# kmjc/riptide

Measured on AMD Instinct MI355X. Metric: DM trials/sec (node) at 2^23 samples, P=0.1-10 s; FFA-pass HBM GB/s, higher is better.
Workload: dtype f32

## Files before the change

### include/riptide_amd.h

```cpp
#ifndef RIPTIDE_AMD_H
#define RIPTIDE_AMD_H

#include <stddef.h>
#include <stdint.h>

#ifdef __cplusplus
extern "C" {
#endif

#define RT_OK 0
#define RT_EINVAL 1
#define RT_EHIP 2
#define RT_EINTERNAL 3

const char* rt_last_error(void);
const char* rt_version(void);
int rt_set_device(int device);


int rt_rollback(const float* x, size_t size, size_t shift, float* out);

int rt_fused_rollback_add(const float* x, const float* y, size_t size, size_t shift, float* out);

int rt_circular_prefix_sum(const float* x, size_t size, size_t nsum, float* out);

int rt_ffa2(const float* in, size_t rows, size_t cols, float* out);

int rt_benchmark_ffa2(size_t rows, size_t cols, size_t loops, double* seconds);

int rt_snr1(const float* x, size_t size, const uint64_t* widths, size_t num_widths, float stdnoise, float* out);

int rt_snr2(const float* x, size_t rows, size_t cols, const uint64_t* widths, size_t num_widths,
            float stdnoise, float* out);

size_t rt_downsampled_size(size_t size, double f);

int rt_downsample(const float* x, size_t size, double factor, float* out);
int rt_downsample_rows(const float* x, size_t rows, size_t size, double f, float* out);

int rt_periodogram_length(size_t size, double tsamp, double period_min, double period_max,
                          size_t bins_min, size_t bins_max, size_t* length);

int rt_periodogram(const float* data, size_t size, double tsamp, const uint64_t* widths, size_t num_widths,
                   double period_min, double period_max, size_t bins_min, size_t bins_max,
                   double* periods, uint32_t* foldbins, float* snrs);

int rt_running_median(const float* x, size_t size, size_t width, float* out);

int rt_fast_running_median(const float* x, size_t size, size_t width_samples, size_t min_points, double* out);

int rt_deredden_normalise(const float* x, size_t size, size_t width_samples, size_t min_points,
                          int deredden, int normalise, float* out);

int rt_periodogram_grid(size_t size, double tsamp, double period_min, double period_max, size_t bins_min,
                        size_t bins_max, double* periods, uint32_t* foldbins);

int rt_schedule_check(size_t size, double tsamp, size_t num_widths, double period_min, double period_max,
                      size_t bins_min, size_t bins_max, uint64_t* transforms, uint64_t* items,
                      uint64_t* launches, double* alg_bytes_per_trial, double* moved_bytes_per_trial,
                      uint64_t* cells_per_trial);

int rt_schedule_final_kinds(size_t size, double tsamp, const uint64_t* widths, size_t num_widths, double period_min,
                            double period_max, size_t bins_min, size_t bins_max, uint64_t* launches,
                            uint64_t* rows_launches, uint64_t* seg_launches, uint8_t* bins_kinds, size_t bins_cap);

int rt_ladder_check(size_t size, double tsamp, double period_min, double period_max, size_t bins_min,
                    size_t bins_max, int* fused, uint64_t* rungs);

typedef struct rt_ladder_rung {
    double   f;
    uint64_t n;
    uint64_t leaf_off;
    uint32_t fused;
    uint32_t reserved;
} rt_ladder_rung;
int rt_ladder_layout(size_t size, double tsamp, double period_min, double period_max, size_t bins_min,
                     size_t bins_max, rt_ladder_rung* rungs, size_t cap, uint64_t* count, uint64_t* leaf_floats,
                     int* mode, uint32_t* margin);

int rt_ffa_schedule_check(size_t rows, size_t cols, uint64_t* launches);


typedef struct rt_plan rt_plan;

int rt_plan_create(size_t size, double tsamp, const uint64_t* widths, size_t num_widths,
                   double period_min, double period_max, size_t bins_min, size_t bins_max,
                   rt_plan** plan);
void rt_plan_destroy(rt_plan* plan);
int rt_plan_shape(const rt_plan* plan, size_t* length, size_t* num_widths);
int rt_plan_grid(const rt_plan* plan, double* periods, uint32_t* foldbins);
int rt_plan_workspace_bytes(const rt_plan* plan, size_t batch, size_t* bytes);

int rt_periodogram_device(const rt_plan* plan, const float* d_data, size_t batch, size_t data_stride,
                          float* d_snrs, size_t snr_stride, void* d_workspace, size_t workspace_bytes,
                          void* stream);
int rt_periodogram_ladder_device(const rt_plan* plan, const float* d_data, size_t batch, size_t data_stride,
                                 void* d_workspace, size_t workspace_bytes, void* stream);
int rt_periodogram_passes_device(const rt_plan* plan, size_t batch, float* d_snrs, size_t snr_stride,
                                 void* d_workspace, size_t workspace_bytes, void* stream);

int rt_plan_check(const rt_plan* plan, void* stream);

int rt_deredden_workspace_bytes(size_t size, size_t width_samples, size_t min_points, size_t batch,
                                size_t* bytes);
int rt_deredden_normalise_device(const float* d_in, size_t size, size_t batch, size_t in_stride,
                                 size_t width_samples, size_t min_points, int deredden, int normalise,
                                 float* d_out, size_t out_stride, void* d_workspace, size_t workspace_bytes,
                                 void* stream);

int rt_segment_order_stats_device(const float* d_snrs, size_t batch, size_t snr_stride, size_t length,
                                  size_t num_widths, size_t nseg, size_t per_seg, const uint32_t* ranks,
                                  size_t nranks, float* d_out, void* stream);
int rt_threshold_select_device(const float* d_snrs, size_t batch, size_t snr_stride, size_t length,
                               size_t num_widths, const double* d_logf, const double* d_coeffs, size_t ncoef,
                               double smin, uint32_t* d_counts, uint32_t* d_idx, size_t cap, void* stream);
int rt_find_peaks_workspace_bytes(size_t batch, size_t length, size_t num_widths, size_t chunk_rows, size_t* bytes);
int rt_find_peaks_device(const float* d_snrs, size_t batch, size_t snr_stride, size_t length, size_t num_widths,
                         const double* d_logf, const double* d_freqs, const double* d_coeffs, size_t ncoef,
                         double smin, double radius, uint32_t* d_counts, uint32_t* d_rows, float* d_snr,
                         size_t cap, size_t chunk_rows, void* d_workspace, size_t workspace_bytes, void* stream);
int rt_find_peaks_host(const float* snrs, size_t length, size_t num_widths, const double* logf, const double* freqs,
                       const double* coeffs, size_t ncoef, double smin, double radius,
                       uint32_t* counts, uint32_t* rows, float* snr, size_t cap);

typedef struct rt_fold_spec {
    double   factor;
    uint64_t out_off;
    uint32_t series;
    uint32_t bins;
    uint32_t subints;
    uint32_t reserved;
} rt_fold_spec;

int rt_fold_shape(size_t size, double factor, size_t bins, size_t subints, size_t* m, size_t* rows);
int rt_fold_workspace_bytes(size_t size, const rt_fold_spec* specs, size_t nspecs, size_t* bytes);
int rt_fold_device(const float* d_data, size_t size, size_t data_stride, size_t nseries,
                   const rt_fold_spec* specs, size_t nspecs, float* d_out, size_t out_floats,
                   void* d_workspace, size_t workspace_bytes, void* stream);
int rt_fold(const float* x, size_t size, size_t nseries, const rt_fold_spec* specs, size_t nspecs,
            float* out, size_t out_floats);

typedef struct rt_htest_params {
    double   tobs;
    double   band;
    double   phase_distance_max;
    double   dm_distance_max;
    double   snr_distance_max;
    uint32_t denom_max;
} rt_htest_params;

int rt_hdiag_host(const double* freq, const double* snr, const double* ducy, const double* dm, size_t n,
                  const int32_t* pi, const int32_t* pj, size_t npairs, const rt_htest_params* params,
                  int64_t* num, int64_t* den, double* phase_distance, double* dm_distance, double* snr_distance);
int rt_hdiag_pairs(const double* freq, const double* snr, const double* ducy, const double* dm, size_t n,
                   const int32_t* pi, const int32_t* pj, size_t npairs, const rt_htest_params* params,
                   int64_t* num, int64_t* den, double* phase_distance, double* dm_distance, double* snr_distance);
int rt_flag_harmonics(const double* freq, const double* snr, const double* ducy, const double* dm, size_t n,
                      const rt_htest_params* params, size_t block_rows, int32_t* parent, int64_t* hnum,
                      int64_t* hden);
int rt_flag_harmonics_stats(uint64_t* tiles, uint64_t* near_pairs, uint64_t* host_rows, double* kernel_ms);

int rt_convert_samples_device(const void* d_raw, size_t n, int is_signed, float* d_out, void* stream);

int rt_profile_enable(int on);
int rt_profile_read(int kind, double* milliseconds, double* alg_bytes, double* moved_bytes, uint64_t* launches);
int rt_profile_reset(void);

int rt_diag_stamps(uint64_t* out8, int reset);
int rt_diag_timeline(uint64_t* out, uint64_t cap, uint64_t* count);
int rt_diag_launches(uint64_t* out, uint64_t cap, uint64_t* count);

int rt_plan_stats(const rt_plan* plan, uint64_t* transforms, uint64_t* items, uint64_t* launches,
                  double* alg_bytes_per_trial, double* moved_bytes_per_trial, uint64_t* cells_per_trial);


#ifdef __cplusplus
}
#endif

#endif
```

### riptide_amd/_lib.py

```python
import ctypes
import os

_HERE = os.path.dirname(os.path.abspath(__file__))
LIB_PATH = os.environ.get("RIPTIDE_AMD_LIB") or os.path.join(_HERE, "libriptide_amd.so")

RT_OK, RT_EINVAL, RT_EHIP, RT_EINTERNAL = 0, 1, 2, 3

_c_sz = ctypes.c_size_t
_c_d = ctypes.c_double
_c_f = ctypes.c_float
_c_i = ctypes.c_int
_vp = ctypes.c_void_p
_psz = ctypes.POINTER(ctypes.c_size_t)
_pd = ctypes.POINTER(ctypes.c_double)
_pu64 = ctypes.POINTER(ctypes.c_uint64)

_SIGNATURES = {
    "rt_last_error": (ctypes.c_char_p, []),
    "rt_version": (ctypes.c_char_p, []),
    "rt_set_device": (_c_i, [_c_i]),
    "rt_rollback": (_c_i, [_vp, _c_sz, _c_sz, _vp]),
    "rt_fused_rollback_add": (_c_i, [_vp, _vp, _c_sz, _c_sz, _vp]),
    "rt_circular_prefix_sum": (_c_i, [_vp, _c_sz, _c_sz, _vp]),
    "rt_ffa2": (_c_i, [_vp, _c_sz, _c_sz, _vp]),
    "rt_benchmark_ffa2": (_c_i, [_c_sz, _c_sz, _c_sz, _pd]),
    "rt_snr1": (_c_i, [_vp, _c_sz, _vp, _c_sz, _c_f, _vp]),
    "rt_snr2": (_c_i, [_vp, _c_sz, _c_sz, _vp, _c_sz, _c_f, _vp]),
    "rt_downsampled_size": (_c_sz, [_c_sz, _c_d]),
    "rt_downsample": (_c_i, [_vp, _c_sz, _c_d, _vp]),
    "rt_downsample_rows": (_c_i, [_vp, _c_sz, _c_sz, _c_d, _vp]),
    "rt_fold_shape": (_c_i, [_c_sz, _c_d, _c_sz, _c_sz, _psz, _psz]),
    "rt_fold_workspace_bytes": (_c_i, [_c_sz, _vp, _c_sz, _psz]),
    "rt_fold_device": (_c_i, [_vp, _c_sz, _c_sz, _c_sz, _vp, _c_sz, _vp, _c_sz, _vp, _c_sz, _vp]),
    "rt_fold": (_c_i, [_vp, _c_sz, _c_sz, _vp, _c_sz, _vp, _c_sz]),
    "rt_periodogram_length": (_c_i, [_c_sz, _c_d, _c_d, _c_d, _c_sz, _c_sz, _psz]),
    "rt_periodogram": (_c_i, [_vp, _c_sz, _c_d, _vp, _c_sz, _c_d, _c_d, _c_sz, _c_sz, _vp, _vp, _vp]),
    "rt_running_median": (_c_i, [_vp, _c_sz, _c_sz, _vp]),
    "rt_fast_running_median": (_c_i, [_vp, _c_sz, _c_sz, _c_sz, _vp]),
    "rt_deredden_normalise": (_c_i, [_vp, _c_sz, _c_sz, _c_sz, _c_i, _c_i, _vp]),
    "rt_periodogram_grid": (_c_i, [_c_sz, _c_d, _c_d, _c_d, _c_sz, _c_sz, _vp, _vp]),
    "rt_ffa_schedule_check": (_c_i, [_c_sz, _c_sz, _pu64]),
    "rt_schedule_check": (_c_i, [_c_sz, _c_d, _c_sz, _c_d, _c_d, _c_sz, _c_sz, _pu64, _pu64, _pu64, _pd, _pd,
                                 _pu64]),
    "rt_schedule_final_kinds": (_c_i, [_c_sz, _c_d, _vp, _c_sz, _c_d, _c_d, _c_sz, _c_sz, _pu64, _pu64, _pu64, _vp,
                                       _c_sz]),
    "rt_plan_create": (_c_i, [_c_sz, _c_d, _vp, _c_sz, _c_d, _c_d, _c_sz, _c_sz, _vp]),
    "rt_plan_destroy": (None, [_vp]),
    "rt_plan_shape": (_c_i, [_vp, _psz, _psz]),
    "rt_plan_grid": (_c_i, [_vp, _vp, _vp]),
    "rt_plan_workspace_bytes": (_c_i, [_vp, _c_sz, _psz]),
    "rt_periodogram_device": (_c_i, [_vp, _vp, _c_sz, _c_sz, _vp, _c_sz, _vp, _c_sz, _vp]),
    "rt_periodogram_ladder_device": (_c_i, [_vp, _vp, _c_sz, _c_sz, _vp, _c_sz, _vp]),
    "rt_periodogram_passes_device": (_c_i, [_vp, _c_sz, _vp, _c_sz, _vp, _c_sz, _vp]),
    "rt_plan_check": (_c_i, [_vp, _vp]),
    "rt_deredden_workspace_bytes": (_c_i, [_c_sz, _c_sz, _c_sz, _c_sz, _psz]),
    "rt_deredden_normalise_device": (_c_i, [_vp, _c_sz, _c_sz, _c_sz, _c_sz, _c_sz, _c_i, _c_i, _vp, _c_sz,
                                            _vp, _c_sz, _vp]),
    "rt_profile_enable": (_c_i, [_c_i]),
    "rt_profile_read": (_c_i, [_c_i, _pd, _pd, _pd, _pu64]),
    "rt_profile_reset": (_c_i, []),
    "rt_diag_stamps": (_c_i, [_pu64, _c_i]),
    "rt_diag_timeline": (_c_i, [_pu64, ctypes.c_uint64, _pu64]),
    "rt_diag_launches": (_c_i, [_pu64, ctypes.c_uint64, _pu64]),
    "rt_plan_stats": (_c_i, [_vp, _pu64, _pu64, _pu64, _pd, _pd, _pu64]),
    "rt_convert_samples_device": (_c_i, [_vp, _c_sz, _c_i, _vp, _vp]),
    "rt_segment_order_stats_device": (_c_i, [_vp, _c_sz, _c_sz, _c_sz, _c_sz, _c_sz, _c_sz, _vp, _c_sz, _vp, _vp]),
    "rt_threshold_select_device": (_c_i, [_vp, _c_sz, _c_sz, _c_sz, _c_sz, _vp, _vp, _c_sz, _c_d, _vp, _vp, _c_sz,
                                          _vp]),
    "rt_find_peaks_workspace_bytes": (_c_i, [_c_sz, _c_sz, _c_sz, _c_sz, _psz]),
    "rt_find_peaks_device": (_c_i, [_vp, _c_sz, _c_sz, _c_sz, _c_sz, _vp, _vp, _vp, _c_sz, _c_d, _c_d, _vp, _vp, _vp,
                                    _c_sz, _c_sz, _vp, _c_sz, _vp]),
    "rt_find_peaks_host": (_c_i, [_vp, _c_sz, _c_sz, _vp, _vp, _vp, _c_sz, _c_d, _c_d, _vp, _vp, _vp, _c_sz]),
    "rt_ladder_check": (_c_i, [_c_sz, _c_d, _c_d, _c_d, _c_sz, _c_sz, ctypes.POINTER(_c_i), _pu64]),
    "rt_ladder_layout": (_c_i, [_c_sz, _c_d, _c_d, _c_d, _c_sz, _c_sz, _vp, _c_sz, _pu64, _pu64,
                                ctypes.POINTER(_c_i), ctypes.POINTER(ctypes.c_uint32)]),
    "rt_hdiag_host": (_c_i, [_vp, _vp, _vp, _vp, _c_sz, _vp, _vp, _c_sz, _vp, _vp, _vp, _vp, _vp, _vp]),
    "rt_hdiag_pairs": (_c_i, [_vp, _vp, _vp, _vp, _c_sz, _vp, _vp, _c_sz, _vp, _vp, _vp, _vp, _vp, _vp]),
    "rt_flag_harmonics": (_c_i, [_vp, _vp, _vp, _vp, _c_sz, _vp, _c_sz, _vp, _vp, _vp]),
    "rt_flag_harmonics_stats": (_c_i, [_pu64, _pu64, _pu64, _pd]),
}

EXPORTED = tuple(_SIGNATURES)

_TEST_SIGNATURES = {
    "rt_test_corrupt_next_plans": (_c_i, [_c_i]),
}
TESTHOOKS_PATH = os.path.join(_HERE, "libriptide_amd_testhooks.so")

_lib = None


class EngineError(RuntimeError):
    """A HIP runtime or internal failure inside the engine."""


def load():
    global _lib
    if _lib is not None:
        return _lib
    if not os.path.exists(LIB_PATH):
        raise ImportError(
            f"riptide_amd engine library not found at {LIB_PATH}; build it with "
            "`make -C riptide_amd/csrc` or `python -c 'import __graft_entry__ as g; g.build()'`")
    try:
        import torch
    except ImportError:
        pass
    lib = ctypes.CDLL(LIB_PATH, mode=ctypes.RTLD_LOCAL)
    for name, (res, args) in _SIGNATURES.items():
        fn = getattr(lib, name)
        fn.restype = res
        fn.argtypes = args
    for name, (res, args) in _TEST_SIGNATURES.items():
        if hasattr(lib, name):
            fn = getattr(lib, name)
            fn.restype = res
            fn.argtypes = args
    _lib = lib
    return lib


def check(rc):
    if rc == RT_OK:
        return
    msg = _lib.rt_last_error().decode("utf-8", "replace")
    if rc == RT_EINVAL:
        raise ValueError(msg)
    raise EngineError(msg)


def ptr(a):
    if hasattr(a, "data_ptr"):
        return ctypes.c_void_p(a.data_ptr())
    return ctypes.c_void_p(a.ctypes.data)
```

### riptide_amd/csrc/common.hpp

```cpp
#pragma once
#include <cmath>
#include <cstddef>
#include <cstdint>

#if defined(__HIPCC__)
#define RT_HD __host__ __device__
#else
#define RT_HD
#endif

namespace rt {

constexpr int kConeWgsPerCu = 2;
constexpr int kConeBlock = 512;
static_assert(kConeBlock % 64 == 0, "whole waves");
constexpr int kConeWaves = kConeBlock / 64;
constexpr int kConeWavesPerSimd = kConeWgsPerCu * kConeWaves / 4;
constexpr int kLdsBufFloats = 18176;
constexpr int kLdsDataFloats = kLdsBufFloats - 256;
constexpr int kLdsPadFloats = 128;
constexpr int kMaxRows = 384;
constexpr int kDescEntries = 1024;
constexpr int kMaxTileLevels = 6;
constexpr int kMaxLevels = 11;
constexpr int kMaxRanges = (1 << (kMaxTileLevels + 1)) - 1;
constexpr int kMaxWidths = 32;
constexpr int kSnrChunk = 17;
constexpr int kSnrWin = 12;
constexpr int kSnrMaxChunk = 17;
RT_HD inline int snr_wide_stride(int p, int wmax)
{
    return p + (wmax > kSnrMaxChunk ? wmax : kSnrMaxChunk);
}
RT_HD inline bool snr_wide_ok(int p, int q, int wmax)
{
    return wmax > kSnrWin && wmax < p && q >= snr_wide_stride(p, wmax);
}
RT_HD constexpr int snr_group(int p)
{
    int G = 8;
    while (G < 64 && ((((p + G - 1) / G) | 1) > kSnrMaxChunk)) G <<= 1;
    return G;
}
constexpr int kSnrSegCols = 33;
constexpr int kSnrSegWmax = 9;
constexpr int kSnrSegRows = 64;
constexpr int kSnrSegStride = 8 * kSnrSegCols + 1;
constexpr int kSnrSegExch = 2 * 64 * 8;
static_assert(kSnrSegRows * kSnrSegStride <= kLdsDataFloats, "segmented S/N rows");
static_assert(kSnrSegRows * kSnrSegStride + kSnrSegExch <= kLdsBufFloats, "segmented S/N exchange area");
RT_HD inline bool snr_seg_ok(int p, int wmax, int rows)
{
    return p >= 8 * kSnrSegCols - 24 && p <= 8 * kSnrSegCols && wmax >= 1 && wmax <= kSnrSegWmax && rows >= 1 &&
           rows <= kSnrSegRows;
}
RT_HD inline bool snr_seg_unit(int smax, int levels, int p, int wmax, int rows)
{
    return (smax == 4 || smax == 5) && levels > 0 && snr_seg_ok(p, wmax, rows);
}
constexpr int kStageRegs = 45 * 8 / kConeWaves;
constexpr int kMaxSlots = 45;
constexpr int kMaxRowsPerWave = 24;
constexpr int kBlobHeader = 48;
enum : int {
    kHdrRows = 0, kHdrDesc = 12, kHdrRuns = 24, kHdrEntries = 25, kHdrBottom = 26, kHdrSlotWords = 27,
    kHdrRunOff = 28, kHdrFill = 29, kHdrZero = 30, kHdrSlotOff = 32
};
enum : uint32_t { kSlotOne = 0, kSlotTwo = 1, kSlotPair = 2, kSlotHalf = 3 };
constexpr int kSlotWords = 544;
RT_HD constexpr bool resolved_slots(int smax) { return smax == 4 || smax == 5; }
constexpr int kAuxMetaWords = kBlobHeader + kDescEntries + kMaxRows + kSlotWords;
constexpr int kLutPad = 64;
constexpr int kLut4Words = 2 * (256 + 64);
constexpr int kLut4Off = kAuxMetaWords + kLutPad - kLut4Words;
constexpr uint32_t kNoBlob = 0xFFFFFFFFu;
constexpr uint32_t kCarriedRow = 1023;
RT_HD inline int fill_chunks_bound(int n, int p, int runs) { return (n * p + 6 * runs + 3) >> 2; }
RT_HD inline int pack_blob_words(int entries, int nb) { return (kBlobHeader + entries + nb + 2 * kMaxLevels + 4) & ~3; }

constexpr int kPack2 = 64;
RT_HD inline int merge_slots(uint32_t p)
{
    if (p <= 32) return kPack2;
    if (p == 0) return 1;
    const int s = (int)((p + 63) / 64);
    if (s <= 5) return s;
    if (s <= 8) return 8;
    if (s <= 11) return 11;
    if (s <= 16) return 16;
    if (s <= 22) return 22;
    if (s <= kMaxSlots) return kMaxSlots;
    return 0;
}

RT_HD inline int pack_stride(int p)
{
    if (p < 8) return p;
    if (p < 16) return p <= 8 ? 9 : 17;
    if (p <= 32)
        return p == 16 ? 34 : p < 20 ? 35 : p < 25 ? 36 : p < 28 ? 37 : p == 28 ? 36 : p == 29 ? 37 : 38;
    return p | 1;
}
RT_HD constexpr int slot_count(int smax) { return smax == kPack2 ? 1 : smax; }
RT_HD constexpr int row_pack(int smax) { return smax == kPack2 ? 2 : 1; }

constexpr int kRw4 = (72 + kConeWaves - 1) / kConeWaves;
RT_HD constexpr int merge_rows_per_wave(int smax)
{
    return smax == 4
               ? kRw4
               : (kStageRegs / slot_count(smax) < 1
                      ? 1
                      : (kStageRegs / slot_count(smax) < kMaxRowsPerWave ? kStageRegs / slot_count(smax)
                                                                         : kMaxRowsPerWave));
}

RT_HD inline int lds_row_capacity(uint32_t p, int smax)
{
    if (!smax || p == 0) return 0;
    int c = kLdsDataFloats / (int)p;
    const int stage = kConeWaves * merge_rows_per_wave(smax) * row_pack(smax);
    if (stage < c) c = stage;
    return c < kMaxRows ? c : kMaxRows;
}

RT_HD inline int lds_row_capacity(uint32_t p) { return lds_row_capacity(p, merge_slots(p)); }

constexpr uint32_t kDsSpanFloats = 4096;
constexpr uint32_t kDsFusedMargin = 512;
constexpr uint32_t kDsMaxRungs = 256;

struct DsRung {
    double f;
    uint64_t n;
    uint64_t out_off;
    uint32_t first_block;
    uint32_t identity;
    uint32_t per_block;
    uint32_t staged;
};

inline uint32_t ds_per_block(double f)
{
    const double o = std::floor((double)(kDsSpanFloats - 4) / (f + 1.0)) - 1.0;
    if (o < 1.0) return 0;
    return o > 256.0 ? 256u : (uint32_t)o;
}

inline void ds_configure(DsRung& r)
{
    const uint32_t o = r.identity ? 256u : ds_per_block(r.f);
    r.staged = o >= 32;
    r.per_block = r.staged ? o : 256u;
}

inline uint32_t ds_fused_margin(const DsRung* rungs, size_t num_rungs)
{
    double need = 2.0;
    for (size_t i = 0; i < num_rungs; ++i)
        if (!rungs[i].identity) need = std::fmax(need, std::ceil(rungs[i].f) + 2.0);
    if (need > (double)kDsFusedMargin) return 0;
    const uint32_t m = ((uint32_t)need + 63u) & ~63u;
    return m < kDsFusedMargin ? m : kDsFusedMargin;
}

struct FfaXform {
    uint32_t p;
    uint32_t m;
    uint32_t rows_eval;
    uint32_t rung;
    uint64_t src_off;
    uint64_t buf_off;
    uint64_t snr_row;
    float stdnoise;
    uint32_t pad;
};
static_assert(sizeof(FfaXform) == 48, "FfaXform layout");

enum : uint8_t { kModeWhole = 0, kModeTile = 1 };
constexpr int kStampMarks = 16;
constexpr int kStampRecWords = kStampMarks + 2;
constexpr uint64_t kTimelineCap = 1u << 23;
enum : uint32_t {
    kConeStoreFromRegs = 1u,
    kConeFuse2 = 2u,
    kConeSnrStride = 4u,
    kConeSnrSeg = 8u,
    kConeDiagNoSnr = 1u << 30,
    kConeDiagNoMerge = 1u << 29,
    kConeDiagNoWrite = 1u << 28,
    kConeDiagNoBarrier = 1u << 27,
    kConeDiagNoLand = 1u << 26,
    kConeDiagNoDesc = 1u << 25,
    kConeDiagNoFill = 1u << 23,
    kConeDefaultFeatures = 15u
};
enum : uint8_t { kSelLeaves = 0, kSelPing = 1, kSelPong = 2, kSelSnr = 3, kSelSnrSeg = 4 };
RT_HD inline bool is_snr_dst(int dst) { return dst == kSelSnr || dst == kSelSnrSeg; }
enum : uint32_t { kSnrNone = 0, kSnrRows = 1, kSnrSeg = 2 };

struct ConeItem {
    uint32_t xform;
    uint32_t node_start;
    uint32_t node_size;
    uint32_t s0, s1;
    uint8_t levels;
    uint8_t mode;
    uint8_t src;
    uint8_t dst;
    uint32_t pad;
};
static_assert(sizeof(ConeItem) == 28, "ConeItem layout");

struct UnitDesc {
    uint32_t node_start, node_size, s0, s1;
    uint32_t p, m, rows_eval;
    float stdnoise;
    uint64_t src_off, buf_off, snr_row;
    uint8_t levels, mode, src, dst;
    uint32_t pad;
    uint32_t nruns, entries, nb, slot_words, run_off;
    uint32_t fill_chunks;
    uint32_t zero_row;
    uint32_t pad2;
};
static_assert(sizeof(UnitDesc) == 96, "UnitDesc layout");

struct ConeArgs {
    const UnitDesc* items;
    uint32_t num_items;
    uint32_t num_widths;
    const float* leaves;
    uint64_t leaves_stride;
    float* ping;
    float* pong;
    uint64_t buf_stride;
    float* snr;
    uint64_t snr_stride;
    const uint32_t* widths;
    int* error_flag;
    const uint32_t* blob;
    unsigned long long* stamps;
    uint32_t batch;
    uint32_t flags;
    uint32_t trials_per_wg;
};
constexpr uint32_t kConeTrialsPerWg = 16;
RT_HD inline uint32_t cone_trial_groups(uint32_t batch, uint32_t tpw)
{
    const uint32_t t = tpw ? tpw : 1u;
    return (batch + t - 1) / t;
}

#if defined(__HIPCC__)
__host__ __device__
#endif
inline uint32_t merge_index(float k, uint32_t s)
{
#if defined(__HIP_DEVICE_COMPILE__)
    return (uint32_t)__builtin_fmaf(k, (float)s, 0.5f);
#else
    return (uint32_t)__builtin_fmaf(k, (float)s, 0.5f);
#endif
}

#if defined(__HIPCC__)
__host__ __device__
#endif
inline float merge_coef(uint32_t child_rows, uint32_t rows)
{
    return ((float)child_rows - 1.0f) / ((float)rows - 1.0f);
}

}
```

### riptide_amd/csrc/ffa_kernels.hip

```cpp
#include <hip/hip_runtime.h>

#include <cstdlib>

#include "common.hpp"
#include "kernels.hpp"

namespace rt {

template <int N> struct IntC { static constexpr int value = N; };

__device__ __forceinline__ float window_sum(const float* w, float wmin, uint32_t cnt)
{
    float acc = __fmul_rn(wmin, w[0]);
    uint32_t i = 1;
    for (; i + 8 <= cnt; i += 8) {
        float v[8];
#pragma unroll
        for (int j = 0; j < 8; ++j) v[j] = w[i + j];
#pragma unroll
        for (int j = 0; j < 8; ++j) acc = __fadd_rn(acc, v[j]);
    }
    if (i < cnt) {
        float v[8];
#pragma unroll
// ... 341 lines not shown
}

template <class T>
__device__ __forceinline__ T* uni_ptr(T* p)
{
    return reinterpret_cast<T*>(uni64(reinterpret_cast<uint64_t>(p)));
}

struct UnitView {
    int item, trial;
    int node_start, node_size, s0, s1, levels, mode, src, dst;
    int p, m, rows_eval;
    uint64_t src_off, buf_off, snr_row;
    float stdnoise;
    uint32_t blob;
    int nruns, entries, nb, slot_words, run_off;
    int fill_chunks;
    int zero_row;
};

typedef const __attribute__((address_space(4))) uint32_t* const_u32_ptr;

__device__ __forceinline__ UnitView unit_view(const ConeArgs& a, int item, int trial)
{
    UnitView v;
    v.item = uni(item);
    v.trial = uni(trial);
    const const_u32_ptr w = (const_u32_ptr)(uintptr_t)(a.items + v.item);
    uint32_t x[sizeof(UnitDesc) / 4];
#pragma unroll
    for (int i = 0; i < (int)(sizeof(UnitDesc) / 4); ++i) x[i] = w[i];
    UnitDesc d;
    __builtin_memcpy(&d, x, sizeof d);
    v.node_start = uni((int)d.node_start);
    v.node_size = uni((int)d.node_size);
    v.s0 = uni((int)d.s0);
    v.s1 = uni((int)d.s1);
    v.levels = uni((int)d.levels);
    v.mode = uni((int)d.mode);
    v.src = uni((int)d.src);
    v.dst = uni((int)d.dst);
    v.p = uni((int)d.p);
    v.m = uni((int)d.m);
    v.rows_eval = uni((int)d.rows_eval);
    v.src_off = uni64(d.src_off);
    v.buf_off = uni64(d.buf_off);
    v.snr_row = uni64(d.snr_row);
    v.stdnoise = __int_as_float(uni(__float_as_int(d.stdnoise)));
    v.blob = (uint32_t)uni((int)d.pad);
    v.nruns = uni((int)d.nruns);
    v.entries = uni((int)d.entries);
    v.nb = uni((int)d.nb);
    v.slot_words = uni((int)d.slot_words);
    v.run_off = uni((int)d.run_off);
    v.fill_chunks = uni((int)d.fill_chunks);
    v.zero_row = uni((int)d.zero_row);
    return v;
}

constexpr int kAuxWords = kBlobHeader + kDescEntries + kMaxRows + kSlotWords;
static_assert(kAuxWords == kAuxMetaWords, "metadata area");
struct UnitCtx {
    UnitView U;
    bool tile;
    bool table;
    int al;
    bool slots;
    int nruns, entries, nb;
    const uint32_t* aux;
    const uint32_t* aux0;
    uint4 sv;
    int mine;
};

__device__ __forceinline__ int rows_at(const UnitCtx& C, int l)
{
    return C.table ? uni((int)C.aux[kHdrRows + l]) : C.U.node_size;
}
__device__ __forceinline__ int desc_offset(const UnitCtx& C, int l) { return uni((int)C.aux[kHdrDesc + l]); }
__device__ __forceinline__ const uint32_t* desc_table(const UnitCtx& C) { return C.aux + kBlobHeader; }
__device__ __forceinline__ const uint32_t* slot_table(const UnitCtx& C, int lo)
{
    return C.aux + uni((int)C.aux[kHdrSlotOff + lo]);
}
__device__ __forceinline__ const int* bottom_offsets(const UnitCtx& C)
{
    return reinterpret_cast<const int*>(desc_table(C) + C.entries);
}

__device__ __forceinline__ __amdgpu_buffer_rsrc_t buffer_rsrc(const void* p, uint32_t bytes)
{
    return __builtin_amdgcn_make_buffer_rsrc(uni_ptr(const_cast<void*>(p)), (short)0, uni((int)bytes), 0x00020000);
}

__device__ __forceinline__ void dma_run(__amdgpu_buffer_rsrc_t rs, uint32_t goff, int nch, float* lds, int wave,
                                        int wstep, int lane)
{
    for (int c0 = wave * 64; c0 < nch; c0 += wstep * 64) {
        const int c = c0 + lane;
        if (c < nch)
            __builtin_amdgcn_raw_ptr_buffer_load_lds(rs, (__attribute__((address_space(3))) void*)(lds + 4 * c0), 16,
                                                     (int)(goff + 16u * (uint32_t)c), 0, 0, kFillCpol);
    }
}

__device__ __forceinline__ __amdgpu_buffer_rsrc_t unit_src(const ConeArgs& a, const UnitView& U, int trial)
{
    const float* src;
    if (U.src == kSelLeaves) src = a.leaves + (uint64_t)trial * a.leaves_stride + U.src_off;
    else src = (U.src == kSelPing ? a.ping : a.pong) + (uint64_t)trial * a.buf_stride + U.buf_off;
    return buffer_rsrc(src, (((uint32_t)U.m * (uint32_t)U.p + 3u) & ~3u) * 4u);
}

template <int SMAX>
__device__ __forceinline__ void unit_fill(const ConeArgs& a, const UnitCtx& C, int trial, float* buf, int tid,
                                          bool blob_too)
{
    const int lane = tid & 63, wave = tid >> 6;
    const UnitView& U = C.U;
    const int p = U.p;
    const __amdgpu_buffer_rsrc_t rs = unit_src(a, U, trial);
    if (!C.table) {
        const int nch = (U.node_size * p + C.al + 3) >> 2;
        dma_run(rs, ((uint32_t)U.node_start * (uint32_t)p - (uint32_t)C.al) * 4u, nch, buf, wave, kConeWaves, lane);
        return;
    }
    const int words = U.run_off;
    const uint4 sv = C.sv;
    const int mine = C.mine;
    if (blob_too && wave == kConeWaves - 1) {
        const __amdgpu_buffer_rsrc_t rb = buffer_rsrc(a.blob + U.blob, (uint32_t)words * 4u);
        dma_run(rb, 0u, words >> 2, (float*)const_cast<uint32_t*>(C.aux), 0, 1, lane);
    }
    for (int i = 0; i < mine; ++i) {
        const int c0 = __builtin_amdgcn_readlane((int)sv.x, i);
        const int n = __builtin_amdgcn_readlane((int)sv.y, i);
        const uint32_t g = (uint32_t)__builtin_amdgcn_readlane((int)sv.z, i);
        if (lane < n && 4 * (c0 + n) <= kLdsBufFloats && !(a.flags & kConeDiagNoFill))
            __builtin_amdgcn_raw_ptr_buffer_load_lds(rs, (__attribute__((address_space(3))) void*)(buf + 4 * c0), 16,
                                                     (int)((g + (uint32_t)lane) * 16u), 0, 0, kFillCpol);
    }
}

__device__ __forceinline__ void unit_segments(const ConeArgs& a, UnitCtx& C, int tid)
{
    const int lane = tid & 63, wave = tid >> 6;
    const uint4* const segs = reinterpret_cast<const uint4*>(a.blob + C.U.blob + C.U.run_off);
    C.mine = uni(C.nruns > wave ? (C.nruns - wave + kConeWaves - 1) / kConeWaves : 0);
    C.sv = make_uint4(0u, 0u, 0u, 0u);
    const int K = (C.nruns + kConeWaves - 1) / kConeWaves;
    if (lane < C.mine) C.sv = segs[wave * K + lane];
}

template <int SMAX, int RW>
__device__ __forceinline__ UnitCtx unit_begin(const ConeArgs& a, uint32_t item, uint32_t trial, uint32_t* aux,
                                              float* buf, int tid, bool dma, bool& ok, unsigned long long* ts = nullptr)
{
    UnitCtx C;
    C.U = unit_view(a, (int)item, (int)trial);
    const UnitView& U = C.U;
#ifdef RT_STAMPS
    if (ts) ts[0] = __builtin_amdgcn_s_memtime() + (U.p & 0);
#endif
    C.tile = U.mode == kModeTile;
    C.table = U.blob != kNoBlob;
    C.aux = aux;
    C.aux0 = aux;
    const int p = U.p;
    const int slots = merge_slots((uint32_t)p);
    ok = U.levels <= kMaxLevels && p > 0 &&
         ((SMAX <= 5 || SMAX == kPack2) ? slots == SMAX : (slots <= SMAX && slots != kPack2));
    const int cap = min(lds_row_capacity((uint32_t)p, SMAX), kConeWaves * RW * row_pack(SMAX));
    if (!C.table) {
        ok = ok && SMAX != kPack2 && (!resolved_slots(SMAX) || U.levels == 0);
        C.al = (int)(((uint32_t)U.node_start * (uint32_t)p) & 3u);
        C.slots = false;
        C.nruns = C.entries = C.nb = 0;
        const int nch = (U.node_size * p + C.al + 3) >> 2;
        ok = ok && !C.tile && U.node_size <= cap && 4 * nch <= kLdsBufFloats;
    } else {
        C.al = 0;
        C.nruns = U.nruns;
        C.entries = U.entries;
        C.nb = U.nb;
        C.slots = U.slot_words != 0;
        const int words = U.run_off;
        if constexpr (SMAX == kPack2) {
            C.aux = reinterpret_cast<uint32_t*>(buf + kLdsBufFloats) - words;
            ok = ok && C.nb <= cap && 4 * U.fill_chunks + words <= kLdsBufFloats &&
                 C.nb * pack_stride(p) + words <= kLdsBufFloats;
        } else {
            ok = ok && C.nb <= cap && C.entries <= kDescEntries && words <= kAuxWords;
            if (SMAX == 4 && C.slots) ok = ok && words <= kLut4Off;
            if (resolved_slots(SMAX)) ok = ok && (U.levels == 0 || (C.slots && (a.flags & kConeFuse2)));
            if (U.zero_row)
                ok = ok && resolved_slots(SMAX) && !C.tile && U.zero_row >= 4 * U.fill_chunks &&
                     U.zero_row + 64 * SMAX <= kLdsDataFloats;
        }
        ok = ok && words >= kBlobHeader + C.entries + C.nb && C.nruns <= 64 * kConeWaves && (words & 3) == 0;
    }
#ifdef RT_STAMPS
    if (ts) ts[1] = __builtin_amdgcn_s_memtime() + (ok ? 0 : 0);
#endif
    C.sv = make_uint4(0u, 0u, 0u, 0u);
    C.mine = 0;
    if (ok && dma) {
        if (C.table) unit_segments(a, C, tid);
        unit_fill<SMAX>(a, C, (int)trial, buf, tid, true);
    }
#ifdef RT_STAMPS
    if (ts) ts[2] = __builtin_amdgcn_s_memtime();
#endif
    return C;
}

__device__ __forceinline__ int mod_small(int x, int p)
{
    const int q = (int)((float)x * __builtin_amdgcn_rcpf((float)p));
    int r = x - (int)__umul24((unsigned)q, (unsigned)p);
    r = r < 0 ? r + p : r;
    return r >= p ? r - p : r;
}

__device__ __forceinline__ void row_desc(int node_size, int l, int r, int p, int& h, int& t, int& sh)
{
    int a0 = 0, sz = node_size;
    for (int d = 0; d < l; ++d) {
        if (sz > 1) {
            const int hs = sz >> 1;
            if (r - a0 < hs) sz = hs;
            else {
                a0 += hs;
                sz -= hs;
            }
        }
    }
    if (sz <= 1) {
        h = r;
        t = -1;
        sh = 0;
    } else {
        const int s = r - a0;
        const uint32_t hs = (uint32_t)sz >> 1, ts = (uint32_t)sz - hs;
        const int hh = (int)merge_index(merge_coef(hs, (uint32_t)sz), (uint32_t)s);
        const int tt = (int)merge_index(merge_coef(ts, (uint32_t)sz), (uint32_t)s);
        h = a0 + hh;
        t = a0 + (int)hs + tt;
        sh = mod_small(s - tt, p);
    }
}

constexpr uint32_t kCarried = kCarriedRow;

__device__ __forceinline__ uint32_t pack_desc(int h, int t, int sh)
{
    return (uint32_t)h | ((t < 0 ? kCarried : (uint32_t)t) << 10) | ((uint32_t)sh << 20);
}

__device__ __forceinline__ uint32_t unit_desc(const UnitCtx& C, int l, int r, int p)
{
    if (C.table) return desc_table(C)[desc_offset(C, l) + r];
    int h, t, sh;
    row_desc(C.U.node_size, l, r, p, h, t, sh);
    return pack_desc(h, t, sh);
}

typedef const __attribute__((address_space(3))) float* lds_cptr;

__device__ __forceinline__ float lds_ld(lds_cptr p) { return *(const volatile __attribute__((address_space(3))) float*)p; }

template <int SMAX, int RW, bool CARRIED>
__device__ __forceinline__ void merge_level_dense(const UnitCtx& C, const float* src, int p, int l, int lane,
                                                  int wave, int nr, float (&v)[RW][SMAX], const int* loff)
{
    const int S = (p + 63) >> 6;
    int ho = 0, to = 0, sh = 0, car = 0;
    if (lane < nr) {
        const uint32_t d = unit_desc(C, l, wave + kConeWaves * lane, p);
        const uint32_t tc = (d >> 10) & 1023u;
        sh = (int)(d >> 20);
        ho = loff ? loff[d & 1023u] : (int)(d & 1023u) * p;
        to = (tc == kCarried ? ho : (loff ? loff[tc] : (int)tc * p)) + sh;
        car = tc == kCarried;
    }
    const lds_cptr l1 = (lds_cptr)src + lane;
#pragma unroll
    for (int i = 0; i < RW; ++i) {
        const int hoi = __builtin_amdgcn_readlane(ho, i);
        const int toi = __builtin_amdgcn_readlane(to, i);
        const int si = __builtin_amdgcn_readlane(sh, i);
        uint32_t keep = 0xFFFFFFFFu, neg0 = 0u;
        if (CARRIED) {
            keep = __builtin_amdgcn_readlane(car, i) ? 0u : 0xFFFFFFFFu;
            neg0 = ~keep & 0x80000000u;
        }
        const lds_cptr hrow = l1 + hoi;
        lds_cptr ta = l1 + toi;
        lds_cptr tw = ta - p;
        asm("" : "+v"(ta), "+v"(tw));
        const int ls = lane + si;
#pragma unroll
        for (int k = 0; k < SMAX; ++k) {
            if (SMAX <= 5 || k < S) {
                const lds_cptr tp = ls >= p - 64 * k ? tw : ta;
                float x = lds_ld(tp + 64 * k);
                if (CARRIED) x = __uint_as_float((__float_as_uint(x) & keep) | neg0);
                v[i][k] = __fadd_rn(hrow[64 * k], x);
            }
        }
    }
}

template <int SMAX, int RW>
__device__ __forceinline__ void merge_level2_dense(const UnitCtx& C, const float* src, int p, int l, int lane,
                                                   int wave, int nr, float (&v)[RW][SMAX], const int* loff)
{
    const int S = (p + 63) >> 6;
    int o0 = 0, o1 = 0, o2 = 0, o3 = 0, s1 = 0, s2 = 0, s3 = 0;
    if (lane < nr) {
        const uint32_t d0 = unit_desc(C, l, wave + kConeWaves * lane, p);
        const uint32_t dh = unit_desc(C, l + 1, (int)(d0 & 1023u), p);
        const uint32_t dt = unit_desc(C, l + 1, (int)((d0 >> 10) & 1023u), p);
        const int sh = (int)(d0 >> 20), sH = (int)(dh >> 20), sT = (int)(dt >> 20);
        int sTT = sh + sT;
        sTT = sTT >= p ? sTT - p : sTT;
        const uint32_t r0 = dh & 1023u, r1 = (dh >> 10) & 1023u, r2 = dt & 1023u, r3 = (dt >> 10) & 1023u;
        o0 = (loff ? loff[r0] : (int)r0 * p);
        o1 = (loff ? loff[r1] : (int)r1 * p) + sH;
        o2 = (loff ? loff[r2] : (int)r2 * p) + sh;
        o3 = (loff ? loff[r3] : (int)r3 * p) + sTT;
        s1 = sH;
        s2 = sh;
        s3 = sTT;
    }
    const lds_cptr l1 = (lds_cptr)src + lane;
#pragma unroll
    for (int i = 0; i < RW; ++i) {
        const lds_cptr hrow = l1 + __builtin_amdgcn_readlane(o0, i);
        lds_cptr b1 = l1 + __builtin_amdgcn_readlane(o1, i);
        lds_cptr b2 = l1 + __builtin_amdgcn_readlane(o2, i);
        lds_cptr b3 = l1 + __builtin_amdgcn_readlane(o3, i);
        lds_cptr w1 = b1 - p, w2 = b2 - p, w3 = b3 - p;
        asm("" : "+v"(b1), "+v"(w1), "+v"(b2), "+v"(w2), "+v"(b3), "+v"(w3));
        const int ls1 = lane + __builtin_amdgcn_readlane(s1, i);
        const int ls2 = lane + __builtin_amdgcn_readlane(s2, i);
        const int ls3 = lane + __builtin_amdgcn_readlane(s3, i);
#pragma unroll
        for (int k = 0; k < SMAX; ++k) {
            if (SMAX <= 5 || k < S) {
                const int wk = p - 64 * k;
// ... 93 lines not shown
        }
    } else if constexpr (!HEAD) {
        lds_cptr ta = l1 + r1;
        lds_cptr tw = ta - p;
        asm("" : "+v"(ta), "+v"(tw));
        const int ls = lane + t1;
#pragma unroll
        for (int k = 0; k < SMAX; ++k) ts[k] = lds_ld((ls >= p - 64 * k ? tw : ta) + 64 * k);
    } else {
        const lds_cptr hrow = l1 + r0;
        lds_cptr ta = l1 + r1;
        lds_cptr tw = ta - p;
        asm("" : "+v"(ta), "+v"(tw));
        const int ls = lane + t1;
        const uint32_t keep = c1 ? 0u : 0xFFFFFFFFu;
        const uint32_t neg0 = ~keep & 0x80000000u;
#pragma unroll
        for (int k = 0; k < SMAX; ++k) {
            const float x = lds_ld((ls >= p - 64 * k ? tw : ta) + 64 * k);
            hs[k] = lds_ld(hrow + 64 * k);
            ts[k] = __uint_as_float((__float_as_uint(x) & keep) | neg0);
        }
    }
}

typedef const __attribute__((address_space(3))) unsigned long long* lut_cptr;
typedef const __attribute__((address_space(3))) char* lds_ccptr;

__device__ __forceinline__ void rolled_lut4(lds_ccptr rb, unsigned long long e, float (&x)[4])
{
    const uint32_t e0 = (uint32_t)e, e1 = (uint32_t)(e >> 32);
    x[0] = lds_ld((lds_cptr)(rb + (e0 & 0xFFFFu)));
    x[1] = lds_ld((lds_cptr)(rb + (e0 >> 16)));
    x[2] = lds_ld((lds_cptr)(rb + (e1 & 0xFFFFu)));
    x[3] = lds_ld((lds_cptr)(rb + (e1 >> 16)));
}

template <bool TWO, bool HEAD = true>
__device__ __forceinline__ void row_terms_lut(lds_cptr l1, lds_cptr s0, lut_cptr lutl, int r0, int q1, int q2, int q3,
                                              int t1, int t2, int t3, int c1, float (&hs)[4], float (&ts)[4])
{
    const lds_ccptr b = (lds_ccptr)s0;
    if constexpr (TWO) {
        const unsigned long long e1 = HEAD ? lutl[t1] : 0ull;
        const unsigned long long e2 = lutl[t2], e3 = lutl[t3];
        float h[4], x1[4], x2[4], x3[4];
        if constexpr (HEAD) {
#pragma unroll
            for (int k = 0; k < 4; ++k) h[k] = lds_ld(l1 + r0 + 64 * k);
            rolled_lut4(b + 4 * q1, e1, x1);
        }
        rolled_lut4(b + 4 * q2, e2, x2);
        rolled_lut4(b + 4 * q3, e3, x3);
#pragma unroll
        for (int k = 0; k < 4; ++k) {
            if constexpr (HEAD) hs[k] = __fadd_rn(h[k], x1[k]);
            ts[k] = __fadd_rn(x2[k], x3[k]);
        }
    } else {
        const unsigned long long e = lutl[t1];
        float x[4];
        if constexpr (HEAD) {
#pragma unroll
            for (int k = 0; k < 4; ++k) hs[k] = lds_ld(l1 + r0 + 64 * k);
        }
        rolled_lut4(b + 4 * q1, e, x);
        if constexpr (HEAD) {
            const uint32_t keep = c1 ? 0u : 0xFFFFFFFFu;
            const uint32_t neg0 = ~keep & 0x80000000u;
#pragma unroll
            for (int k = 0; k < 4; ++k) ts[k] = __uint_as_float((__float_as_uint(x[k]) & keep) | neg0);
        } else {
#pragma unroll
            for (int k = 0; k < 4; ++k) ts[k] = x[k];
        }
    }
}

__device__ __forceinline__ void build_roll_lut4(uint32_t* lut, int p, int tid)
{
    for (int w = tid; w < 2 * (p + 64); w += kConeBlock) {
        const int x = (w >> 1) + 128 * (w & 1);
        int y0 = x, y1 = x + 64;
        y0 -= y0 >= p ? p : 0;
        y0 -= y0 >= p ? p : 0;
        y1 -= y1 >= p ? p : 0;
        y1 -= y1 >= p ? p : 0;
        lut[w] = (uint32_t)(4 * y0) | ((uint32_t)(4 * y1) << 16);
    }
}

template <int SMAX, bool TWO, bool HEAD = true>
__device__ __forceinline__ void row_terms(lds_cptr l1, int p, int lane, int i, int o0, int o1, int o2, int o3, int s1,
                                          int s2, int s3, float (&hs)[SMAX], float (&ts)[SMAX],
                                          lds_cptr s0 = nullptr, lut_cptr lutl = nullptr)
{
    if constexpr (SMAX == 4) {
        if constexpr (TWO) {
            if constexpr (HEAD) {
                int r0 = __builtin_amdgcn_readlane(o0, i), q1 = __builtin_amdgcn_readlane(o1, i);
                int q2 = __builtin_amdgcn_readlane(o2, i), q3 = __builtin_amdgcn_readlane(o3, i);
                int t1 = __builtin_amdgcn_readlane(s1, i), t2 = __builtin_amdgcn_readlane(s2, i);
                int t3 = __builtin_amdgcn_readlane(s3, i);
                asm volatile("" : "+s"(r0), "+s"(q1), "+s"(q2), "+s"(q3), "+s"(t1), "+s"(t2), "+s"(t3));
                row_terms_lut<true>(l1, s0, lutl, r0, q1, q2, q3, t1, t2, t3, 0, hs, ts);
            } else {
                int q2 = __builtin_amdgcn_readlane(o2, i), q3 = __builtin_amdgcn_readlane(o3, i);
                int t2 = __builtin_amdgcn_readlane(s2, i), t3 = __builtin_amdgcn_readlane(s3, i);
                asm volatile("" : "+s"(q2), "+s"(q3), "+s"(t2), "+s"(t3));
                row_terms_lut<true, false>(l1, s0, lutl, 0, 0, q2, q3, 0, t2, t3, 0, hs, ts);
            }
        } else {
            if constexpr (HEAD) {
                int r0 = __builtin_amdgcn_readlane(o0, i), q1 = __builtin_amdgcn_readlane(o1, i);
                int t1 = __builtin_amdgcn_readlane(s1, i), c1 = __builtin_amdgcn_readlane(o2, i);
                asm volatile("" : "+s"(r0), "+s"(q1), "+s"(t1), "+s"(c1));
                row_terms_lut<false>(l1, s0, lutl, r0, q1, 0, 0, t1, 0, 0, c1, hs, ts);
            } else {
                int q1 = __builtin_amdgcn_readlane(o1, i), t1 = __builtin_amdgcn_readlane(s1, i);
                asm volatile("" : "+s"(q1), "+s"(t1));
                row_terms_lut<false, false>(l1, s0, lutl, 0, q1, 0, 0, t1, 0, 0, 0, hs, ts);
            }
        }
        return;
    }
    if constexpr (TWO) {
        if constexpr (HEAD) {
            int r0 = __builtin_amdgcn_readlane(o0, i), r1 = __builtin_amdgcn_readlane(o1, i);
            int r2 = __builtin_amdgcn_readlane(o2, i), r3 = __builtin_amdgcn_readlane(o3, i);
            int t1 = __builtin_amdgcn_readlane(s1, i), t2 = __builtin_amdgcn_readlane(s2, i);
            int t3 = __builtin_amdgcn_readlane(s3, i);
            asm volatile("" : "+s"(r0), "+s"(r1), "+s"(r2), "+s"(r3), "+s"(t1), "+s"(t2), "+s"(t3));
            row_terms_s<SMAX, true>(l1, p, lane, r0, r1, r2, r3, t1, t2, t3, 0, hs, ts);
        } else {
            int r2 = __builtin_amdgcn_readlane(o2, i), r3 = __builtin_amdgcn_readlane(o3, i);
            int t2 = __builtin_amdgcn_readlane(s2, i), t3 = __builtin_amdgcn_readlane(s3, i);
            asm volatile("" : "+s"(r2), "+s"(r3), "+s"(t2), "+s"(t3));
            row_terms_s<SMAX, true, false>(l1, p, lane, 0, 0, r2, r3, 0, t2, t3, 0, hs, ts);
        }
    } else {
        if constexpr (HEAD) {
            int r0 = __builtin_amdgcn_readlane(o0, i), r1 = __builtin_amdgcn_readlane(o1, i);
            int t1 = __builtin_amdgcn_readlane(s1, i), c1 = __builtin_amdgcn_readlane(o2, i);
            asm volatile("" : "+s"(r0), "+s"(r1), "+s"(t1), "+s"(c1));
            row_terms_s<SMAX, false>(l1, p, lane, r0, r1, 0, 0, t1, 0, 0, c1, hs, ts);
        } else {
            int r1 = __builtin_amdgcn_readlane(o1, i), t1 = __builtin_amdgcn_readlane(s1, i);
            asm volatile("" : "+s"(r1), "+s"(t1));
            row_terms_s<SMAX, false, false>(l1, p, lane, 0, r1, 0, 0, t1, 0, 0, 0, hs, ts);
        }
    }
}

template <int SMAX, int RW, bool TWO>
__device__ __forceinline__ void merge_step_slots(const UnitCtx& C, const float* src, int p, int lo, int lane,
                                                 int wave, float (&v)[RW][SMAX], const int* loff, uint32_t& sw,
                                                 int& nq)
{
    constexpr int Q = (RW + 1) / 2;
    static_assert(Q <= 32, "row slots: one lane per slot row");
    const uint32_t* st = slot_table(C, lo);
    const int ns = uni((int)st[0]);
    nq = uni(ns > wave ? (ns - wave + kConeWaves - 1) / kConeWaves : 0);
    const int qi = lane & 31;
    int o0 = 0, o1 = 0, o2 = 0, o3 = 0, s1 = 0, s2 = 0, s3 = 0;
    if constexpr (resolved_slots(SMAX)) {
        const int qc = qi < Q ? qi : Q - 1;
        const uint4 e = reinterpret_cast<const uint4*>(st)[1 + (lane >> 5) * (kConeWaves * Q) + wave * Q + qc];
        sw = lane < 32 ? e.w : 0u;
        s1 = (int)(e.z & 1023u);
        constexpr int roll_in = SMAX == 4 ? 0 : 1;
        if constexpr (TWO) {
            s2 = (int)((e.z >> 10) & 1023u);
            s3 = (int)((e.z >> 20) & 1023u);
            o0 = (int)(e.x & 0xFFFFu);
            o1 = (int)(e.x >> 16) + roll_in * s1;
            o2 = (int)(e.y & 0xFFFFu) + roll_in * s2;
            o3 = (int)(e.y >> 16) + roll_in * s3;
        } else {
            o0 = (int)(e.x & 0xFFFFu);
            o1 = (int)(e.x >> 16) + roll_in * s1;
            o2 = (int)((e.z >> 30) & 1u);
        }
        (void)loff;
    } else {
    sw = qi < nq ? st[1 + wave + kConeWaves * qi] : 0u;
    const bool act = qi < nq && (lane < 32 || (sw >> 20) == kSlotTwo || (sw >> 20) == kSlotHalf);
    const int r = lane < 32 ? (int)(sw & 1023u) : (int)((sw >> 10) & 1023u);
    const uint32_t* const desc = desc_table(C);
    const bool use_loff = loff != nullptr;
    if (act) {
        if constexpr (TWO) {
            const uint32_t d0 = desc[desc_offset(C, lo) + r];
            const uint32_t dh = desc[desc_offset(C, lo + 1) + (int)(d0 & 1023u)];
            const uint32_t dt = desc[desc_offset(C, lo + 1) + (int)((d0 >> 10) & 1023u)];
            const int sh = (int)(d0 >> 20), sH = (int)(dh >> 20), sT = (int)(dt >> 20);
            int sTT = sh + sT;
            sTT = sTT >= p ? sTT - p : sTT;
            const uint32_t r0 = dh & 1023u, r1 = (dh >> 10) & 1023u, r2 = dt & 1023u, r3 = (dt >> 10) & 1023u;
            o0 = (use_loff ? loff[r0] : (int)__umul24(r0, (uint32_t)p));
            o1 = (use_loff ? loff[r1] : (int)__umul24(r1, (uint32_t)p)) + sH;
            o2 = (use_loff ? loff[r2] : (int)__umul24(r2, (uint32_t)p)) + sh;
            o3 = (use_loff ? loff[r3] : (int)__umul24(r3, (uint32_t)p)) + sTT;
            s1 = sH;
            s2 = sh;
            s3 = sTT;
        } else {
            const uint32_t d = desc[desc_offset(C, lo) + r];
            const uint32_t tc = (d >> 10) & 1023u;
            s1 = (int)(d >> 20);
            o0 = use_loff ? loff[d & 1023u] : (int)__umul24(d & 1023u, (uint32_t)p);
            o1 = (tc == kCarried ? o0 : (use_loff ? loff[tc] : (int)__umul24(tc, (uint32_t)p))) + s1;
            o2 = tc == kCarried;
        }
    }
    }
    const lds_cptr l1 = (lds_cptr)src + lane;
    const lds_cptr s0 = (lds_cptr)src;
    const lut_cptr lutl = (lut_cptr)(C.aux0 + kLut4Off) + lane;
    const int jl = p - 1 - 64 * (SMAX - 1);
#pragma unroll
    for (int q = 0; q < Q; ++q) {
        if (q < nq) {
            const uint32_t kq = (uint32_t)__builtin_amdgcn_readlane((int)sw, q) >> 20;
            float hs[SMAX], ts[SMAX];
            row_terms<SMAX, TWO>(l1, p, lane, q, o0, o1, o2, o3, s1, s2, s3, hs, ts, s0, lutl);
#pragma unroll
            for (int k = 0; k < SMAX; ++k) v[2 * q][k] = __fadd_rn(hs[k], ts[k]);
            const int qb = 2 * q + 1 < RW ? 2 * q + 1 : RW - 1;
            if (2 * q + 1 < RW) {
                if (kq == kSlotPair) {
#ifdef RT_PAIR_SELECT
                    int n0[SMAX];
#pragma unroll
                    for (int k = 0; k < SMAX; ++k) n0[k] = __builtin_amdgcn_readlane(__float_as_int(ts[(k + 1) % SMAX]), 0);
#pragma unroll
                    for (int k = 0; k < SMAX; ++k) {
                        float x = __int_as_float(__builtin_amdgcn_mov_dpp(__float_as_int(ts[k]), 0x130, 0xF, 0xF, true));
                        x = lane == (k + 1 < SMAX ? 63 : jl) ? __int_as_float(n0[k]) : x;
                        v[qb][k] = __fadd_rn(hs[k], x);
                    }
#else
                    const int w0 = __builtin_amdgcn_readlane(__float_as_int(ts[0]), 0);
#pragma unroll
                    for (int k = 0; k < SMAX; ++k) {
                        int x;
                        if (k + 1 < SMAX) {
                            const int nx = __builtin_amdgcn_mov_dpp(__float_as_int(ts[k + 1]), 0x134, 0xF, 0xF, false);
                            x = __builtin_amdgcn_update_dpp(nx, __float_as_int(ts[k]), 0x130, 0xF, 0xF, false);
                        } else {
                            x = __builtin_amdgcn_mov_dpp(__float_as_int(ts[k]), 0x130, 0xF, 0xF, true);
                            asm volatile("s_mov_b32 m0, %2\n\tv_writelane_b32 %0, %1, m0" : "+v"(x) : "s"(w0), "s"(jl)
                                         : "m0");
                        }
                        v[qb][k] = __fadd_rn(hs[k], __int_as_float(x));
                    }
#endif
                } else if (kq == kSlotHalf) {
                    float tb[SMAX];
                    row_terms<SMAX, TWO, false>(l1, p, lane, 32 + q, o0, o1, o2, o3, s1, s2, s3, hs, tb, s0, lutl);
#pragma unroll
                    for (int k = 0; k < SMAX; ++k) v[qb][k] = __fadd_rn(hs[k], tb[k]);
                } else if (kq == kSlotTwo) {
                    row_terms<SMAX, TWO>(l1, p, lane, 32 + q, o0, o1, o2, o3, s1, s2, s3, hs, ts, s0, lutl);
#pragma unroll
                    for (int k = 0; k < SMAX; ++k) v[qb][k] = __fadd_rn(hs[k], ts[k]);
                }
            }
        }
    }
}

#ifndef RT_NO_ADDTID_WRITES
template <int SMAX>
__device__ __forceinline__ void write_row_addtid(uint32_t a, const float (&x)[SMAX])
{
    static_assert(SMAX == 4 || SMAX == 5, "4/5-slot rows");
    if (a <= 0xFFFFu - 256u * (SMAX - 2)) {
        if constexpr (SMAX == 4)
            asm volatile("s_mov_b32 m0, %0\n\ts_nop 0\n\tds_write_addtid_b32 %1\n\tds_write_addtid_b32 %2 offset:256\n\t"
                         "ds_write_addtid_b32 %3 offset:512"
                         :: "s"(a), "v"(x[0]), "v"(x[1]), "v"(x[2]) : "memory", "m0");
        else
            asm volatile("s_mov_b32 m0, %0\n\ts_nop 0\n\tds_write_addtid_b32 %1\n\tds_write_addtid_b32 %2 offset:256\n\t"
                         "ds_write_addtid_b32 %3 offset:512\n\tds_write_addtid_b32 %4 offset:768"
                         :: "s"(a), "v"(x[0]), "v"(x[1]), "v"(x[2]), "v"(x[3]) : "memory", "m0");
    } else {
        const uint32_t b = a - 32768u;
        if constexpr (SMAX == 4)
            asm volatile("s_mov_b32 m0, %0\n\ts_nop 0\n\tds_write_addtid_b32 %1 offset:32768\n\t"
                         "ds_write_addtid_b32 %2 offset:33024\n\tds_write_addtid_b32 %3 offset:33280"
                         :: "s"(b), "v"(x[0]), "v"(x[1]), "v"(x[2]) : "memory", "m0");
        else
            asm volatile("s_mov_b32 m0, %0\n\ts_nop 0\n\tds_write_addtid_b32 %1 offset:32768\n\t"
                         "ds_write_addtid_b32 %2 offset:33024\n\tds_write_addtid_b32 %3 offset:33280\n\t"
                         "ds_write_addtid_b32 %4 offset:33536"
                         :: "s"(b), "v"(x[0]), "v"(x[1]), "v"(x[2]), "v"(x[3]) : "memory", "m0");
    }
}
#endif

template <int SMAX, int RW>
__device__ __forceinline__ void write_rows_slots(float* base, float* dummy, const float (&v)[RW][SMAX], int p,
                                                 int lane, uint32_t sw, int nq, int q)
{
    const bool tail_ok = lane + 64 * (SMAX - 1) < p;
#ifndef RT_NO_ADDTID_WRITES
    if constexpr (resolved_slots(SMAX)) {
        typedef __attribute__((address_space(3))) float* lds_fptr;
        const uint32_t b0 = (uint32_t)(uintptr_t)(lds_fptr)base;
#pragma unroll
        for (int i = 0; i < RW; ++i) {
            if (i / 2 < nq) {
                const uint32_t w = (uint32_t)__builtin_amdgcn_readlane((int)sw, i / 2);
                if (i % 2 == 0 || (w >> 20) != kSlotOne) {
                    const int row = (int)((i % 2 == 0 ? w : w >> 10) & 1023u);
                    write_row_addtid<SMAX>(b0 + 4u * (uint32_t)(row * q), v[i]);
                    float* orow = base + row * q + lane;
                    *(tail_ok ? orow + 64 * (SMAX - 1) : dummy) = v[i][SMAX - 1];
                }
            }
        }
        return;
    }
#endif
#pragma unroll
    for (int i = 0; i < RW; ++i) {
        if (i / 2 < nq) {
            const uint32_t w = (uint32_t)__builtin_amdgcn_readlane((int)sw, i / 2);
            if (i % 2 == 0 || (w >> 20) != kSlotOne) {
                const int row = (int)((i % 2 == 0 ? w : w >> 10) & 1023u);
                float* orow = base + row * q + lane;
#pragma unroll
                for (int k = 0; k < SMAX; ++k) {
                    if (k < SMAX - 1) orow[64 * k] = v[i][k];
                    else *(tail_ok ? orow + 64 * k : dummy) = v[i][k];
                }
            }
        }
    }
}

template <int SMAX, int RW>
__device__ __forceinline__ void store_rows_slots(const float (&v)[RW][SMAX], int p, int lane, uint32_t sw, int nq,
                                                 __amdgpu_buffer_rsrc_t rs, uint32_t st_o0)
{
    const bool tail_ok = lane + 64 * (SMAX - 1) < p;
#pragma unroll
    for (int i = 0; i < RW; ++i) {
        if (i / 2 < nq) {
            const uint32_t w = (uint32_t)__builtin_amdgcn_readlane((int)sw, i / 2);
            if (i % 2 == 0 || (w >> 20) != kSlotOne) {
                const int row = (int)((i % 2 == 0 ? w : w >> 10) & 1023u);
                const uint32_t ob = st_o0 + (uint32_t)(row * p + lane) * 4u;
#pragma unroll
                for (int k = 0; k < SMAX; ++k) {
                    const uint32_t o = k < SMAX - 1 ? ob + 256u * (uint32_t)k
                                                    : (tail_ok ? ob + 256u * (uint32_t)k : 0x80000000u);
                    __builtin_amdgcn_raw_buffer_store_b32(__float_as_uint(v[i][k]), rs, (int)o, 0, kStoreCpol);
                }
            }
        }
    }
}

template <int RW, bool TWO, bool FIRST>
__device__ __forceinline__ void merge_step_lanes(const UnitCtx& C, const float* src, int p, int lo, int lane, int wave,
                                                 int nrows, float (&v)[RW][1], const int* loff)
{
    int ln = lane;
    asm volatile("" : "+v"(ln));
    const int h = ln >> 5, j = (ln & 31) < p ? (ln & 31) : 0;
    const uint32_t* const desc = desc_table(C);
    const int dl = TWO ? 0 : desc_offset(C, lo);
    const uint2* const step = reinterpret_cast<const uint2*>(TWO ? slot_table(C, lo) : C.aux);
    const lds_cptr sp = (lds_cptr)src;
    constexpr int G = 4;
    auto rowidx = [&](int i) {
        const int r = 2 * (wave + kConeWaves * i) + h;
        return r < nrows ? r : nrows - 1;
    };
    uint2 enext = make_uint2(0u, 0u);
    auto row = [&](int i, bool pre) {
        const int r = rowidx(i);
        if constexpr (TWO) {
            const uint2 e = enext;
            if (pre) enext = step[rowidx(i + 1)];
            const uint32_t q0 = e.x & 1023u, q1 = (e.x >> 10) & 1023u, q2 = (e.x >> 20) & 1023u, q3 = e.y & 1023u;
            const int sH = (int)((e.y >> 10) & 63u), sh = (int)((e.y >> 16) & 63u), sTT = (int)((e.y >> 22) & 63u);
            const int o0 = FIRST ? loff[q0] : (int)__umul24(q0, (uint32_t)p);
            const int o1 = FIRST ? loff[q1] : (int)__umul24(q1, (uint32_t)p);
            const int o2 = FIRST ? loff[q2] : (int)__umul24(q2, (uint32_t)p);
            const int o3 = FIRST ? loff[q3] : (int)__umul24(q3, (uint32_t)p);
            uint32_t u1 = (uint32_t)(j + sH), u2 = (uint32_t)(j + sh), u3 = (uint32_t)(j + sTT);
            const int i1 = (int)min(u1, u1 - (uint32_t)p), i2 = (int)min(u2, u2 - (uint32_t)p);
            const int i3 = (int)min(u3, u3 - (uint32_t)p);
            const float x0 = lds_ld(sp + o0 + j);
            const float x1 = lds_ld(sp + o1 + i1);
            const float x2 = lds_ld(sp + o2 + i2);
            const float x3 = lds_ld(sp + o3 + i3);
            v[i][0] = __fadd_rn(__fadd_rn(x0, x1), __fadd_rn(x2, x3));
        } else {
            const uint32_t d = desc[dl + r];
            const uint32_t tc = (d >> 10) & 1023u;
            const bool car = tc == kCarried;
            const int sh = (int)(d >> 20);
            const int ho = FIRST ? loff[d & 1023u] : (int)__umul24(d & 1023u, (uint32_t)p);
            const int to = car ? ho : (FIRST ? loff[tc & 1023u] : (int)__umul24(tc, (uint32_t)p));
            const uint32_t u1 = (uint32_t)(j + sh);
            const int i1 = (int)min(u1, u1 - (uint32_t)p);
            const float x0 = lds_ld(sp + ho + j);
            float x1 = lds_ld(sp + to + i1);
            x1 = car ? -0.0f : x1;
            v[i][0] = __fadd_rn(x0, x1);
        }
    };
#pragma unroll
    for (int g = 0; g < RW; g += G) {
        if (2 * (wave + kConeWaves * g) < nrows) {
            const int ge = g + G < RW ? g + G : RW;
            if constexpr (TWO) enext = step[rowidx(g)];
#pragma unroll
            for (int i = g; i < ge; ++i) row(i, i + 1 < ge);
        }
    }
}

template <int RW>
__device__ __forceinline__ void write_rows_lanes(float* base, float* dummy, const float (&v)[RW][1], int p, int lane,
                                                 int wave, int nrows)
{
    int ln = lane;
    asm volatile("" : "+v"(ln));
    const int h = ln >> 5, j = ln & 31;
#pragma unroll
    for (int i = 0; i < RW; ++i) {
        if (2 * (wave + kConeWaves * i) < nrows) {
            const int r = 2 * (wave + kConeWaves * i) + h;
            *((r < nrows && j < p) ? base + (int)__umul24((uint32_t)r, (uint32_t)p) + j : dummy) = v[i][0];
        }
    }
}

template <int RW>
__device__ __forceinline__ void store_rows_lanes(const float (&v)[RW][1], int p, int lane, int wave, int nrows,
                                                 __amdgpu_buffer_rsrc_t rs, uint32_t st_o0)
{
    int ln = lane;
    asm volatile("" : "+v"(ln));
    const int h = ln >> 5, j = ln & 31;
#pragma unroll
    for (int i = 0; i < RW; ++i) {
        if (2 * (wave + kConeWaves * i) < nrows) {
            const int r = 2 * (wave + kConeWaves * i) + h;
            const uint32_t o = (r < nrows && j < p) ? st_o0 + (__umul24((uint32_t)r, (uint32_t)p) + (uint32_t)j) * 4u : 0x80000000u;
            __builtin_amdgcn_raw_buffer_store_b32(__float_as_uint(v[i][0]), rs, (int)o, 0, 0);
        }
    }
}

constexpr int kPackSeg = 8;
constexpr int kPackTasks = 3;
static_assert(kMaxRows * 4 <= kPackTasks * kConeBlock, "short-row tasks per lane");
RT_HD inline int pack_segments(int p) { return (p + kPackSeg - 1) / kPackSeg; }

__device__ __forceinline__ void pack_task(int t, int segs, int p, int& r, int& j0)
{
    const uint32_t m = segs == 1 ? (1u << 20) : (segs == 2 ? (1u << 19) : (segs == 3 ? 349526u : (1u << 18)));
    r = (int)(__umul24((uint32_t)t, m) >> 20);
    j0 = min((t - r * segs) * kPackSeg, p - kPackSeg);
}

__device__ __forceinline__ void pack_rolled_lut(lds_cptr sp, int o, unsigned long long e, float (&x)[kPackSeg])
{
    const lds_ccptr rb = (lds_ccptr)(sp + o);
    const uint32_t e0 = (uint32_t)e, e1 = (uint32_t)(e >> 32);
#pragma unroll
    for (int k = 0; k < 4; ++k) x[k] = lds_ld((lds_cptr)(rb + ((e0 >> (8 * k)) & 0xFFu)));
#pragma unroll
    for (int k = 0; k < 4; ++k) x[4 + k] = lds_ld((lds_cptr)(rb + ((e1 >> (8 * k)) & 0xFFu)));
}

constexpr int kPackLutI = 128;
static_assert(kPackLutI + 2 * (32 + 4) <= kAuxWords, "short-row roll tables");

__device__ __forceinline__ void build_pack_lut(uint32_t* lut, int p, int tid)
{
    for (int w = tid; w < 4 * p; w += kConeBlock) {
        const int x = (w >> 1) + 4 * (w & 1);
        uint32_t word = 0;
#pragma unroll
        for (int i = 0; i < 4; ++i) {
            int y = x + i;
            y -= y >= p ? p : 0;
            y -= y >= p ? p : 0;
            word |= (uint32_t)(4 * y) << (8 * i);
        }
        lut[w] = word;
    }
    const int segs = pack_segments(p);
    if (segs >= 2)
        for (int w = tid; w < 2 * (p + segs); w += kConeBlock) {
            const int x = w >> 1, e0 = 4 * (w & 1);
            uint32_t word = 0;
#pragma unroll
            for (int i = 0; i < 4; ++i) {
                int y = x + segs * (e0 + i);
                y -= y >= p ? p : 0;
                y -= y >= p ? p : 0;
                word |= (uint32_t)(4 * y) << (8 * i);
            }
            lut[kPackLutI + w] = word;
        }
}

template <int SEGS>
__device__ __forceinline__ void pack_task_i(int t, int& r, int& seg)
{
    r = t / SEGS;
    seg = t - r * SEGS;
}

template <bool TWO, bool FIRST, int SEGS>
__device__ __forceinline__ void merge_step_tasks(const UnitCtx& C, const float* src, int p, int qs, int lo, int tid,
                                                 int nrows, float (&v)[kPackTasks][kPackSeg], const int* loff)
{
    const lut_cptr plut = (lut_cptr)(C.aux0 + (SEGS ? kPackLutI : 0));
    const int segs = SEGS ? SEGS : pack_segments(p);
    constexpr int ES = SEGS ? SEGS : 1;
    const int ntask = nrows * segs;
    const uint32_t* const desc = desc_table(C);
    const int dl = TWO ? 0 : desc_offset(C, lo);
    const uint2* const step = reinterpret_cast<const uint2*>(TWO ? slot_table(C, lo) : C.aux);
    const lds_cptr sp = (lds_cptr)src;
    const int wave0 = tid & ~63;
#pragma unroll
    for (int i = 0; i < kPackTasks; ++i) {
        if (kConeBlock * i + wave0 < ntask) {
            int r, j0;
            if constexpr (SEGS) pack_task_i<SEGS>(min(tid + kConeBlock * i, ntask - 1), r, j0);
            else pack_task(min(tid + kConeBlock * i, ntask - 1), segs, p, r, j0);
            float x0[kPackSeg], x1[kPackSeg];
            if constexpr (TWO) {
                const uint2 e = step[r];
                const uint32_t q0 = e.x & 1023u, q1 = (e.x >> 10) & 1023u, q2 = (e.x >> 20) & 1023u, q3 = e.y & 1023u;
                const int sH = (int)((e.y >> 10) & 63u), sh = (int)((e.y >> 16) & 63u), sTT = (int)((e.y >> 22) & 63u);
                const int o0 = FIRST ? loff[q0] : (int)__umul24(q0, (uint32_t)qs);
                const int o1 = FIRST ? loff[q1] : (int)__umul24(q1, (uint32_t)qs);
                const int o2 = FIRST ? loff[q2] : (int)__umul24(q2, (uint32_t)qs);
                const int o3 = FIRST ? loff[q3] : (int)__umul24(q3, (uint32_t)qs);
                float x2[kPackSeg], x3[kPackSeg];
                const lds_cptr h0 = sp + o0 + j0;
                const unsigned long long e1 = plut[j0 + sH], e2 = plut[j0 + sh], e3 = plut[j0 + sTT];
#pragma unroll
                for (int k = 0; k < kPackSeg; ++k) x0[k] = lds_ld(h0 + ES * k);
                pack_rolled_lut(sp, o1, e1, x1);
                pack_rolled_lut(sp, o2, e2, x2);
                pack_rolled_lut(sp, o3, e3, x3);
#pragma unroll
                for (int k = 0; k < kPackSeg; ++k) v[i][k] = __fadd_rn(__fadd_rn(x0[k], x1[k]), __fadd_rn(x2[k], x3[k]));
            } else {
                const uint32_t d = desc[dl + r];
                const uint32_t tc = (d >> 10) & 1023u;
                const bool car = tc == kCarried;
                const int sh = (int)(d >> 20);
                const int ho = FIRST ? loff[d & 1023u] : (int)__umul24(d & 1023u, (uint32_t)qs);
                const int to = car ? ho : (FIRST ? loff[tc & 1023u] : (int)__umul24(tc, (uint32_t)qs));
                const lds_cptr h0 = sp + ho + j0;
                const unsigned long long e1 = plut[j0 + (car ? 0 : sh)];
#pragma unroll
                for (int k = 0; k < kPackSeg; ++k) x0[k] = lds_ld(h0 + ES * k);
                pack_rolled_lut(sp, to, e1, x1);
#pragma unroll
                for (int k = 0; k < kPackSeg; ++k) v[i][k] = __fadd_rn(x0[k], car ? -0.0f : x1[k]);
            }
        }
    }
}

typedef uint32_t v4u __attribute__((ext_vector_type(4)));

template <bool GLOBAL, int SEGS>
__device__ __forceinline__ void put_tasks(float* base, int q, const float (&v)[kPackTasks][kPackSeg], int p, int tid,
                                          int nrows, __amdgpu_buffer_rsrc_t rs, uint32_t st_o0)
{
    static_assert(!(GLOBAL && SEGS), "HBM stores take the contiguous tasks");
    const int segs = SEGS ? SEGS : pack_segments(p);
    constexpr int ES = SEGS ? SEGS : 1;
    const int ntask = nrows * segs;
    const int wave0 = tid & ~63;
#pragma unroll
    for (int i = 0; i < kPackTasks; ++i) {
        if (kConeBlock * i + wave0 < ntask) {
            int r, j0;
            if constexpr (SEGS) pack_task_i<SEGS>(min(tid + kConeBlock * i, ntask - 1), r, j0);
            else pack_task(min(tid + kConeBlock * i, ntask - 1), segs, p, r, j0);
            if constexpr (GLOBAL) {
                const uint32_t ob = st_o0 + (uint32_t)(r * p + j0) * 4u;
#pragma unroll
                for (int k = 0; k < kPackSeg; k += 4) {
                    const v4u w = {__float_as_uint(v[i][k]), __float_as_uint(v[i][k + 1]),
                                   __float_as_uint(v[i][k + 2]), __float_as_uint(v[i][k + 3])};
                    __builtin_amdgcn_raw_buffer_store_b128(w, rs, (int)(ob + 4u * k), 0, 0);
                }
            } else {
                float* const o = base + r * q + j0;
#pragma unroll
                for (int k = 0; k < kPackSeg; ++k) o[ES * k] = v[i][k];
            }
        }
    }
}

template <int SMAX, int RW, class PreStore>
__device__ __forceinline__ void merge_levels(const UnitCtx& C, float* base, int p, int L, int tid, bool st,
                                             __amdgpu_buffer_rsrc_t rs, uint32_t st_o0, uint32_t flags, float* dummy,
                                             int qout, int oshift, PreStore&& pre_store)
{
    const int lane = tid & 63, wave = tid >> 6;
    const bool tile = C.tile;
    const int node_size = C.U.node_size;
    const int* const loff = C.table ? bottom_offsets(C) : nullptr;
    float* const src0 = C.table ? base : base + C.al;
    const bool fuse = (flags & kConeFuse2) != 0;
    if constexpr (SMAX == kPack2) {
        if (p >= kPackSeg) {
            const int qs = pack_stride(p);
            for (int l = L - 1; l >= 0;) {
                const bool two = fuse && l >= 1 && (tile || (node_size >> l) >= 2);
                const int lo = two ? l - 1 : l;
                const int nrows = rows_at(C, lo);
                float v[kPackTasks][kPackSeg];
                const bool first = l == L - 1;
                const float* src = first ? src0 : base;
                const int segs = pack_segments(p);
                const int inter = (segs >= 2 && !(lo == 0 && st)) ? segs : 0;
                auto step = [&](auto sc) {
                    constexpr int S = decltype(sc)::value;
                    if (first) {
                        if (two) merge_step_tasks<true, true, S>(C, src, p, qs, lo, tid, nrows, v, loff);
                        else merge_step_tasks<false, true, S>(C, src, p, qs, lo, tid, nrows, v, loff);
                    } else {
                        if (two) merge_step_tasks<true, false, S>(C, src, p, qs, lo, tid, nrows, v, nullptr);
                        else merge_step_tasks<false, false, S>(C, src, p, qs, lo, tid, nrows, v, nullptr);
                    }
                };
                if (inter == 2) step(IntC<2>{});
                else if (inter == 3) step(IntC<3>{});
                else if (inter == 4) step(IntC<4>{});
                else step(IntC<0>{});
                l = lo - 1;
                if (lo == 0 && st) {
                    pre_store();
                    put_tasks<true, 0>(base, qs, v, p, tid, nrows, rs, st_o0);
                    return;
                }
                if (!(flags & kConeDiagNoBarrier)) lds_barrier();
                if (!(flags & kConeDiagNoWrite)) {
                    const int qw = lo == 0 ? qout : qs;
                    if (inter == 2) put_tasks<false, 2>(base, qw, v, p, tid, nrows, rs, st_o0);
                    else if (inter == 3) put_tasks<false, 3>(base, qw, v, p, tid, nrows, rs, st_o0);
                    else if (inter == 4) put_tasks<false, 4>(base, qw, v, p, tid, nrows, rs, st_o0);
                    else put_tasks<false, 0>(base, qw, v, p, tid, nrows, rs, st_o0);
                }
                if (!(flags & kConeDiagNoBarrier)) lds_barrier();
            }
            return;
        }
        for (int l = L - 1; l >= 0;) {
            const bool two = fuse && l >= 1 && (tile || (node_size >> l) >= 2);
            const int lo = two ? l - 1 : l;
            const int nrows = rows_at(C, lo);
            float v[RW][1];
            const bool first = l == L - 1;
            const float* src = first ? src0 : base;
            const int* lo_src = first ? loff : nullptr;
            if (first) {
                if (two) merge_step_lanes<RW, true, true>(C, src, p, lo, lane, wave, nrows, v, lo_src);
                else merge_step_lanes<RW, false, true>(C, src, p, lo, lane, wave, nrows, v, lo_src);
            } else {
                if (two) merge_step_lanes<RW, true, false>(C, src, p, lo, lane, wave, nrows, v, lo_src);
                else merge_step_lanes<RW, false, false>(C, src, p, lo, lane, wave, nrows, v, lo_src);
            }
            l = lo - 1;
            if (lo == 0 && st) {
                pre_store();
                store_rows_lanes<RW>(v, p, lane, wave, nrows, rs, st_o0);
                return;
            }
            if (!(flags & kConeDiagNoBarrier)) lds_barrier();
            if (!(flags & kConeDiagNoWrite)) write_rows_lanes<RW>(base, dummy, v, p, lane, wave, nrows);
            if (!(flags & kConeDiagNoBarrier)) lds_barrier();
        }
        return;
    }
    if constexpr (SMAX <= 5) {
        if (resolved_slots(SMAX) || (C.slots && fuse)) {
            const bool all2 = C.U.zero_row != 0;
            for (int l = L - 1; l >= 0;) {
                const bool two = l >= 1 && (tile || all2 || (node_size >> l) >= 2);
                const int lo = two ? l - 1 : l;
                float v[RW][SMAX];
                const bool first = l == L - 1;
                const float* src = first ? src0 : base;
                const int* lo_src = first ? loff : nullptr;
                uint32_t sw;
                int nq;
                if (two) merge_step_slots<SMAX, RW, true>(C, src, p, lo, lane, wave, v, lo_src, sw, nq);
                else merge_step_slots<SMAX, RW, false>(C, src, p, lo, lane, wave, v, lo_src, sw, nq);
                l = lo - 1;
                if (lo == 0 && st) {
                    pre_store();
                    store_rows_slots<SMAX, RW>(v, p, lane, sw, nq, rs, st_o0);
                    return;
                }
                if (!(flags & kConeDiagNoBarrier)) lds_barrier();
                if (!(flags & kConeDiagNoWrite))
                    write_rows_slots<SMAX, RW>(lo == 0 ? base + oshift : base, dummy, v, p, lane, sw, nq,
                                               lo == 0 ? qout : p);
                if (!(flags & kConeDiagNoBarrier)) lds_barrier();
            }
            return;
        }
    }
    if constexpr (!resolved_slots(SMAX)) {
    for (int l = L - 1; l >= 0;) {
        const bool two = fuse && l >= 1 && (tile || (node_size >> l) >= 2);
        const int lo = two ? l - 1 : l;
        const int orows = rows_at(C, lo);
        const int nr = uni(orows > wave ? (orows - wave + kConeWaves - 1) / kConeWaves : 0);
        constexpr int S = slot_count(SMAX);
        float v[RW][S];
        const bool carried = !tile && (node_size >> l) < 2;
        const bool first = l == L - 1;
        const float* src = first ? src0 : base;
        const int* lo_src = first ? loff : nullptr;
        if (two)
            merge_level2_dense<S, RW>(C, src, p, lo, lane, wave, nr, v, lo_src);
        else if (carried)
            merge_level_dense<S, RW, true>(C, src, p, l, lane, wave, nr, v, lo_src);
        else
            merge_level_dense<S, RW, false>(C, src, p, l, lane, wave, nr, v, lo_src);
        l = lo - 1;
        if (lo == 0 && st) {
            pre_store();
            store_rows<S, RW>(v, p, lane, wave, nr, rs, st_o0);
            return;
        }
        if (!(flags & kConeDiagNoBarrier)) lds_barrier();
        if (!(flags & kConeDiagNoWrite)) {
            write_rows<S, RW>(base, dummy, v, p, lane, wave, nr);
        }
        if (!(flags & kConeDiagNoBarrier)) lds_barrier();
    }
    }
}

template <int CTRL>
__device__ __forceinline__ double dpp_d(double v)
{
    const int lo = __builtin_amdgcn_update_dpp(0, __double2loint(v), CTRL, 0xF, 0xF, true);
    const int hi = __builtin_amdgcn_update_dpp(0, __double2hiint(v), CTRL, 0xF, 0xF, true);
    return __hiloint2double(hi, lo);
}

template <int CTRL, int ROWS>
__device__ __forceinline__ double dpp_d_rows(double v)
{
    const int lo = __builtin_amdgcn_update_dpp(0, __double2loint(v), CTRL, ROWS, 0xF, false);
    const int hi = __builtin_amdgcn_update_dpp(0, __double2hiint(v), CTRL, ROWS, 0xF, false);
    return __hiloint2double(hi, lo);
}

template <int G>
__device__ __forceinline__ double seg_scan_dpp(double v, int lane)
{
    const int g = lane & (G < 16 ? G - 1 : 15);
    double y = dpp_d<0x111>(v);
    v = g >= 1 ? v + y : v;
    if (G >= 4) {
        y = dpp_d<0x112>(v);
        v = g >= 2 ? v + y : v;
    }
    if (G >= 8) {
        y = dpp_d<0x114>(v);
        v = g >= 4 ? v + y : v;
    }
    if (G >= 16) {
        y = dpp_d<0x118>(v);
        v = g >= 8 ? v + y : v;
    }
    if (G >= 32) v = v + dpp_d_rows<0x142, 0xA>(v);
    if (G >= 64) v = v + dpp_d_rows<0x143, 0xC>(v);
    return v;
}

template <int CH, int W>
__device__ __forceinline__ float window_max(const float (&z)[CH + kSnrWin], const float (&cp)[CH])
{
    float dm = -INFINITY;
#pragma unroll
    for (int i = 0; i + 1 < CH; i += 2) {
        float t0, t1;
        asm volatile("v_sub_f32 %1, %3, %4\n\tv_sub_f32 %2, %5, %6\n\tv_max3_f32 %0, %0, %1, %2"
                     : "+v"(dm), "=&v"(t0), "=&v"(t1)
                     : "v"(z[i + W]), "v"(cp[i]), "v"(z[i + 1 + W]), "v"(cp[i + 1]));
    }
    if constexpr (CH & 1) {
        float t0;
        asm volatile("v_sub_f32 %1, %2, %3\n\tv_max_f32 %0, %0, %1"
                     : "+v"(dm), "=&v"(t0)
                     : "v"(z[CH - 1 + W]), "v"(cp[CH - 1]));
    }
    return dm;
}

template <int CH>
__device__ __forceinline__ float window_dispatch(int w, const float (&z)[CH + kSnrWin], const float (&cp)[CH])
{
    static_assert(kSnrWin == 12, "cases below");
    switch (w) {
    case 1: return window_max<CH, 1>(z, cp);
    case 2: return window_max<CH, 2>(z, cp);
    case 3: return window_max<CH, 3>(z, cp);
    case 4: return window_max<CH, 4>(z, cp);
    case 5: return window_max<CH, 5>(z, cp);
    case 6: return window_max<CH, 6>(z, cp);
    case 7: return window_max<CH, 7>(z, cp);
    case 8: return window_max<CH, 8>(z, cp);
    case 9: return window_max<CH, 9>(z, cp);
    case 10: return window_max<CH, 10>(z, cp);
    case 11: return window_max<CH, 11>(z, cp);
    case 12: return window_max<CH, 12>(z, cp);
    default: return -INFINITY;
    }
}

constexpr int kStdWidths[6] = {1, 2, 3, 4, 6, 9};

template <int CH, int W>
__device__ __forceinline__ float window_max_nv(const float (&z)[CH + kSnrWin], const float (&cp)[CH])
{
    float dm = -INFINITY;
#pragma unroll
    for (int i = 0; i + 1 < CH; i += 2) {
        float t0, t1;
        asm("v_sub_f32 %1, %3, %4\n\tv_sub_f32 %2, %5, %6\n\tv_max3_f32 %0, %0, %1, %2"
            : "+v"(dm), "=&v"(t0), "=&v"(t1)
            : "v"(z[i + W]), "v"(cp[i]), "v"(z[i + 1 + W]), "v"(cp[i + 1]));
    }
    if constexpr (CH & 1) {
        float t0;
        asm("v_sub_f32 %1, %2, %3\n\tv_max_f32 %0, %0, %1" : "+v"(dm), "=&v"(t0) : "v"(z[CH - 1 + W]), "v"(cp[CH - 1]));
    }
    return dm;
}

#define RT_MAX6_STEP(CTRL)                                                                                  \
    asm volatile("v_max_f32_dpp %0, %0, %0 " CTRL " row_mask:0xf bank_mask:0xf\n\t"                        \
                 "v_max_f32_dpp %1, %1, %1 " CTRL " row_mask:0xf bank_mask:0xf\n\t"                        \
                 "v_max_f32_dpp %2, %2, %2 " CTRL " row_mask:0xf bank_mask:0xf\n\t"                        \
                 "v_max_f32_dpp %3, %3, %3 " CTRL " row_mask:0xf bank_mask:0xf\n\t"                        \
                 "v_max_f32_dpp %4, %4, %4 " CTRL " row_mask:0xf bank_mask:0xf\n\t"                        \
                 "v_max_f32_dpp %5, %5, %5 " CTRL " row_mask:0xf bank_mask:0xf"                              \
                 : "+v"(m[0]), "+v"(m[1]), "+v"(m[2]), "+v"(m[3]), "+v"(m[4]), "+v"(m[5]))

template <int CH, int G>
__device__ __forceinline__ float snr_std6(const float (&z)[CH + kSnrWin], const float (&cp)[CH], int g)
{
    static_assert(G == 8 || G == 16, "one DPP row per group");
    float m[6] = {window_max_nv<CH, 1>(z, cp), window_max_nv<CH, 2>(z, cp), window_max_nv<CH, 3>(z, cp),
                  window_max_nv<CH, 4>(z, cp), window_max_nv<CH, 6>(z, cp), window_max_nv<CH, 9>(z, cp)};
// ... 401 lines not shown
        const lds_cptr mx = (lds_cptr)(maxa + (w - 1) * 64 + lane);
        float dm = lds_ld(mx);
#pragma unroll
        for (int k = 1; k < 8; ++k) dm = fmaxf(dm, lds_ld(mx + E * 64 * k));
        const float hpb = whb[2 * iw], b = whb[2 * iw + 1];
        const float v = (hpb * dm - b * sumx) / U.stdnoise;
        const uint32_t o = act ? ((uint32_t)r * nw + (uint32_t)iw) * 4u : 0x80000000u;
        __builtin_amdgcn_raw_buffer_store_b32(__float_as_uint(v), srs, (int)o, 0, kSnrCpol);
    }
}

constexpr int variant_pmin(int smax)
{
    return smax == kPack2 ? 1
                          : (smax <= 5 ? 64 * (smax - 1) + 1
                                       : (smax == 8 ? 321 : (smax == 11 ? 513 : (smax == 16 ? 705 : (smax == 22 ? 1025 : 1409)))));
}
constexpr int variant_pmax(int smax) { return smax == kPack2 ? 32 : 64 * smax; }
constexpr bool variant_has_group(int smax, int G)
{
    return snr_group(variant_pmin(smax)) <= G && G <= snr_group(variant_pmax(smax));
}

constexpr int kSnrShortG = 4;

__device__ __forceinline__ int snr_short_ch(int p)
{
    const int cs = ((p + kSnrShortG - 1) / kSnrShortG) | 1;
    return cs <= 5 ? 5 : (cs <= 9 ? 9 : kSnrMaxChunk);
}

__device__ __forceinline__ int snr_short_stride(int p)
{
    const int cs = ((p + kSnrShortG - 1) / kSnrShortG) | 1;
    const int ch = snr_short_ch(p);
    const int q0 = max(p + max(ch, kSnrWin), (kSnrShortG - 1) * cs + ch);
    return q0 + ((4 - q0) & 7);
}

template <int SMAX, bool WIDE = false>
__device__ __forceinline__ void snr_epilogue(const ConeArgs& a, const UnitView& U, float* data, int q, const int* wl,
                                             int nrows, int tid, float* whb, unsigned long long* tl)
{
    asm volatile("" : "+v"(tid));
    const int lane = tid & 63, wave = tid >> 6;
    const int p = U.p;
    const int nev = (int)min((int64_t)nrows, (int64_t)U.rows_eval - (int64_t)U.s0);
    if (nev <= 0) return;
    int G = 8;
    while (G < 64 && (((p + G - 1) / G) | 1) > kSnrMaxChunk) G <<= 1;
    int c = (p + G - 1) / G;
    if (c < kSnrMaxChunk) c |= 1;
    const uint32_t nw = a.num_widths;
    float* snr = a.snr + (uint64_t)U.trial * a.snr_stride + (U.snr_row + (uint64_t)U.s0) * (uint64_t)nw;
    if constexpr (SMAX == kPack2) {
        constexpr int GS = kSnrShortG;
        const int cs = ((p + GS - 1) / GS) | 1;
        if (cs <= 5) snr_rows<5, GS>(a, U, data, q, wl, nev, cs, tid, whb, tl);
        else if (cs <= 9) snr_rows<9, GS>(a, U, data, q, wl, nev, cs, tid, whb, tl);
        else snr_rows<kSnrMaxChunk, GS>(a, U, data, q, wl, nev, cs, tid, whb, tl);
        return;
    }
    if (c <= kSnrMaxChunk) {
        if constexpr (variant_has_group(SMAX, 8)) {
            if (G == 8) {
                if (c <= 5) snr_rows<5, 8>(a, U, data, q, wl, nev, c, tid, whb, tl);
                else if (c <= 9) snr_rows<9, 8>(a, U, data, q, wl, nev, c, tid, whb, tl);
                else snr_rows<kSnrMaxChunk, 8>(a, U, data, q, wl, nev, c, tid, whb, tl);
                return;
            }
        }
        if constexpr (variant_has_group(SMAX, 16)) {
            if (G == 16) {
                if constexpr (WIDE) {
                    if (snr_wide_ok(p, q, wl[kMaxWidths])) {
                        snr_rows<kSnrMaxChunk, 16, true>(a, U, data, q, wl, nev, c, tid, whb, tl);
                        return;
                    }
                }
                snr_rows<kSnrMaxChunk, 16>(a, U, data, q, wl, nev, c, tid, whb, tl);
                return;
            }
        }
        if constexpr (variant_has_group(SMAX, 32)) {
            if (G == 32) {
                snr_rows<kSnrMaxChunk, 32>(a, U, data, q, wl, nev, c, tid, whb, tl);
                return;
            }
        }
        if constexpr (variant_has_group(SMAX, 64)) snr_rows<kSnrMaxChunk, 64>(a, U, data, q, wl, nev, c, tid, whb, tl);
    } else if (c <= kSnrChunk) {
        if constexpr (variant_has_group(SMAX, 64)) snr_rows<kSnrChunk, 64>(a, U, data, q, wl, nev, c, tid, whb, tl);
    } else if constexpr (variant_pmax(SMAX) > 64 * kSnrChunk) {
        const int g = lane;
        const int j0 = min(g * c, p);
        const int cnt = min(j0 + c, p) - j0;
        const int owner = (p - 1) / c;
        for (int base = 0; base < nev; base += kConeWaves) {
            const int r = base + wave;
            const bool active = r < nev;
            float* row = data + min(r, nev - 1) * q;
            double part = 0.0;
            for (int j = j0; j < j0 + cnt; ++j) part += (double)row[j];
            double incl = part;
            for (int d = 1; d < 64; d <<= 1) {
                const double y = __shfl_up(incl, d, 64);
                if (g >= d) incl += y;
            }
            double acc = __shfl_up(incl, 1, 64);
            if (g == 0) acc = 0.0;
            lds_barrier();
            if (active)
                for (int j = j0; j < j0 + cnt; ++j) {
                    acc += (double)row[j];
                    row[j] = (float)acc;
                }
            const float sum = __shfl((float)acc, owner, 64);
            lds_barrier();
            for (uint32_t iw = 0; iw < nw; ++iw) {
                const int w = uni(wl[iw]);
                float dmax = -INFINITY;
                for (int i = j0; i < j0 + cnt; ++i) {
                    const int k = i + w;
                    const float ck = k < p ? row[k] : __fadd_rn(row[k - p], sum);
                    dmax = fmaxf(dmax, __fsub_rn(ck, row[i]));
                }
                for (int o = 32; o > 0; o >>= 1) dmax = fmaxf(dmax, __shfl_xor(dmax, o, 64));
                if (active && g == 0) {
                    const float h = sqrtf((float)(p - w) / (float)(p * w));
                    const float b = (float)w / (float)(p - w) * h;
                    snr[(uint64_t)r * nw + iw] = ((h + b) * dmax - b * sum) / U.stdnoise;
                }
            }
            lds_barrier();
        }
    }
}

#ifdef RT_STAMPS
#define RT_MARK(i)                                                               \
    do {                                                                         \
        if (tid == 0) tl[i] = __builtin_amdgcn_s_memtime();                      \
    } while (0)
#else
#define RT_MARK(i) do { } while (0)
#endif

#ifdef RT_NO_TRIAL_LOOP
template <int SMAX> constexpr bool kTrialLoop = false;
#else
template <int SMAX> constexpr bool kTrialLoop = SMAX >= 4;
#endif

template <int SMAX, int RWT, bool WIDE, uint32_t SNR>
__global__ __launch_bounds__(kConeBlock, kConeWavesPerSimd) void cone_kernel(ConeArgs a)
{
    constexpr bool FIN = SNR != kSnrNone;
    constexpr bool SEG = SNR == kSnrSeg;
    static_assert(SNR <= kSnrSeg && (!WIDE || SNR == kSnrRows), "S/N kind");
    static_assert(!SEG || (resolved_slots(SMAX) && RWT == 0), "the segmented S/N: 4/5-slot instances");
    constexpr int RW = RWT ? RWT : merge_rows_per_wave(SMAX);
    __shared__ __attribute__((aligned(16))) float data[kLdsBufFloats + kLdsPadFloats];
    __shared__ __attribute__((aligned(16))) uint32_t aux[kAuxWords + kLutPad];
    __shared__ int wl[kMaxWidths + 1];
    __shared__ float whb[2 * kMaxWidths];

    const int tid = threadIdx.x;
#ifdef RT_STAMPS
    unsigned long long t_entry = __builtin_amdgcn_s_memtime();
    unsigned long long r_entry = __builtin_amdgcn_s_memrealtime();
    unsigned long long t_begin[3] = {};
#endif
    const uint32_t tpw = (kTrialLoop<SMAX> && a.trials_per_wg) ? a.trials_per_wg : 1u;
    const uint32_t groups = cone_trial_groups(a.batch, tpw);
    const uint32_t total = a.num_items * groups;
    if (blockIdx.x >= total) return;
    const uint32_t item = blockIdx.x / groups;
    const uint32_t t0 = (blockIdx.x - item * groups) * tpw;
    const int tn = (int)min(tpw, a.batch - t0);
    if (tid < (int)a.num_widths) wl[tid] = (int)a.widths[tid];
    if (tid == 0) {
        uint32_t wm = 0;
        for (uint32_t i = 0; i < a.num_widths; ++i) wm = max(wm, a.widths[i]);
        wl[kMaxWidths] = (int)wm;
    }
    const bool dma = !(a.flags & kConeDiagNoLand);
    bool ok;
#ifdef RT_STAMPS
    UnitCtx C = unit_begin<SMAX, RW>(a, item, t0, aux, data, tid, dma, ok, t_begin);
    unsigned long long tl[kStampMarks] = {};
    tl[0] = __builtin_amdgcn_s_memtime();
#else
    UnitCtx C = unit_begin<SMAX, RW>(a, item, t0, aux, data, tid, dma, ok);
#endif
    const UnitView& U = C.U;
    const int p = U.p;
    const int L = U.levels;
    float* const buf = data;
    {
        const uint32_t ukind = U.dst == kSelSnrSeg ? ((a.flags & kConeSnrSeg) ? kSnrSeg : kSnrRows)
                                                   : (U.dst == kSelSnr ? kSnrRows : kSnrNone);
        ok = ok && ukind == SNR;
    }
    if (FIN && tid < (int)a.num_widths) snr_width_consts(wl[tid], p, whb + 2 * tid);
    if constexpr (SMAX == 4)
        if (C.slots && ok) build_roll_lut4(aux + kLut4Off, p, tid);
    if constexpr (resolved_slots(SMAX))
        if (ok && U.zero_row)
            for (int j = tid; j < 64 * SMAX; j += kConeBlock) data[U.zero_row + j] = -0.0f;
    if constexpr (SMAX == kPack2)
        if (ok && p >= kPackSeg) build_pack_lut(aux, p, tid);
    __builtin_amdgcn_s_waitcnt(0x0F70);
    lds_barrier();
    RT_MARK(1);
    RT_MARK(2);
    if constexpr (SEG)
        ok = ok && C.slots && snr_seg_unit(SMAX, L, p, wl[kMaxWidths], rows_at(C, 0));
    if (!ok) {
        if (tid == 0 && a.error_flag) atomicOr(a.error_flag, 1);
        return;
    }
    constexpr bool st = !FIN;
    const bool st_regs = st && (a.flags & kConeStoreFromRegs);
    const uint32_t o0 = (uint32_t)(U.node_start + U.s0) * (uint32_t)p * 4u;
    const int n0 = rows_at(C, 0);
    int qout = SEG ? kSnrSegStride : p;
    bool blob_clobbered = SMAX == kPack2 && FIN;
    if constexpr (SMAX == kPack2) {
        if (L > 0) qout = pack_stride(p);
        if (FIN && L > 0 && p >= kPackSeg && (a.flags & kConeSnrStride)) {
            const int qf = snr_short_stride(p);
            if (n0 * qf <= kLdsDataFloats) qout = qf;
            if (qout == qf && n0 * qf + U.run_off <= kLdsBufFloats) blob_clobbered = false;
        }
    }
    if constexpr (SMAX <= 5 && SMAX != kPack2 && !SEG) {
        const int qa = p + kSnrMaxChunk + ((16 - ((p + kSnrMaxChunk) & 31)) & 31);
        const int qb = p + kSnrWin + ((16 - ((p + kSnrWin) & 31)) & 31);
        if (!st && L > 0 && C.slots && (a.flags & kConeFuse2) && (a.flags & kConeSnrStride)) {
            qout = n0 * qa <= kLdsDataFloats ? qa : (n0 * qb <= kLdsDataFloats ? qb : p);
            const int wmax = wl[kMaxWidths];
            if (WIDE && snr_group(p) == 16 && wmax > kSnrWin && wmax < p) {
                const int qw = snr_wide_stride(p, wmax);
                const int qwp = qw + ((16 - (qw & 31)) & 31);
                if (n0 * qwp <= kLdsDataFloats) qout = qwp;
                else if (n0 * qw <= kLdsDataFloats) qout = qw;
            }
        }
    }
    for (int k = 0;;) {
        const int trial = C.U.trial;
        const float* dst = (U.dst == kSelPing ? a.ping : a.pong) + (uint64_t)trial * a.buf_stride + U.buf_off;
        const __amdgpu_buffer_rsrc_t rs = buffer_rsrc(dst, (((uint32_t)U.m * (uint32_t)p + 3u) & ~3u) * 4u);
        const bool more = k + 1 < tn;
        bool next_issued = false;
        auto fill_next = [&]() {
            if (more) {
                lds_barrier();
                if (dma) unit_fill<SMAX>(a, C, trial + 1, buf, tid, blob_clobbered);
            }
            next_issued = true;
        };
        if (L > 0 && !(a.flags & kConeDiagNoMerge))
            merge_levels<SMAX, RW>(C, buf, p, L, tid, st_regs, rs, o0, a.flags, buf + kLdsBufFloats + 4 + (tid & 63),
                                   qout, SEG ? 8 * kSnrSegCols - p : 0, fill_next);
        RT_MARK(3);
        float* const obase = L > 0 ? buf : buf + (C.table ? uni(bottom_offsets(C)[0]) : C.al);
        if (st) {
            if (L == 0 || !st_regs) {
                const int qst = L > 0 ? qout : p;
                for (int r = 0; r < n0; ++r)
                    for (int j = tid; j < p; j += kConeBlock)
                        __builtin_amdgcn_raw_buffer_store_b32(__float_as_uint(obase[r * qst + j]), rs,
                                                              (int)(o0 + (uint32_t)(r * p + j) * 4u), 0, kStoreCpol);
            }
        } else if constexpr (SEG) {
            if (!(a.flags & kConeDiagNoSnr)) snr_segments<SMAX>(a, C.U, buf, wl, n0, tid, whb);
        } else if constexpr (FIN) {
#ifdef RT_STAMPS
            if (!(a.flags & kConeDiagNoSnr)) snr_epilogue<SMAX, WIDE>(a, C.U, obase, qout, wl, n0, tid, whb, tl);
#else
            if (!(a.flags & kConeDiagNoSnr)) snr_epilogue<SMAX, WIDE>(a, C.U, obase, qout, wl, n0, tid, whb, nullptr);
#endif
        }
#ifdef RT_STAMPS
        lds_barrier();
        RT_MARK(4);
        tl[5] = t_entry;
        tl[11] = t_begin[0];
        tl[12] = t_begin[1];
        tl[13] = t_begin[2];
        RT_MARK(6);
        tl[14] = r_entry;
        tl[15] = __builtin_amdgcn_s_memrealtime();
        if (tid == 0 && a.stamps) {
            unsigned long long* e = a.stamps + (uint64_t)kStampRecWords * ((uint64_t)item * a.batch + (uint32_t)trial);
            const uint32_t hw = (uint32_t)__builtin_amdgcn_s_getreg(4 | (31 << 11));
            const uint32_t xcc = (uint32_t)__builtin_amdgcn_s_getreg(20 | (31 << 11));
            e[0] = (unsigned long long)hw | ((unsigned long long)xcc << 32);
#pragma unroll
            for (int i = 0; i < kStampMarks; ++i) e[1 + i] = tl[i];
            e[1 + kStampMarks] = (unsigned long long)p | ((unsigned long long)L << 16) |
                                 ((unsigned long long)U.mode << 24) | ((unsigned long long)rows_at(C, 0) << 32) |
                                 ((unsigned long long)is_snr_dst(U.dst) << 48);
        }
#endif
        if (!kTrialLoop<SMAX> || !more) break;
        if (!next_issued) fill_next();
        if constexpr (resolved_slots(SMAX) && FIN)
            if (U.zero_row)
                for (int j = tid; j < 64 * SMAX; j += kConeBlock) data[U.zero_row + j] = -0.0f;
        ++k;
        C.U.trial = trial + 1;
#ifdef RT_STAMPS
        t_entry = __builtin_amdgcn_s_memtime();
        r_entry = __builtin_amdgcn_s_memrealtime();
        t_begin[0] = t_begin[1] = t_begin[2] = t_entry;
        tl[0] = t_entry;
#endif
        __builtin_amdgcn_s_waitcnt(0x0F70);
        lds_barrier();
        RT_MARK(1);
        RT_MARK(2);
    }
}

template <int SMAX, int RW = 0>
static hipError_t launch_kind(const ConeArgs& args, dim3 g, dim3 b, bool wide_snr, uint32_t snr, hipStream_t s)
{
    if (snr == kSnrNone) {
        if (wide_snr) return hipErrorInvalidValue;
        hipLaunchKernelGGL((cone_kernel<SMAX, RW, false, kSnrNone>), g, b, 0, s, args);
    } else if (snr == kSnrSeg) {
        if (wide_snr || !resolved_slots(SMAX) || RW != 0) return hipErrorInvalidValue;
        if constexpr (resolved_slots(SMAX) && RW == 0) hipLaunchKernelGGL((cone_kernel<SMAX, 0, false, kSnrSeg>), g, b, 0, s, args);
    } else if (snr != kSnrRows) {
        return hipErrorInvalidValue;
    } else if (wide_snr && SMAX >= 3 && SMAX <= 5 && RW == 0) {
        if constexpr (SMAX >= 3 && SMAX <= 5 && RW == 0) hipLaunchKernelGGL((cone_kernel<SMAX, 0, true, kSnrRows>), g, b, 0, s, args);
    } else {
        hipLaunchKernelGGL((cone_kernel<SMAX, RW, false, kSnrRows>), g, b, 0, s, args);
    }
    return hipSuccess;
}

hipError_t launch_cone(const ConeArgs& args_in, uint32_t smax, uint32_t rw, bool wide_snr, uint32_t snr, hipStream_t s)
{
    if (!args_in.num_items || !args_in.batch) return hipSuccess;
    ConeArgs args = args_in;
    if (snr == kSnrSeg && !(args.flags & kConeSnrSeg)) snr = kSnrRows;
#ifdef RT_NO_TRIAL_LOOP
    args.trials_per_wg = 1;
#else
    if (smax < 4) args.trials_per_wg = 1;
#endif
    const uint64_t total = (uint64_t)args.num_items * cone_trial_groups(args.batch, args.trials_per_wg);
    if (total > 0xFFFFFFFFull) return hipErrorInvalidValue;
    const dim3 g((uint32_t)total), b(kConeBlock);
    hipError_t e = hipErrorInvalidValue;
    if (rw != 0) return hipErrorInvalidValue;
    switch (smax) {
    case 1: e = launch_kind<1>(args, g, b, wide_snr, snr, s); break;
    case 2: e = launch_kind<2>(args, g, b, wide_snr, snr, s); break;
    case 3: e = launch_kind<3>(args, g, b, wide_snr, snr, s); break;
    case 4: e = launch_kind<4>(args, g, b, wide_snr, snr, s); break;
    case 5: e = launch_kind<5>(args, g, b, wide_snr, snr, s); break;
    case 8: e = launch_kind<8>(args, g, b, wide_snr, snr, s); break;
    case 11: e = launch_kind<11>(args, g, b, wide_snr, snr, s); break;
    case 16: e = launch_kind<16>(args, g, b, wide_snr, snr, s); break;
    case 22: e = launch_kind<22>(args, g, b, wide_snr, snr, s); break;
    case kMaxSlots: e = launch_kind<kMaxSlots>(args, g, b, wide_snr, snr, s); break;
    case kPack2: e = launch_kind<kPack2>(args, g, b, wide_snr, snr, s); break;
    default: return hipErrorInvalidValue;
    }
    if (e != hipSuccess) return e;
    return hipGetLastError();
}

}

namespace rt {

__global__ __launch_bounds__(256) void ffa_level_kernel(const float* __restrict__ in, float* __restrict__ out,
                                                        const uint2* __restrict__ nodes, uint32_t num_nodes,
                                                        uint32_t p)
{
    const uint32_t u = blockIdx.x;
    uint32_t lo = 0, hi = num_nodes - 1;
    while (lo < hi) {
        const uint32_t mid = (lo + hi + 1) >> 1;
        if (nodes[mid].x <= u) lo = mid; else hi = mid - 1;
    }
    const uint2 nd = nodes[lo];
    const float* hrow;
    const float* trow = nullptr;
    uint32_t shift = 0;
    if (nd.y <= 1) {
        hrow = in + (uint64_t)u * p;
    } else {
        const uint32_t s = u - nd.x, sh = nd.y >> 1, st = nd.y - sh;
        const uint32_t h = merge_index(merge_coef(sh, nd.y), s);
        const uint32_t t = merge_index(merge_coef(st, nd.y), s);
        hrow = in + (uint64_t)(nd.x + h) * p;
        trow = in + (uint64_t)(nd.x + sh + t) * p;
        shift = (s - t) % p;
    }
    float* o = out + (uint64_t)u * p;
    for (uint32_t j = threadIdx.x; j < p; j += 256) {
        float v = hrow[j];
        if (trow) {
            uint32_t c = j + shift;
            if (c >= p) c -= p;
            v = __fadd_rn(v, trow[c]);
        }
        o[j] = v;
    }
}

hipError_t launch_ffa_level(const float* in, float* out, const uint2* d_nodes, uint32_t num_nodes,
                            uint32_t rows, uint32_t p, hipStream_t s)
{
    hipLaunchKernelGGL(ffa_level_kernel, dim3(rows), dim3(256), 0, s, in, out, d_nodes, num_nodes, p);
    return hipGetLastError();
}

}
```

### riptide_amd/csrc/host_api.cpp

```cpp
#include "riptide_amd.h"

#include <algorithm>
#include <stdexcept>

#include "capi_common.hpp"
#include "peaks_host.hpp"
#include "plan.hpp"

using namespace rt;

namespace {

PgramPlan pgram_plan(size_t size, double tsamp, double pmin, double pmax, size_t bmin, size_t bmax)
{
    PgramPlan pg;
    build_pgram_plan(checked_params(size, tsamp, pmin, pmax, bmin, bmax), pg);
    return pg;
}

HostPlan host_plan(size_t size, double tsamp, size_t nw, uint32_t wmax, double pmin, double pmax, size_t bmin,
                   size_t bmax)
{
    HostPlan hp;
    plan_periodogram(checked_params(size, tsamp, pmin, pmax, bmin, bmax), (uint32_t)nw, wmax, scratch_budget_floats(),
                     cosched_banks(), hp);
    return hp;
}

}

extern "C" {

const char* rt_last_error(void) { return last_error().c_str(); }

int rt_periodogram_length(size_t size, double tsamp, double pmin, double pmax, size_t bmin, size_t bmax,
                          size_t* length)
{
    return guarded([&] {
        *length = pgram_plan(size, tsamp, pmin, pmax, bmin, bmax).length;
        return RT_OK;
    });
}

int rt_periodogram_grid(size_t size, double tsamp, double pmin, double pmax, size_t bmin, size_t bmax,
                        double* periods, uint32_t* foldbins)
{
    return guarded([&] {
        fill_grid(pgram_plan(size, tsamp, pmin, pmax, bmin, bmax), periods, foldbins);
        return RT_OK;
    });
}

int rt_ffa_schedule_check(size_t rows, size_t cols, uint64_t* launches)
{
    return guarded([&] {
        if (!rows || !cols || rows > 0xFFFFFFFFull || cols > 0xFFFFFFFFull || !merge_slots((uint32_t)cols))
            throw std::invalid_argument("rt_ffa_schedule_check: bad shape");
        FfaXform X{};
        X.p = (uint32_t)cols;
        X.m = (uint32_t)rows;
        X.rows_eval = (uint32_t)rows;
        ExecPlan ex;
        build_exec_plan({X}, false, 0, ~0ull, ex);
        if (launches) *launches = ex.launches.size();
        return RT_OK;
    });
}

int rt_ladder_check(size_t size, double tsamp, double pmin, double pmax, size_t bmin, size_t bmax, int* fused,
                    uint64_t* rungs)
{
    return guarded([&] {
        const LadderPlan l = plan_ladder(pgram_plan(size, tsamp, pmin, pmax, bmin, bmax));
        if (fused) *fused = l.mode;
        if (rungs) *rungs = l.rungs.size();
        return RT_OK;
    });
}

int rt_ladder_layout(size_t size, double tsamp, double pmin, double pmax, size_t bmin, size_t bmax,
                     rt_ladder_rung* rungs, size_t cap, uint64_t* count, uint64_t* leaf_floats, int* mode,
                     uint32_t* margin)
{
    return guarded([&] {
        const PgramPlan pg = pgram_plan(size, tsamp, pmin, pmax, bmin, bmax);
        if (cap && !rungs) throw std::invalid_argument("rt_ladder_layout: rungs is NULL");
        const LadderPlan l = plan_ladder(pg);
        for (size_t i = 0; i < l.rungs.size() && i < cap; ++i) {
            const DsRung& d = l.rungs[i];
            rt_ladder_rung o{};
            o.f = d.f;
            o.n = d.n;
            o.leaf_off = d.out_off;
            o.fused = rung_in_fused(l.mode, d);
            rungs[i] = o;
        }
        if (count) *count = l.rungs.size();
        if (leaf_floats) *leaf_floats = pg.leaf_floats;
        if (mode) *mode = l.mode;
        if (margin) *margin = l.margin;
        return RT_OK;
    });
}

int rt_schedule_check(size_t size, double tsamp, size_t nw, double pmin, double pmax, size_t bmin, size_t bmax,
                      uint64_t* transforms, uint64_t* items, uint64_t* launches, double* alg_bytes,
                      double* moved_bytes, uint64_t* cells)
{
    return guarded([&] {
        const ExecTotals t = exec_totals(host_plan(size, tsamp, nw, 0, pmin, pmax, bmin, bmax).ex);
        *transforms = t.transforms;
        *items = t.items;
        *launches = t.launches;
        *alg_bytes = t.alg_bytes;
        *moved_bytes = t.moved_bytes;
        *cells = t.cells;
        return RT_OK;
    });
}

int rt_schedule_final_kinds(size_t size, double tsamp, const uint64_t* widths, size_t nw, double pmin, double pmax,
                            size_t bmin, size_t bmax, uint64_t* launches, uint64_t* rows_launches,
                            uint64_t* seg_launches, uint8_t* bins_kinds, size_t bins_cap)
{
    return guarded([&] {
        const uint32_t wmax = checked_plan_widths(widths, nw, bmin);
        const ExecPlan ex = host_plan(size, tsamp, nw, wmax, pmin, pmax, bmin, bmax).ex;
        uint64_t nr = 0, ns = 0;
        if (bins_kinds) std::fill(bins_kinds, bins_kinds + bins_cap, (uint8_t)0);
        for (const Launch& L : ex.launches) {
            if (L.snr == kSnrNone) continue;
            ++(L.snr == kSnrSeg ? ns : nr);
            if (!bins_kinds) continue;
            for (uint32_t i = L.first; i < L.first + L.count; ++i) {
                const uint32_t p = ex.xf[ex.items[i].xform].p;
                if (p < bins_cap) bins_kinds[p] |= (uint8_t)(L.snr == kSnrSeg ? 2 : 1);
            }
        }
        if (launches) *launches = ex.launches.size();
        if (rows_launches) *rows_launches = nr;
        if (seg_launches) *seg_launches = ns;
        return RT_OK;
    });
}

int rt_find_peaks_workspace_bytes(size_t batch, size_t length, size_t num_widths, size_t chunk_rows, size_t* bytes)
{
    return guarded([&] {
        *bytes = checked_peak_workspace(batch, length, num_widths, chunk_rows);
        return RT_OK;
    });
}

int rt_find_peaks_host(const float* snrs, size_t length, size_t num_widths, const double* logf, const double* freqs,
                       const double* coeffs, size_t ncoef, double smin, double radius, uint32_t* counts,
                       uint32_t* rows, float* snr, size_t cap)
{
    return guarded([&] {
        if (!cap) throw std::invalid_argument("rt_find_peaks_host: cap is 0");
        if (!ncoef || ncoef > 64) throw std::invalid_argument("rt_find_peaks_host: 1 to 64 polynomial coefficients");
        if (length >= (1ull << 32)) throw std::invalid_argument("rt_find_peaks_host: length must be below 2^32");
        for (size_t iw = 0; iw < num_widths; ++iw)
            counts[iw] = find_peaks_column(snrs + iw, num_widths, length, logf, freqs, coeffs + iw * ncoef,
                                           (uint32_t)ncoef, smin, radius, rows + iw * cap, snr + iw * cap, cap);
        return RT_OK;
    });
}

}
```

### riptide_amd/csrc/plan.cpp

```cpp
#include "plan.hpp"

#include <algorithm>
#include <cstdlib>
#include <cmath>
#include <stdexcept>
#include <string>

namespace rt {

std::string check_pgram_args(const PgramParams& a)
{
    if (!(a.tsamp > 0)) return "tsamp must be > 0";
    if (!(a.pmin > 0)) return "period_min must be > 0";
    if (!(a.pmax > a.pmin)) return "period_max must be > period_min";
    if (!(a.bmin > 1)) return "bins_min must be > 1";
    if (!(a.bmax >= a.bmin)) return "bins_max must be >= bins_min";
    if (!(a.pmin >= a.tsamp * (double)a.bmin)) return "Must have: period_min >= tsamp * bins_min ";
    return "";
}

size_t downsampled_size(size_t n, double f)
{
    return (size_t)std::floor((double)n / f);
}
// ... 88 lines not shown
            nxt.push_back({n.start + h, n.size - h});
        }
        out.swap(nxt);
    }
}

ConeNeed cone_need(uint32_t node_size, uint32_t s0, uint32_t s1, int levels, uint32_t p)
{
    struct R { uint32_t size, lo, hi; };
    std::vector<R> cur{{node_size, s0, s1 - 1}}, nxt;
    ConeNeed need;
    auto account = [&](const std::vector<R>& lv) {
        int rows = 0;
        for (const R& r : lv) rows += (int)(r.hi - r.lo + 1);
        need.entries += need.rows_bottom;
        need.rows_bottom = rows;
        need.runs_bottom = (int)lv.size();
        need.max_rows = std::max(need.max_rows, rows);
        need.max_floats = std::max(need.max_floats, rows * (int)p);
        need.ranges += (int)lv.size();
    };
    account(cur);
    for (int l = 0; l < levels; ++l) {
        nxt.clear();
        for (const R& r : cur) {
            if (r.size <= 1) {
                need.degenerate = true;
                nxt.push_back(r);
                continue;
            }
            const uint32_t sh = r.size >> 1, st = r.size - sh;
            const float kh = merge_coef(sh, r.size), kt = merge_coef(st, r.size);
            nxt.push_back({sh, merge_index(kh, r.lo), merge_index(kh, r.hi)});
            nxt.push_back({st, merge_index(kt, r.lo), merge_index(kt, r.hi)});
        }
        cur.swap(nxt);
        account(cur);
    }
    return need;
}

static bool fits(const ConeNeed& n, uint32_t p, int smax)
{
    if (n.degenerate || n.max_rows > lds_row_capacity(p, smax) || n.ranges > kMaxRanges) return false;
    const int fill = 4 * fill_chunks_bound(n.rows_bottom, (int)p, n.runs_bottom);
    if (smax == kPack2)
        return std::max(fill, n.max_rows * pack_stride((int)p)) + pack_blob_words(n.entries, n.rows_bottom) <=
               kLdsBufFloats;
    return n.max_floats <= kLdsDataFloats && fill <= kLdsBufFloats && n.entries <= kDescEntries;
}

struct PassItems { std::vector<ConeItem> items; double read = 0, written = 0; };

static double pass_weight()
{
    if (const char* e = std::getenv("RIPTIDE_AMD_PASS_WEIGHT")) {
        const double v = std::atof(e);
        if (v >= 0) return v;
    }
    return 100.0;
}

static void plan_transform(const FfaXform& X, uint32_t xi, int smax, uint32_t final_kmax, std::vector<PassItems>& passes)
{
    passes.clear();
    const uint32_t m = X.m, p = X.p;
    const int C = lds_row_capacity(p, smax);
    if (C < 3) throw std::invalid_argument("phase bins too large for the LDS cone kernel");
    int db = 0;
    while (((uint64_t)m + (1ull << db) - 1) >> db > (uint64_t)C) ++db;
    std::vector<Node> nodes;
    nodes_at_depth(m, db, nodes);
    PassItems bottom;
    for (const Node& n : nodes) {
        ConeItem it{};
        it.xform = xi;
        it.node_start = n.start;
        it.node_size = n.size;
        it.s0 = 0;
        it.s1 = n.size;
        it.levels = (uint8_t)ceil_log2(n.size);
        it.mode = kModeWhole;
        bottom.items.push_back(it);
        bottom.read += 4.0 * n.size * p;
        bottom.written += 4.0 * n.size * p;
    }
    passes.push_back(std::move(bottom));
    if (db == 0) return;

    int bestL = 1;
    double best = 1e300;
    for (int L = 1; L <= kMaxTileLevels; ++L) {
        const int extra = 2 << L;
        if (extra + 1 >= C) break;
        const int npass = (db + L - 1) / L;
        const double cost = npass * ((double)C / (double)(C - extra) + pass_weight());
        if (cost < best - 1e-9) { best = cost; bestL = L; }
    }
    const int npass = (db + bestL - 1) / bestL;
    std::vector<int> lv(npass, db / npass);
    for (int i = 0; i < db % npass; ++i) lv[i] += 1;
    int depth_below = db;
    for (int k = 0; k < npass; ++k) {
        const int L = lv[k];
        const int dtop = depth_below - L;
        nodes_at_depth(m, dtop, nodes);
        PassItems pass;
        const int guess = std::max(1, C - (2 << L) - 2);
        const uint32_t kmax = k == npass - 1 && final_kmax ? final_kmax : ~0u;
        for (const Node& n : nodes) {
            uint32_t s0 = 0;
            while (s0 < n.size) {
                uint32_t K = std::min<uint32_t>(std::min<uint32_t>((uint32_t)guess, kmax), n.size - s0);
                ConeNeed need = cone_need(n.size, s0, s0 + K, L, p);
                while (K > 1 && !fits(need, p, smax)) {
                    K -= std::max<uint32_t>(1, K / 32);
                    need = cone_need(n.size, s0, s0 + K, L, p);
                }
                if (!fits(need, p, smax)) throw std::invalid_argument("cone tile does not fit in LDS");
                while (s0 + K < n.size && K < kmax) {
                    ConeNeed nn = cone_need(n.size, s0, s0 + K + 1, L, p);
                    if (!fits(nn, p, smax)) break;
                    need = nn;
                    ++K;
                }
                ConeItem it{};
                it.xform = xi;
                it.node_start = n.start;
                it.node_size = n.size;
                it.s0 = s0;
                it.s1 = s0 + K;
                it.levels = (uint8_t)L;
                it.mode = kModeTile;
                pass.items.push_back(it);
                pass.read += 4.0 * need.max_rows * p;
                pass.written += 4.0 * K * p;
                s0 += K;
            }
        }
        passes.push_back(std::move(pass));
        depth_below = dtop;
    }
}

static double item_cost(const ConeItem& it, const FfaXform& X)
{
    const double rows = it.mode == kModeTile ? (double)(it.s1 - it.s0) + (double)(2u << it.levels)
                                             : (double)it.node_size;
    return rows * (double)X.p * ((double)it.levels + 2.0);
}

static bool wide_snr(const FfaXform& X, int smax, bool snr_epilogue, uint32_t max_width)
{
    if (!snr_epilogue || smax > 5 || smax == kPack2) return false;
    if (snr_group((int)X.p) != 16 || (int)max_width <= kSnrWin || max_width >= X.p) return false;
    if (const char* e = std::getenv("RIPTIDE_AMD_SNR_WIDE"))
        if (e[0] == '0') return false;
    return true;
}

static bool seg_snr(const FfaXform& X, int smax, bool snr_epilogue, uint32_t max_width)
{
    if (!snr_epilogue || (smax != 4 && smax != 5)) return false;
    if (!snr_seg_ok((int)X.p, (int)max_width, 1)) return false;
    if (const char* e = std::getenv("RIPTIDE_AMD_CONE_FLAGS"))
        if (!(std::strtoul(e, nullptr, 0) & kConeSnrSeg)) return false;
    return true;
}

static uint32_t final_snr_kind(const FfaXform& X, int smax, uint32_t max_width, const std::vector<ConeItem>& items)
{
    if (!seg_snr(X, smax, true, max_width)) return kSnrRows;
    for (const ConeItem& it : items) {
        const int rows = it.mode == kModeTile ? (int)(it.s1 - it.s0) : (int)it.node_size;
        if (!snr_seg_unit(smax, it.levels, (int)X.p, (int)max_width, rows)) return kSnrRows;
    }
    return kSnrSeg;
}

static uint32_t final_tile_cap(const FfaXform& X, int smax, bool snr_epilogue, uint32_t max_width)
{
    if (seg_snr(X, smax, snr_epilogue, max_width)) return kSnrSegRows;
    if (!wide_snr(X, smax, snr_epilogue, max_width)) return 0;
    const int q = snr_wide_stride((int)X.p, (int)max_width);
    const int k = kLdsDataFloats / q;
    return k >= 8 ? (uint32_t)k : 0;
}

void build_exec_plan(const std::vector<FfaXform>& xforms, bool snr_epilogue, uint32_t num_widths,
                     uint64_t scratch_budget, ExecPlan& out, uint32_t max_width, uint32_t banks)
{
    if (banks != 1 && banks != 2) throw std::invalid_argument("scratch banks: 1 or 2");
    out = ExecPlan();
    out.xf = xforms;
    out.max_width = max_width;
    for (const FfaXform& X : xforms) {
        if (!merge_slots(X.p)) throw std::invalid_argument("phase bins too large for the LDS cone kernel");
        if ((uint64_t)X.m * X.p * 4u >= kMaxBlockBytes)
            throw std::invalid_argument("FFA transform block of " + std::to_string(X.m) + " x " + std::to_string(X.p) +
                                        " floats exceeds the 2 GiB range of the cone kernel");
    }
    const size_t nx = xforms.size();
    std::vector<uint32_t> xgroup(nx, 0);
    size_t g0 = 0;
    uint32_t group = 0;
    std::vector<std::vector<PassItems>> sched;
    while (g0 < nx) {
        uint64_t scratch = 0;
        size_t g1 = g0;
        while (g1 < nx) {
            const uint64_t cells = ((uint64_t)xforms[g1].m * xforms[g1].p + 3) & ~(uint64_t)3;
            if (g1 > g0 && scratch + cells > scratch_budget) break;
            out.xf[g1].buf_off = scratch;
            xgroup[g1] = group;
            scratch += cells;
            ++g1;
        }
        out.scratch_floats = std::max(out.scratch_floats, scratch);
        sched.assign(g1 - g0, {});
        uint32_t gpasses = 0;
        for (size_t i = g0; i < g1; ++i) {
            plan_transform(out.xf[i], (uint32_t)i, merge_slots(out.xf[i].p),
                           final_tile_cap(out.xf[i], merge_slots(out.xf[i].p), snr_epilogue, max_width), sched[i - g0]);
            gpasses = std::max<uint32_t>(gpasses, (uint32_t)sched[i - g0].size());
        }
        out.max_passes = std::max(out.max_passes, gpasses);
        const size_t first_launch = out.launches.size();
        std::vector<int> buckets;
        for (size_t i = g0; i < g1; ++i) buckets.push_back(merge_slots(out.xf[i].p));
        std::sort(buckets.begin(), buckets.end());
        buckets.erase(std::unique(buckets.begin(), buckets.end()), buckets.end());
        for (uint32_t k = 0; k < gpasses; ++k) {
            for (const int bucket : buckets) for (uint32_t kind = kSnrNone; kind <= kSnrSeg; ++kind) {
                Launch L;
                L.snr = kind;
                L.smax = (uint32_t)bucket;
                L.first = (uint32_t)out.items.size();
                L.group = group;
                L.pass = k;
                for (size_t i = g0; i < g1; ++i) {
                    auto& sp = sched[i - g0];
                    const uint32_t P = (uint32_t)sp.size();
                    if (k >= P || merge_slots(out.xf[i].p) != bucket) continue;
                    const FfaXform& X = out.xf[i];
                    const uint8_t src = k == 0 ? kSelLeaves : (((P - k) % 2 == 0) ? kSelPing : kSelPong);
                    const bool last = (k == P - 1);
                    const uint32_t xkind =
                        (last && snr_epilogue) ? final_snr_kind(X, bucket, max_width, sp[k].items) : (uint32_t)kSnrNone;
                    if (xkind != kind) continue;
                    const uint8_t dst = last ? (snr_epilogue ? (kind == kSnrSeg ? kSelSnrSeg : kSelSnr) : kSelPing)
                                             : (((P - 1 - k) % 2 == 0) ? kSelPing : kSelPong);
                    for (ConeItem it : sp[k].items) {
                        it.src = src;
                        it.dst = dst;
                        out.items.push_back(it);
                    }
                    const double cells = (double)X.m * X.p;
                    if (last && wide_snr(X, bucket, snr_epilogue, max_width)) L.wide_snr = 1;
                    L.cells += (uint64_t)X.m * X.p;
                    L.alg_bytes += 4.0 * cells + ((last && snr_epilogue) ? 4.0 * X.rows_eval * num_widths : 4.0 * cells);
                    L.moved_bytes += sp[k].read + ((last && snr_epilogue) ? 4.0 * X.rows_eval * num_widths : sp[k].written);
                }
                L.count = (uint32_t)out.items.size() - L.first;
                std::stable_sort(out.items.begin() + L.first, out.items.end(),
                                 [&](const ConeItem& x, const ConeItem& y) {
                                     return item_cost(x, out.xf[x.xform]) > item_cost(y, out.xf[y.xform]);
                                 });
                if (!L.count) continue;
                out.launches.push_back(L);
            }
        }
        std::stable_partition(out.launches.begin() + first_launch, out.launches.end(),
                              [](const Launch& L) { return L.snr == 0; });
        g0 = g1;
        ++group;
    }
    out.groups = group;
    out.bank_floats = out.scratch_floats;
    out.banks = group > 1 ? banks : 1;
    if (out.banks == 2) {
        for (size_t i = 0; i < nx; ++i)
            if (xgroup[i] & 1u) out.xf[i].buf_off += out.bank_floats;
        out.scratch_floats = 2 * out.bank_floats;
    }
    std::vector<int> slot_rw(out.items.size(), 0);
    std::vector<bool> packed(out.items.size(), false);
    std::vector<int> smax_of(out.items.size(), 0);
    for (const Launch& L : out.launches) {
        const int rw = L.smax <= 5 ? (L.rw ? (int)L.rw : merge_rows_per_wave((int)L.smax)) : 0;
        for (uint32_t i = L.first; i < L.first + L.count; ++i) {
            slot_rw[i] = rw;
            packed[i] = L.smax == (uint32_t)kPack2;
            smax_of[i] = (int)L.smax;
        }
    }
    for (size_t i = 0; i < out.items.size(); ++i) {
        ConeItem& it = out.items[i];
        it.pad = kNoBlob;
        if (!packed[i] && it.mode != kModeTile &&
            ((uint64_t)it.levels * it.node_size > (uint64_t)kDescEntries || it.node_size > (uint32_t)kMaxRows))
            continue;
        it.pad = (uint32_t)out.blob.size();
        build_tile_blob(it, out.xf[it.xform].p, slot_rw[i], smax_of[i], out.blob);
    }
    validate_exec_plan(out, snr_epilogue);
}

static void build_row_slots(const uint32_t* d, uint32_t n, uint32_t p, int rw, std::vector<uint32_t>& slots)
{
    struct Item { uint32_t r; uint32_t kind; };
    std::vector<Item> items;
    for (uint32_t r = 0; r < n;) {
        const uint32_t a = d[r];
        const bool carried = ((a >> 10) & 1023u) == kCarriedRow;
        if (r + 1 < n && ((a ^ d[r + 1]) & 0xFFFFFu) == 0 && !carried && (d[r + 1] >> 20) == ((a >> 20) + 1) % p) {
            items.push_back({r, kSlotPair});
            r += 2;
        } else if (r + 1 < n && ((a ^ d[r + 1]) & 1023u) == 0 && !carried &&
                   ((d[r + 1] >> 10) & 1023u) != kCarriedRow) {
            items.push_back({r, kSlotHalf});
            r += 2;
        } else {
            items.push_back({r, kSlotOne});
            r += 1;
        }
    }
    const int Q = (rw + 1) / 2;
    slots.clear();
    size_t c = 0;
    for (int g = 0; c < items.size(); ++g) {
        if (g >= kConeWaves * Q) throw std::runtime_error("schedule: merge level exceeds the register rows");
        const int cap = (g / kConeWaves == Q - 1 && (rw & 1)) ? 1 : 2;
        Item& A = items[c];
        if (A.kind != kSlotOne && cap == 2) {
            slots.push_back(A.r | ((A.r + 1) << 10) | (A.kind << 20));
            ++c;
            continue;
        }
        const uint32_t ra = A.r;
        if (A.kind != kSlotOne) {
            A.r += 1;
            A.kind = kSlotOne;
        } else {
            ++c;
        }
        if (cap == 1 || c == items.size()) {
            slots.push_back(ra | (kSlotOne << 20));
            continue;
        }
        Item& B = items[c];
        const uint32_t rb = B.r;
        if (B.kind != kSlotOne) {
            B.r += 1;
            B.kind = kSlotOne;
        } else {
            ++c;
        }
        slots.push_back(ra | (rb << 10) | (kSlotTwo << 20));
    }
}

void build_tile_blob(const ConeItem& it, uint32_t p, int slot_rw, int smax, std::vector<uint32_t>& out)
{
    const bool packed = smax == kPack2;
    const bool resolved = slot_rw > 0 && resolved_slots(smax);
    struct R { uint32_t size, lo, hi; uint32_t start; uint32_t base; };
    const int L = it.levels;
    const bool tile = it.mode == kModeTile;
    std::vector<std::vector<R>> lv(L + 1);
    lv[0].push_back({it.node_size, it.s0, it.s1 - 1, it.node_start, 0});
    for (int l = 1; l <= L; ++l) {
        if (!tile) {
            lv[l].push_back(lv[0][0]);
            continue;
        }
        for (const R& r : lv[l - 1]) {
            const uint32_t sh = r.size >> 1, st = r.size - sh;
            const float kh = merge_coef(sh, r.size), kt = merge_coef(st, r.size);
            lv[l].push_back({sh, merge_index(kh, r.lo), merge_index(kh, r.hi), r.start, 0});
            lv[l].push_back({st, merge_index(kt, r.lo), merge_index(kt, r.hi), r.start + sh, 0});
        }
    }
    uint32_t nrows[kMaxLevels + 1] = {}, doff[kMaxLevels + 1] = {};
    uint32_t entries = 0;
    for (int l = 0; l <= L; ++l) {
        uint32_t b = 0;
        for (R& r : lv[l]) {
            r.base = b;
            b += r.hi - r.lo + 1;
        }
        nrows[l] = b;
        doff[l] = entries;
        if (l < L) entries += b;
    }
    const size_t o = out.size();
    const uint32_t nruns = (uint32_t)lv[L].size(), nb = nrows[L];
    std::vector<uint32_t> desc_v(entries);
    uint32_t* desc = desc_v.data();
    for (int l = 0; l < L; ++l) {
        if (!tile) {
            for (uint32_t r = 0; r < nrows[l]; ++r) {
                uint32_t a0 = 0, sz = it.node_size;
                for (int d = 0; d < l; ++d)
                    if (sz > 1) {
                        const uint32_t hs = sz >> 1;
                        if (r - a0 < hs) sz = hs;
                        else {
                            a0 += hs;
                            sz -= hs;
                        }
                    }
                uint32_t word;
                if (sz <= 1) {
                    word = r | (kCarriedRow << 10);
                } else {
                    const uint32_t s = r - a0, hs = sz >> 1, ts = sz - hs;
                    const uint32_t hh = merge_index(merge_coef(hs, sz), s);
                    const uint32_t tt = merge_index(merge_coef(ts, sz), s);
                    word = (a0 + hh) | ((a0 + hs + tt) << 10) | (((s - tt) % p) << 20);
                }
                desc[doff[l] + r] = word;
            }
            continue;
        }
        size_t j = 0;
        for (uint32_t r = 0; r < nrows[l]; ++r) {
            while (j + 1 < lv[l].size() && lv[l][j + 1].base <= r) ++j;
            const R& g = lv[l][j];
            const uint32_t u = g.lo + (r - g.base);
            const R& H = lv[l + 1][2 * j];
            const R& T = lv[l + 1][2 * j + 1];
            const uint32_t hs = g.size >> 1, ts = g.size - hs;
            const uint32_t hh = merge_index(merge_coef(hs, g.size), u);
            const uint32_t tt = merge_index(merge_coef(ts, g.size), u);
            const uint32_t h = H.base + hh - H.lo, t = T.base + tt - T.lo;
            const uint32_t sh = (u - tt) % p;
            desc[doff[l] + r] = h | (t << 10) | (sh << 20);
        }
    }
    std::vector<uint32_t> loff_v(nb), segs;
    uint32_t cb = 0;
    for (uint32_t ri = 0; ri < nruns; ++ri) {
        const R& g = lv[L][ri];
        const uint32_t first = (g.start + g.lo) * p;
        const uint32_t al = first & 3u, cnt = g.hi - g.lo + 1;
        const uint32_t nch = (cnt * p + al + 3) >> 2;
        for (uint32_t r = 0; r < cnt; ++r) loff_v[g.base + r] = 4 * cb + al + r * p;
        for (uint32_t c = 0; c < nch; c += 64) {
            segs.push_back(cb + c);
            segs.push_back(std::min<uint32_t>(64u, nch - c));
            segs.push_back((first - al) / 4 + c);
            segs.push_back(0u);
        }
        cb += nch;
    }
    std::vector<uint32_t> slot_area;
    uint32_t slot_off[kMaxLevels + 1] = {};
    uint32_t zero_row = 0;
    if (packed) {
        std::vector<bool> keep(L + 1, false), fused(L + 1, false);
        std::vector<uint32_t> rel(L + 1, 0);
        for (int l = L - 1; l >= 0;) {
            const bool two = l >= 1 && (tile || (it.node_size >> l) >= 2);
            const int lo = two ? l - 1 : l;
            if (!two) {
                keep[lo] = true;
            } else {
                fused[lo] = true;
                rel[lo] = (uint32_t)slot_area.size();
                for (uint32_t r = 0; r < nrows[lo]; ++r) {
                    const uint32_t d0 = desc[doff[lo] + r];
                    const uint32_t dh = desc[doff[lo + 1] + (d0 & 1023u)];
                    const uint32_t dt = desc[doff[lo + 1] + ((d0 >> 10) & 1023u)];
                    const uint32_t sh = d0 >> 20, sH = dh >> 20, sTT = ((d0 >> 20) + (dt >> 20)) % p;
                    slot_area.push_back((dh & 1023u) | (((dh >> 10) & 1023u) << 10) | ((dt & 1023u) << 20));
                    slot_area.push_back(((dt >> 10) & 1023u) | (sH << 10) | (sh << 16) | (sTT << 22));
                }
            }
            l = lo - 1;
        }
        std::vector<uint32_t> dc;
        for (int l = 0; l < L; ++l) {
            const uint32_t o0 = doff[l];
            doff[l] = (uint32_t)dc.size();
            if (keep[l]) dc.insert(dc.end(), desc_v.begin() + o0, desc_v.begin() + o0 + nrows[l]);
        }
        desc_v.swap(dc);
        desc = desc_v.data();
        entries = (uint32_t)desc_v.size();
        const uint32_t base0 = kBlobHeader + entries + nb;
        if (base0 & 1u) slot_area.insert(slot_area.begin(), 0u);
        const uint32_t base = base0 + (base0 & 1u);
        for (int l = 0; l <= L; ++l)
            if (fused[l]) slot_off[l] = base + rel[l];
    } else if (resolved) {
        if (!tile && L >= 2 && (L % 2) == 0 && 4 * cb + 64 * (uint32_t)smax <= (uint32_t)kLdsDataFloats) zero_row = 4 * cb;
        std::vector<uint32_t> sl;
        const uint32_t base0 = kBlobHeader + nb;
        const uint32_t base = (base0 + 3u) & ~3u;
        slot_area.assign(base - base0, 0u);
        for (int l = L - 1; l >= 0;) {
            const bool two = l >= 1 && (tile || zero_row || (it.node_size >> l) >= 2);
            const int lo = two ? l - 1 : l;
            const bool first = l == L - 1;
            build_row_slots(desc + doff[lo], nrows[lo], p, slot_rw, sl);
            slot_off[lo] = (uint32_t)(base0 + slot_area.size());
            slot_area.insert(slot_area.end(), {(uint32_t)sl.size(), 0u, 0u, 0u});
            auto off = [&](uint32_t row) { return first ? loff_v[row] : row * p; };
            auto entry = [&](uint32_t r, uint32_t* e) {
                const uint32_t d0 = desc[doff[lo] + r];
                if (two) {
                    const uint32_t dh = desc[doff[lo + 1] + (d0 & 1023u)];
                    const uint32_t dt = desc[doff[lo + 1] + ((d0 >> 10) & 1023u)];
                    const bool ch = ((dh >> 10) & 1023u) == kCarriedRow, ct = ((dt >> 10) & 1023u) == kCarriedRow;
                    if ((ch || ct) && !(zero_row && first))
                        throw std::runtime_error("schedule: fused step over carried nodes without a zero row");
                    const uint32_t sh = d0 >> 20, sH = ch ? 0u : dh >> 20;
                    const uint32_t sTT = ((d0 >> 20) + (ct ? 0u : dt >> 20)) % p;
                    e[0] = off(dh & 1023u) | ((ch ? zero_row : off((dh >> 10) & 1023u)) << 16);
                    e[1] = off(dt & 1023u) | ((ct ? zero_row : off((dt >> 10) & 1023u)) << 16);
                    e[2] = sH | (sh << 10) | (sTT << 20);
                } else {
                    const uint32_t tc = (d0 >> 10) & 1023u, car = tc == kCarriedRow;
                    const uint32_t oh = off(d0 & 1023u);
                    e[0] = oh | ((car ? oh : off(tc)) << 16);
                    e[1] = 0u;
                    e[2] = (d0 >> 20) | (car << 30);
                }
            };
            const int Q = (slot_rw + 1) / 2;
            const size_t t0 = slot_area.size();
            slot_area.resize(t0 + 4 * 2 * (size_t)kConeWaves * Q, 0u);
            for (size_t g = 0; g < sl.size(); ++g) {
                const uint32_t sw = sl[g];
                const size_t wq = (g % kConeWaves) * Q + g / kConeWaves;
                uint32_t* ea = slot_area.data() + t0 + 4 * wq;
                uint32_t* eb = slot_area.data() + t0 + 4 * ((size_t)kConeWaves * Q + wq);
                entry(sw & 1023u, ea);
                ea[3] = sw;
                if ((sw >> 20) == kSlotTwo || (sw >> 20) == kSlotHalf) entry((sw >> 10) & 1023u, eb);
            }
            l = lo - 1;
        }
        if (slot_area.size() > (size_t)(kAuxMetaWords - kBlobHeader - nb))
            throw std::runtime_error("schedule: resolved row-slot tables exceed their LDS area");
        entries = 0;
        for (int l = 0; l <= L; ++l) doff[l] = 0;
    } else if (slot_rw > 0) {
        std::vector<uint32_t> sl;
        for (int l = L - 1; l >= 0;) {
            const bool two = l >= 1 && (tile || (it.node_size >> l) >= 2);
            const int lo = two ? l - 1 : l;
            build_row_slots(desc + doff[lo], nrows[lo], p, slot_rw, sl);
            slot_off[lo] = (uint32_t)(kBlobHeader + entries + nb + slot_area.size());
            slot_area.push_back((uint32_t)sl.size());
            slot_area.insert(slot_area.end(), sl.begin(), sl.end());
            l = lo - 1;
        }
        if (slot_area.size() > (size_t)kSlotWords) throw std::runtime_error("schedule: row-slot tables exceed their LDS area");
    }
    const uint32_t nsegs = (uint32_t)(segs.size() / 4);
    {
        const uint32_t K = (nsegs + kConeWaves - 1) / kConeWaves;
        std::vector<uint32_t> wm((size_t)4 * K * kConeWaves, 0u);
        for (uint32_t g = 0; g < nsegs; ++g)
            std::copy(segs.begin() + 4 * g, segs.begin() + 4 * g + 4, wm.begin() + 4 * ((g % kConeWaves) * K + g / kConeWaves));
        segs.swap(wm);
    }
    if (nsegs > (uint32_t)(kConeWaves * 64)) throw std::runtime_error("schedule: unit fill exceeds the DMA segment table");
    const size_t lds_words = kBlobHeader + entries + nb + slot_area.size();
    const size_t runoff = (lds_words + 3) & ~(size_t)3;
    const size_t words = runoff + segs.size();
    out.resize(o + ((words + 3) & ~(size_t)3), 0u);
    uint32_t* w = out.data() + o;
    for (int l = 0; l <= L; ++l) {
        w[kHdrRows + l] = nrows[l];
        w[kHdrDesc + l] = doff[l];
        w[kHdrSlotOff + l] = slot_off[l];
    }
    w[kHdrRuns] = nsegs;
    w[kHdrEntries] = entries;
    w[kHdrBottom] = nb;
    w[kHdrSlotWords] = (uint32_t)slot_area.size();
    w[kHdrRunOff] = (uint32_t)runoff;
    w[kHdrFill] = cb;
    w[kHdrZero] = zero_row;
    if (entries) std::copy(desc_v.begin(), desc_v.begin() + entries, w + kBlobHeader);
    std::copy(loff_v.begin(), loff_v.end(), w + kBlobHeader + entries);
    std::copy(slot_area.begin(), slot_area.end(), w + kBlobHeader + entries + nb);
    std::copy(segs.begin(), segs.end(), w + runoff);
}

constexpr int kMaxSteps4 = 4;
constexpr int kBlobLds4Worst =
    kBlobHeader + kConeWaves * kRw4 + 3 + kMaxSteps4 * (4 + 4 * 2 * kConeWaves * ((kRw4 + 1) / 2));
static_assert(kBlobLds4Worst <= kLut4Off, "4-slot unit blobs may overlap the roll table");
static_assert((kMaxTileLevels + 1) / 2 <= kMaxSteps4, "tile steps");

static void validate_blob(const ConeItem& it, uint32_t p, int smax, int rw, const uint32_t* w)
{
    const uint32_t L = it.levels;
    const uint32_t nseg = w[kHdrRuns], entries = w[kHdrEntries], nb = w[kHdrBottom];
    const uint32_t slot_words = w[kHdrSlotWords], runoff = w[kHdrRunOff], fill = w[kHdrFill];
    if (runoff < (uint32_t)kBlobHeader + entries + nb + slot_words || (runoff & 3u) || nb != w[kHdrRows + L])
        throw std::runtime_error("schedule: malformed unit blob header");
    if (4 * fill > (uint32_t)kLdsBufFloats) throw std::runtime_error("schedule: unit fill exceeds the LDS level buffer");
    if (smax == 4 && slot_words && runoff > (uint32_t)kLut4Off)
        throw std::runtime_error("schedule: unit blob overlaps the roll table");
    uint32_t c = 0;
    const uint32_t K = (nseg + kConeWaves - 1) / kConeWaves;
    for (uint32_t i = 0; i < nseg; ++i) {
        const uint32_t* g = w + runoff + 4 * ((i % kConeWaves) * K + i / kConeWaves);
        if (g[0] != c || g[1] == 0 || g[1] > 64) throw std::runtime_error("schedule: DMA segments do not tile the fill");
        c += g[1];
    }
    if (c != fill) throw std::runtime_error("schedule: DMA segments do not tile the fill");
    const uint32_t* desc = w + kBlobHeader;
    if (smax != kPack2 && !(resolved_slots(smax) && slot_words))
        for (uint32_t l = 0; l < L; ++l)
            if (w[kHdrDesc + l] + w[kHdrRows + l] > entries) throw std::runtime_error("schedule: descriptor table overrun");
    const bool tile = it.mode == kModeTile;
    if (smax == kPack2) {
        for (int l = (int)L - 1; l >= 0;) {
            const bool two = l >= 1 && (tile || (it.node_size >> l) >= 2);
            const int lo = two ? l - 1 : l;
            if (two) {
                const uint32_t so = w[kHdrSlotOff + lo], n = w[kHdrRows + lo], nsrc = w[kHdrRows + lo + 2];
                if (!so || (so & 1u) || so + 2 * n > runoff) throw std::runtime_error("schedule: step table outside the blob");
                for (uint32_t r = 0; r < n; ++r) {
                    const uint32_t a = w[so + 2 * r], b = w[so + 2 * r + 1];
                    const uint32_t s1 = (b >> 10) & 63u, s2 = (b >> 16) & 63u, s3 = (b >> 22) & 63u;
                    if ((a & 1023u) >= nsrc || ((a >> 10) & 1023u) >= nsrc || ((a >> 20) & 1023u) >= nsrc ||
                        (b & 1023u) >= nsrc || s1 >= p || s2 >= p || s3 >= p)
                        throw std::runtime_error("schedule: bad step table entry");
                }
            } else if (w[kHdrDesc + lo] + w[kHdrRows + lo] > entries) {
                throw std::runtime_error("schedule: descriptor table overrun");
            }
            l = lo - 1;
        }
        return;
    }
    if (!slot_words) {
        if (smax <= 5 && L > 0) throw std::runtime_error("schedule: unit without row-slot tables");
        return;
    }
    if (resolved_slots(smax)) {
        const int Q = (rw + 1) / 2;
        const uint32_t zero_row = w[kHdrZero];
        if (zero_row && (tile || (L % 2) || zero_row < 4 * fill || zero_row + 64 * (uint32_t)smax > (uint32_t)kLdsDataFloats))
            throw std::runtime_error("schedule: bad zero row");
        for (int l = (int)L - 1; l >= 0;) {
            const bool two = l >= 1 && (tile || zero_row || (it.node_size >> l) >= 2);
            const int lo = two ? l - 1 : l;
            const uint32_t n = w[kHdrRows + lo], so = w[kHdrSlotOff + lo];
            if ((so & 3u) || so < (uint32_t)kBlobHeader + nb || so + 4 > runoff)
                throw std::runtime_error("schedule: row-slot table outside the blob");
            const uint32_t ns = w[so];
            if (ns > (uint32_t)(kConeWaves * Q) || so + 4 + 8 * (uint32_t)(kConeWaves * Q) > runoff)
                throw std::runtime_error("schedule: row-slot table overrun");
            std::vector<uint8_t> seen(n, 0);
            auto check_entry = [&](const uint32_t* e) {
                const uint32_t s1 = e[2] & 1023u, s2 = (e[2] >> 10) & 1023u, s3 = (e[2] >> 20) & 1023u;
                const uint32_t top = (uint32_t)kLdsBufFloats;
                if (s1 >= p || (two && (s2 >= p || s3 >= p)) || (e[0] & 0xFFFFu) + p > top ||
                    (e[0] >> 16) + p > top || (two && ((e[1] & 0xFFFFu) + p > top || (e[1] >> 16) + p > top)))
                    throw std::runtime_error("schedule: bad resolved row entry");
            };
            for (uint32_t g = 0; g < ns; ++g) {
                const uint32_t wq = (g % kConeWaves) * (uint32_t)Q + g / kConeWaves;
                const uint32_t* e = w + so + 4 + 4 * wq;
                const uint32_t* eb = w + so + 4 + 4 * ((uint32_t)(kConeWaves * Q) + wq);
                const uint32_t sw = e[3], ra = sw & 1023u, rb = (sw >> 10) & 1023u, kind = sw >> 20;
                const int q = (int)g / kConeWaves;
                const bool two_rows = kind != kSlotOne;
                if (kind > kSlotHalf || ra >= n || (two_rows && (rb >= n || 2 * q + 1 >= rw)) ||
                    ((kind == kSlotPair || kind == kSlotHalf) && rb != ra + 1))
                    throw std::runtime_error("schedule: bad row slot");
                if (seen[ra]++ || (two_rows && seen[rb]++)) throw std::runtime_error("schedule: row slot covers a row twice");
                check_entry(e);
                if (kind == kSlotTwo || kind == kSlotHalf) check_entry(eb);
                if (kind == kSlotHalf &&
                    ((two ? (e[0] != eb[0] || (e[2] & 1023u) != (eb[2] & 1023u))
                          : ((e[0] & 0xFFFFu) != (eb[0] & 0xFFFFu))) ||
                     (!two && (((e[2] >> 30) & 1u) || ((eb[2] >> 30) & 1u)))))
                    throw std::runtime_error("schedule: row half without a shared head term");
            }
            for (uint32_t r = 0; r < n; ++r)
                if (!seen[r]) throw std::runtime_error("schedule: row-slot table misses a row");
            l = lo - 1;
        }
        return;
    }
    const int Q = (rw + 1) / 2;
    for (int l = (int)L - 1; l >= 0;) {
        const bool two = l >= 1 && (tile || (it.node_size >> l) >= 2);
        const int lo = two ? l - 1 : l;
        const uint32_t n = w[kHdrRows + lo], so = w[kHdrSlotOff + lo];
        if (so < (uint32_t)kBlobHeader + entries + nb || so >= runoff) throw std::runtime_error("schedule: row-slot table outside the blob");
        const uint32_t ns = w[so];
        if (ns > (uint32_t)(kConeWaves * Q) || so + 1 + ns > runoff) throw std::runtime_error("schedule: row-slot table overrun");
        std::vector<uint8_t> seen(n, 0);
        const uint32_t* d = desc + w[kHdrDesc + lo];
        for (uint32_t g = 0; g < ns; ++g) {
            const uint32_t sw = w[so + 1 + g], ra = sw & 1023u, rb = (sw >> 10) & 1023u, kind = sw >> 20;
            const int q = (int)g / kConeWaves;
            const bool two_rows = kind != kSlotOne;
            if (kind > kSlotHalf || ra >= n || (two_rows && (rb >= n || 2 * q + 1 >= rw)))
                throw std::runtime_error("schedule: bad row slot");
            if (seen[ra]++ || (two_rows && seen[rb]++)) throw std::runtime_error("schedule: row slot covers a row twice");
            if (kind == kSlotHalf) {
                const uint32_t a = d[ra], b = d[rb];
                if (rb != ra + 1 || ((a ^ b) & 1023u) || ((a >> 10) & 1023u) == kCarriedRow ||
                    ((b >> 10) & 1023u) == kCarriedRow)
                    throw std::runtime_error("schedule: row half without a shared head row");
            }
            if (kind == kSlotPair) {
                const uint32_t a = d[ra], b = d[rb];
                if (rb != ra + 1 || ((a ^ b) & 0xFFFFFu) || ((a >> 10) & 1023u) == kCarriedRow ||
                    (b >> 20) != ((a >> 20) + 1) % p)
                    throw std::runtime_error("schedule: row pair without shared head/tail rows");
            }
        }
        for (uint32_t r = 0; r < n; ++r)
            if (!seen[r]) throw std::runtime_error("schedule: row-slot table misses a row");
        l = lo - 1;
    }
}

void validate_exec_plan(const ExecPlan& ex, bool snr_epilogue)
{
    std::vector<uint64_t> covered(ex.xf.size(), 0);
    std::vector<uint32_t> last_pass(ex.xf.size(), 0);
    for (const Launch& L : ex.launches)
        for (uint32_t i = L.first; i < L.first + L.count; ++i)
            last_pass[ex.items[i].xform] = std::max(last_pass[ex.items[i].xform], L.pass);
    for (const FfaXform& X : ex.xf) {
        if ((uint64_t)X.m * X.p * 4u >= kMaxBlockBytes) throw std::runtime_error("schedule: transform block over 2 GiB");
        if (X.buf_off + (((uint64_t)X.m * X.p + 3) & ~(uint64_t)3) > ex.scratch_floats)
            throw std::runtime_error("schedule: transform scratch outside the ping/pong buffers");
    }
    for (const Launch& L : ex.launches) {
        if (L.first + L.count > ex.items.size()) throw std::runtime_error("schedule: launch outside the item list");
        for (uint32_t i = L.first; i < L.first + L.count; ++i) {
            const ConeItem& it = ex.items[i];
            if (it.xform >= ex.xf.size()) throw std::runtime_error("schedule: item of an unknown transform");
            const FfaXform& X = ex.xf[it.xform];
            if (merge_slots(X.p) != (int)L.smax) throw std::runtime_error("schedule: item in the wrong kernel variant");
            if (it.s1 <= it.s0 || it.s1 > it.node_size || (uint64_t)it.node_start + it.node_size > X.m)
                throw std::runtime_error("schedule: tile outside its node");
            int rows;
            if (it.mode == kModeTile) {
                const ConeNeed n = cone_need(it.node_size, it.s0, it.s1, it.levels, X.p);
                if (n.degenerate || n.max_rows > kMaxRows || n.max_floats > kLdsDataFloats || n.ranges > kMaxRanges ||
                    it.levels > kMaxTileLevels)
                    throw std::runtime_error("schedule: tile exceeds the LDS budget");
                rows = n.max_rows;
            } else {
                if ((int)it.node_size * (int)X.p > kLdsDataFloats || it.node_size > (uint32_t)kMaxRows ||
                    it.levels > kMaxLevels || (1u << it.levels) < it.node_size)
                    throw std::runtime_error("schedule: whole node exceeds the LDS budget");
                rows = (int)it.node_size;
            }
            const ConeNeed need = it.mode == kModeTile ? cone_need(it.node_size, it.s0, it.s1, it.levels, X.p)
                                                       : ConeNeed{};
            const int bottom = it.mode == kModeTile ? need.rows_bottom : (int)it.node_size;
            if (4 * fill_chunks_bound(bottom, (int)X.p, it.mode == kModeTile ? 1 << it.levels : 1) > kLdsBufFloats)
                throw std::runtime_error("schedule: unit fill exceeds the LDS level buffer");
            if (L.smax == (uint32_t)kPack2) {
                if (it.pad == kNoBlob) throw std::runtime_error("schedule: short-row unit without a descriptor table");
                const uint32_t* h = ex.blob.data() + it.pad;
                const int top = std::max<int>(4 * (int)h[kHdrFill], rows * pack_stride((int)X.p));
                if (top + (int)h[kHdrRunOff] > kLdsBufFloats)
                    throw std::runtime_error("schedule: short-row unit and its descriptor table exceed the level buffer");
            } else if (it.mode == kModeTile && (need.entries > kDescEntries || it.pad == kNoBlob)) {
                throw std::runtime_error("schedule: tile descriptor table exceeds its LDS area");
            }
            if (resolved_slots((int)L.smax) && it.levels > 0 &&
                (it.pad == kNoBlob || ex.blob[it.pad + kHdrSlotWords] == 0))
                throw std::runtime_error("schedule: 4/5-slot unit without row-slot tables");
            const uint32_t ukind = it.dst == kSelSnrSeg ? kSnrSeg : (it.dst == kSelSnr ? kSnrRows : kSnrNone);
            if (L.snr > kSnrSeg || ukind != L.snr) throw std::runtime_error("schedule: unit in a launch of the other kind");
            if (L.wide_snr && L.snr != kSnrRows) throw std::runtime_error("schedule: wide S/N on a launch without the row-group S/N");
            if (ukind == kSnrSeg &&
                !snr_seg_unit((int)L.smax, it.levels, (int)X.p, (int)ex.max_width,
                              it.mode == kModeTile ? (int)(it.s1 - it.s0) : (int)it.node_size))
                throw std::runtime_error("schedule: segmented S/N on a unit outside its shapes");
            const int rw = L.rw ? (int)L.rw : merge_rows_per_wave((int)L.smax);
            if (it.pad != kNoBlob) {
                if ((size_t)it.pad + kBlobHeader > ex.blob.size()) throw std::runtime_error("schedule: blob outside the plan");
                validate_blob(it, X.p, (int)L.smax, rw, ex.blob.data() + it.pad);
            }
            if (rows > kConeWaves * rw * row_pack((int)L.smax) || rows > lds_row_capacity(X.p, (int)L.smax))
                throw std::runtime_error("schedule: unit rows exceed its kernel instance's register rows");
            if (L.pass == last_pass[it.xform]) {
                if (it.node_start != 0 || snr_epilogue != is_snr_dst(it.dst))
                    throw std::runtime_error("schedule: bad final pass");
                covered[it.xform] += it.s1 - it.s0;
            }
        }
    }
    for (size_t t = 0; t < ex.xf.size(); ++t)
        if (covered[t] != ex.xf[t].m) throw std::runtime_error("schedule: final pass does not cover the transform");
}

ExecTotals exec_totals(const ExecPlan& ex)
{
    ExecTotals t;
    t.transforms = ex.xf.size();
    t.items = ex.items.size();
    t.launches = ex.launches.size();
    for (const Launch& L : ex.launches) {
        t.alg_bytes += L.alg_bytes;
        t.moved_bytes += L.moved_bytes;
        if (L.pass == 0) t.cells += L.cells;
    }
    return t;
}

bool rung_fusable(const DsRung& d) { return d.identity || std::ceil(d.f) + 2.0 <= (double)kDsFusedMargin; }

bool rung_in_fused(int mode, const DsRung& d)
{
    return mode == kLadderFused || (mode == kLadderHybrid && rung_fusable(d));
}

int ladder_split(size_t size, const std::vector<DsRung>& rungs, std::vector<DsRung>* f, std::vector<DsRung>* w)
{
    if ((uint64_t)size >= kDsFusedMaxSize) return kLadderPerRung;
    std::vector<DsRung> a, b;
    uint32_t blocks = 0;
    for (const DsRung& d : rungs) {
        if (rung_fusable(d)) {
            a.push_back(d);
        } else {
            DsRung e = d;
            e.first_block = blocks;
            blocks += (uint32_t)((e.n + e.per_block - 1) / e.per_block);
            b.push_back(e);
        }
    }
    if (a.empty() || a.size() > kDsMaxRungs || ds_fused_margin(a.data(), a.size()) == 0) return kLadderPerRung;
    if (f) *f = a;
    if (w) *w = b;
    return b.empty() ? kLadderFused : kLadderHybrid;
}

std::vector<DsRung> used_rungs(const PgramPlan& pg)
{
    std::vector<bool> used(pg.rungs.size(), false);
    for (const Step& s : pg.steps)
        if (s.rows_eval) used[s.rung] = true;
    std::vector<DsRung> out;
    uint32_t blocks = 0;
    for (size_t r = 0; r < pg.rungs.size(); ++r) {
        if (!used[r]) continue;
        const Rung& R = pg.rungs[r];
        DsRung d{};
        d.f = R.f;
        d.n = R.n;
        d.out_off = R.leaf_off;
        d.first_block = blocks;
        d.identity = R.f == 1.0;
        ds_configure(d);
        blocks += (uint32_t)((R.n + d.per_block - 1) / d.per_block);
        out.push_back(d);
    }
    return out;
}

LadderPlan plan_ladder(const PgramPlan& pg)
{
    LadderPlan l;
    l.rungs = used_rungs(pg);
    l.mode = ladder_split(pg.prm.size, l.rungs, &l.rungs_f, &l.rungs_w);
    if (l.mode != kLadderPerRung) l.margin = ds_fused_margin(l.rungs_f.data(), l.rungs_f.size());
    return l;
}

std::vector<FfaXform> pgram_xforms(const PgramPlan& pg)
{
    std::vector<FfaXform> xf;
    for (const Step& s : pg.steps) {
        if (!s.rows_eval) continue;
        FfaXform X{};
        X.p = s.bins;
        X.m = s.rows;
        X.rows_eval = s.rows_eval;
        X.rung = s.rung;
        X.src_off = pg.rungs[s.rung].leaf_off;
        X.snr_row = s.out_row;
        X.stdnoise = s.stdnoise;
        xf.push_back(X);
    }
    return xf;
}

PgramParams checked_params(size_t size, double tsamp, double pmin, double pmax, size_t bmin, size_t bmax)
{
    PgramParams prm;
    prm.size = size;
// ... 50 lines not shown
```

### riptide_amd/csrc/plan.hpp

```cpp
#pragma once
#include <string>
#include <vector>

#include "common.hpp"

namespace rt {

struct PgramParams {
    size_t size = 0;
    double tsamp = 0, pmin = 0, pmax = 0;
    size_t bmin = 0, bmax = 0;
};

std::string check_pgram_args(const PgramParams& a);

size_t downsampled_size(size_t n, double f);
double downsampled_variance(size_t n, double f);

struct Rung {
    double f = 0, tau = 0;
    size_t n = 0;
    uint64_t leaf_off = 0;
};

struct Step {
    uint32_t rung = 0, bins = 0, rows = 0, rows_eval = 0;
    float stdnoise = 0;
    uint64_t out_row = 0;
};

struct PgramPlan {
    PgramParams prm;
    std::vector<Rung> rungs;
    std::vector<Step> steps;
    uint64_t length = 0;
    uint64_t leaf_floats = 0;
};

void build_pgram_plan(const PgramParams& a, PgramPlan& plan);

void fill_grid(const PgramPlan& plan, double* periods, uint32_t* foldbins);

struct Launch {
    uint32_t first = 0, count = 0;
    uint32_t group = 0, pass = 0;
    uint32_t smax = 0;
    uint32_t rw = 0;
    uint32_t wide_snr = 0;
    uint32_t snr = 0;
    double alg_bytes = 0;
    double moved_bytes = 0;
    uint64_t cells = 0;
};

struct ExecPlan {
    std::vector<FfaXform> xf;
    std::vector<ConeItem> items;
    std::vector<Launch> launches;
    std::vector<uint32_t> blob;
    uint64_t scratch_floats = 0;
    uint32_t max_passes = 0;
    uint32_t max_width = 0;
    uint32_t banks = 1;
    uint64_t bank_floats = 0;
    uint32_t groups = 0;
};

void build_tile_blob(const ConeItem& it, uint32_t p, int slot_rw, int smax, std::vector<uint32_t>& out);

void build_exec_plan(const std::vector<FfaXform>& xforms, bool snr_epilogue, uint32_t num_widths,
                     uint64_t scratch_budget, ExecPlan& out, uint32_t max_width = 0, uint32_t banks = 1);

void validate_exec_plan(const ExecPlan& ex, bool snr_epilogue);

constexpr uint64_t kMaxBlockBytes = 1ull << 31;

struct ConeNeed { int max_rows = 0; int max_floats = 0; int ranges = 0; int rows_bottom = 0; int runs_bottom = 0; int entries = 0; bool degenerate = false; };
ConeNeed cone_need(uint32_t node_size, uint32_t s0, uint32_t s1, int levels, uint32_t p);

struct ExecTotals {
    uint64_t transforms = 0, items = 0, launches = 0, cells = 0;
    double alg_bytes = 0, moved_bytes = 0;
};
ExecTotals exec_totals(const ExecPlan& ex);

constexpr uint64_t kDsFusedMaxSize = 1ull << 29;
constexpr int kLadderPerRung = 0, kLadderFused = 1, kLadderHybrid = 2;

bool rung_fusable(const DsRung& d);
bool rung_in_fused(int mode, const DsRung& d);

int ladder_split(size_t size, const std::vector<DsRung>& rungs, std::vector<DsRung>* f, std::vector<DsRung>* w);

std::vector<DsRung> used_rungs(const PgramPlan& pg);

struct LadderPlan {
    std::vector<DsRung> rungs, rungs_f, rungs_w;
    int mode = kLadderPerRung;
    uint32_t margin = 0;
};
LadderPlan plan_ladder(const PgramPlan& pg);

std::vector<FfaXform> pgram_xforms(const PgramPlan& pg);

PgramParams checked_params(size_t size, double tsamp, double pmin, double pmax, size_t bmin, size_t bmax);

void check_widths(const uint64_t* w, size_t nw, size_t bins);
uint32_t checked_plan_widths(const uint64_t* w, size_t nw, size_t bmin);

uint64_t scratch_budget_floats();
uint32_t cosched_banks();

struct HostPlan {
    PgramPlan pg;
    ExecPlan ex;
    LadderPlan ladder;
};
void plan_periodogram(const PgramParams& prm, uint32_t num_widths, uint32_t max_width, uint64_t scratch_budget,
                      uint32_t banks, HostPlan& out);

}
```

### riptide_amd/csrc/sched_check_main.cpp

```cpp
#include <cstdio>
#include <cstdlib>
#include <cstring>
#include <vector>

#include "riptide_amd.h"

int main(int argc, char** argv)
{
    if (argc >= 9 && !std::strcmp(argv[1], "pgram")) {
        const size_t n = std::strtoull(argv[2], nullptr, 10);
        const double tsamp = std::atof(argv[3]), pmin = std::atof(argv[4]), pmax = std::atof(argv[5]);
        const size_t bmin = std::strtoull(argv[6], nullptr, 10), bmax = std::strtoull(argv[7], nullptr, 10);
        const size_t nw = std::strtoull(argv[8], nullptr, 10);
        size_t L = 0;
        if (rt_periodogram_length(n, tsamp, pmin, pmax, bmin, bmax, &L)) {
            std::printf("length: %s\n", rt_last_error());
            return 1;
        }
        std::vector<double> periods(L);
        std::vector<uint32_t> foldbins(L);
        if (rt_periodogram_grid(n, tsamp, pmin, pmax, bmin, bmax, periods.data(), foldbins.data())) {
            std::printf("grid: %s\n", rt_last_error());
            return 1;
        }
        uint64_t xf = 0, items = 0, launches = 0, cells = 0;
        double alg = 0, moved = 0;
        if (rt_schedule_check(n, tsamp, nw, pmin, pmax, bmin, bmax, &xf, &items, &launches, &alg, &moved, &cells)) {
            std::printf("schedule: %s\n", rt_last_error());
            return 1;
        }
        int fused = -1;
        uint64_t rungs = 0;
        if (rt_ladder_check(n, tsamp, pmin, pmax, bmin, bmax, &fused, &rungs)) {
            std::printf("ladder: %s\n", rt_last_error());
            return 1;
        }
        uint64_t nr = 0, leaf = 0;
        int mode = -1;
        uint32_t margin = 0;
        if (rt_ladder_layout(n, tsamp, pmin, pmax, bmin, bmax, nullptr, 0, &nr, nullptr, nullptr, nullptr)) {
            std::printf("ladder layout: %s\n", rt_last_error());
            return 1;
        }
        std::vector<rt_ladder_rung> lr(nr);
        if (rt_ladder_layout(n, tsamp, pmin, pmax, bmin, bmax, lr.data(), lr.size(), &nr, &leaf, &mode, &margin) ||
            nr != rungs || mode != fused) {
            std::printf("ladder layout: %s\n", rt_last_error());
            return 1;
        }
        for (const rt_ladder_rung& r : lr)
            if (r.leaf_off + r.n > leaf) {
                std::printf("ladder layout: a rung ends past the leaf buffer\n");
                return 1;
            }
        std::printf("pgram L=%zu transforms=%llu items=%llu launches=%llu alg=%.6e moved=%.6e fused=%d rungs=%llu\n", L,
                    (unsigned long long)xf, (unsigned long long)items, (unsigned long long)launches, alg, moved, fused,
                    (unsigned long long)rungs);
        return 0;
    }
    if (argc >= 9 && !std::strcmp(argv[1], "kinds")) {
        const size_t n = std::strtoull(argv[2], nullptr, 10);
        const double tsamp = std::atof(argv[3]), pmin = std::atof(argv[4]), pmax = std::atof(argv[5]);
        const size_t bmin = std::strtoull(argv[6], nullptr, 10), bmax = std::strtoull(argv[7], nullptr, 10);
        std::vector<uint64_t> widths;
        for (int i = 8; i < argc; ++i) widths.push_back(std::strtoull(argv[i], nullptr, 10));
        uint64_t launches = 0, nrows = 0, nseg = 0;
        std::vector<uint8_t> kinds(bmax + 2, 0);
        if (rt_schedule_final_kinds(n, tsamp, widths.data(), widths.size(), pmin, pmax, bmin, bmax, &launches, &nrows, &nseg,
                                    kinds.data(), kinds.size())) {
            std::printf("kinds: %s\n", rt_last_error());
            return 1;
        }
        std::printf("kinds launches=%llu final_row_group=%llu final_segmented=%llu", (unsigned long long)launches,
                    (unsigned long long)nrows, (unsigned long long)nseg);
        for (int k = 1; k <= 2; ++k) {
            std::printf(k == 1 ? " row_group_bins=" : " segmented_bins=");
            bool any = false;
            for (size_t b = 0; b < kinds.size();) {
                if (!(kinds[b] & k)) {
                    ++b;
                    continue;
                }
                size_t e = b;
                while (e + 1 < kinds.size() && (kinds[e + 1] & k)) ++e;
                if (e > b) std::printf("%s%zu-%zu", any ? "," : "", b, e);
                else std::printf("%s%zu", any ? "," : "", b);
                any = true;
                b = e + 1;
            }
            if (!any) std::printf("none");
        }
        std::printf("\n");
        return 0;
    }
    if (argc >= 4 && !std::strcmp(argv[1], "ffa")) {
        uint64_t launches = 0;
        if (rt_ffa_schedule_check(std::strtoull(argv[2], nullptr, 10), std::strtoull(argv[3], nullptr, 10), &launches)) {
            std::printf("ffa: %s\n", rt_last_error());
            return 1;
        }
        std::printf("ffa launches=%llu\n", (unsigned long long)launches);
        return 0;
    }
    std::fprintf(stderr, "usage: sched_check pgram N TSAMP PMIN PMAX BMIN BMAX NWIDTHS | kinds N TSAMP PMIN PMAX BMIN BMAX "
                         "WIDTH... | ffa ROWS COLS\n");
    return 2;
}
```

Baseline: 159.4.

## Add tail-4 merge bucket for 257-260 bin periods using 4-slot kernel

Introduces a new kernel bucket (kTail4) that handles fold widths just above 256 bins with the 4-slot register merge plus a small per-row tail of up to four extra bins. Those widths previously fell into the 5-slot path. The new variant computes the tail bins separately, writes full 256-wide rows with addtid LDS writes, and moves the roll lookup table to fit the extra tail entries. Scheduling, blob building and validation are extended to route these periods to the new variant. It adds new host checks and diagnostics, and it adds complexity and risk in the slot-pair handling of bin 255.

```diff
diff --git a/include/riptide_amd.h b/include/riptide_amd.h
--- a/include/riptide_amd.h
+++ b/include/riptide_amd.h
@@ -63,6 +63,13 @@
 int rt_schedule_final_kinds(size_t size, double tsamp, const uint64_t* widths, size_t num_widths, double period_min,
                             double period_max, size_t bins_min, size_t bins_max, uint64_t* launches,
                             uint64_t* rows_launches, uint64_t* seg_launches, uint8_t* bins_kinds, size_t bins_cap);
+
+int rt_schedule_buckets(size_t size, double tsamp, const uint64_t* widths, size_t num_widths, double period_min,
+                        double period_max, size_t bins_min, size_t bins_max, uint64_t* launches,
+                        uint64_t* slot4_launches, uint64_t* slot5_launches, uint64_t* tail_launches,
+                        uint64_t* mixed_launches, uint8_t* bins_buckets, size_t bins_cap);
+
+int rt_unit_blob_check(size_t rows, size_t cols, int build_bucket, int check_bucket);
 
 int rt_ladder_check(size_t size, double tsamp, double period_min, double period_max, size_t bins_min,
                     size_t bins_max, int* fused, uint64_t* rungs);
diff --git a/riptide_amd/_lib.py b/riptide_amd/_lib.py
--- a/riptide_amd/_lib.py
+++ b/riptide_amd/_lib.py
@@ -44,6 +44,9 @@
                                  _pu64]),
     "rt_schedule_final_kinds": (_c_i, [_c_sz, _c_d, _vp, _c_sz, _c_d, _c_d, _c_sz, _c_sz, _pu64, _pu64, _pu64, _vp,
                                        _c_sz]),
+    "rt_schedule_buckets": (_c_i, [_c_sz, _c_d, _vp, _c_sz, _c_d, _c_d, _c_sz, _c_sz, _pu64, _pu64, _pu64, _pu64, _pu64,
+                                   _vp, _c_sz]),
+    "rt_unit_blob_check": (_c_i, [_c_sz, _c_sz, _c_i, _c_i]),
     "rt_plan_create": (_c_i, [_c_sz, _c_d, _vp, _c_sz, _c_d, _c_d, _c_sz, _c_sz, _vp]),
     "rt_plan_destroy": (None, [_vp]),
     "rt_plan_shape": (_c_i, [_vp, _psz, _psz]),
diff --git a/riptide_amd/csrc/common.hpp b/riptide_amd/csrc/common.hpp
--- a/riptide_amd/csrc/common.hpp
+++ b/riptide_amd/csrc/common.hpp
@@ -54,9 +54,10 @@
     return p >= 8 * kSnrSegCols - 24 && p <= 8 * kSnrSegCols && wmax >= 1 && wmax <= kSnrSegWmax && rows >= 1 &&
            rows <= kSnrSegRows;
 }
+constexpr int kTail4 = 68;
 RT_HD inline bool snr_seg_unit(int smax, int levels, int p, int wmax, int rows)
 {
-    return (smax == 4 || smax == 5) && levels > 0 && snr_seg_ok(p, wmax, rows);
+    return (smax == 4 || smax == 5 || smax == kTail4) && levels > 0 && snr_seg_ok(p, wmax, rows);
 }
 constexpr int kStageRegs = 45 * 8 / kConeWaves;
 constexpr int kMaxSlots = 45;
@@ -68,11 +69,14 @@
 };
 enum : uint32_t { kSlotOne = 0, kSlotTwo = 1, kSlotPair = 2, kSlotHalf = 3 };
 constexpr int kSlotWords = 544;
-RT_HD constexpr bool resolved_slots(int smax) { return smax == 4 || smax == 5; }
+RT_HD constexpr bool resolved_slots(int smax) { return smax == 4 || smax == 5 || smax == kTail4; }
 constexpr int kAuxMetaWords = kBlobHeader + kDescEntries + kMaxRows + kSlotWords;
 constexpr int kLutPad = 64;
 constexpr int kLut4Words = 2 * (256 + 64);
 constexpr int kLut4Off = kAuxMetaWords + kLutPad - kLut4Words;
+constexpr int kTailMaxBins = 4;
+constexpr int kLutTailWords = 2 * (256 + kTailMaxBins + 64);
+constexpr int kLutTailOff = kAuxMetaWords + kLutPad - kLutTailWords;
 constexpr uint32_t kNoBlob = 0xFFFFFFFFu;
 constexpr uint32_t kCarriedRow = 1023;
 RT_HD inline int fill_chunks_bound(int n, int p, int runs) { return (n * p + 6 * runs + 3) >> 2; }
@@ -93,6 +97,16 @@
     return 0;
 }
 
+RT_HD inline bool tail4_bins(uint32_t p) { return p > 256 && p <= 256 + (uint32_t)kTailMaxBins; }
+RT_HD inline int cone_bucket(uint32_t p, uint32_t flags)
+{
+    return ((flags & 16u ) && tail4_bins(p)) ? kTail4 : merge_slots(p);
+}
+RT_HD inline bool bucket_runs(int bucket, uint32_t p)
+{
+    return bucket == kTail4 ? tail4_bins(p) : bucket == merge_slots(p);
+}
+
 RT_HD inline int pack_stride(int p)
 {
     if (p < 8) return p;
@@ -101,13 +115,14 @@
         return p == 16 ? 34 : p < 20 ? 35 : p < 25 ? 36 : p < 28 ? 37 : p == 28 ? 36 : p == 29 ? 37 : 38;
     return p | 1;
 }
-RT_HD constexpr int slot_count(int smax) { return smax == kPack2 ? 1 : smax; }
+RT_HD constexpr int slot_count(int smax) { return smax == kPack2 ? 1 : (smax == kTail4 ? 4 : smax); }
 RT_HD constexpr int row_pack(int smax) { return smax == kPack2 ? 2 : 1; }
+RT_HD constexpr int zero_row_floats(int smax) { return smax == kTail4 ? 64 * 5 : 64 * smax; }
 
 constexpr int kRw4 = (72 + kConeWaves - 1) / kConeWaves;
 RT_HD constexpr int merge_rows_per_wave(int smax)
 {
-    return smax == 4
+    return (smax == 4 || smax == kTail4)
                ? kRw4
                : (kStageRegs / slot_count(smax) < 1
                       ? 1
@@ -186,6 +201,7 @@
     kConeFuse2 = 2u,
     kConeSnrStride = 4u,
     kConeSnrSeg = 8u,
+    kConeTail4 = 16u,
     kConeDiagNoSnr = 1u << 30,
     kConeDiagNoMerge = 1u << 29,
     kConeDiagNoWrite = 1u << 28,
diff --git a/riptide_amd/csrc/ffa_kernels.hip b/riptide_amd/csrc/ffa_kernels.hip
--- a/riptide_amd/csrc/ffa_kernels.hip
+++ b/riptide_amd/csrc/ffa_kernels.hip
@@ -517,7 +517,7 @@
     if (lane < C.mine) C.sv = segs[wave * K + lane];
 }
 
-template <int SMAX, int RW>
+template <int SMAX, int RW, bool TAIL = false>
 __device__ __forceinline__ UnitCtx unit_begin(const ConeArgs& a, uint32_t item, uint32_t trial, uint32_t* aux,
                                               float* buf, int tid, bool dma, bool& ok, unsigned long long* ts = nullptr)
 {
@@ -533,9 +533,12 @@
     C.aux0 = aux;
     const int p = U.p;
     const int slots = merge_slots((uint32_t)p);
+    static_assert(!TAIL || SMAX == 4, "the tail variant is the 4-slot merge's");
+    constexpr int BUCKET = TAIL ? kTail4 : SMAX;
     ok = U.levels <= kMaxLevels && p > 0 &&
-         ((SMAX <= 5 || SMAX == kPack2) ? slots == SMAX : (slots <= SMAX && slots != kPack2));
-    const int cap = min(lds_row_capacity((uint32_t)p, SMAX), kConeWaves * RW * row_pack(SMAX));
+         (TAIL ? tail4_bins((uint32_t)p)
+               : ((SMAX <= 5 || SMAX == kPack2) ? slots == SMAX : (slots <= SMAX && slots != kPack2)));
+    const int cap = min(lds_row_capacity((uint32_t)p, BUCKET), kConeWaves * RW * row_pack(SMAX));
     if (!C.table) {
         ok = ok && SMAX != kPack2 && (!resolved_slots(SMAX) || U.levels == 0);
         C.al = (int)(((uint32_t)U.node_start * (uint32_t)p) & 3u);
@@ -556,11 +559,11 @@
                  C.nb * pack_stride(p) + words <= kLdsBufFloats;
         } else {
             ok = ok && C.nb <= cap && C.entries <= kDescEntries && words <= kAuxWords;
-            if (SMAX == 4 && C.slots) ok = ok && words <= kLut4Off;
+            if (SMAX == 4 && C.slots) ok = ok && words <= (TAIL ? kLutTailOff : kLut4Off);
             if (resolved_slots(SMAX)) ok = ok && (U.levels == 0 || (C.slots && (a.flags & kConeFuse2)));
             if (U.zero_row)
                 ok = ok && resolved_slots(SMAX) && !C.tile && U.zero_row >= 4 * U.fill_chunks &&
-                     U.zero_row + 64 * SMAX <= kLdsDataFloats;
+                     U.zero_row + zero_row_floats(BUCKET) <= kLdsDataFloats;
         }
         ok = ok && words >= kBlobHeader + C.entries + C.nb && C.nruns <= 64 * kConeWaves && (words & 3) == 0;
     }
@@ -960,11 +963,13 @@
     }
 }
 
-template <int SMAX, int RW, bool TWO>
+template <int SMAX, int RW, bool TWO, bool TAIL = false>
 __device__ __forceinline__ void merge_step_slots(const UnitCtx& C, const float* src, int p, int lo, int lane,
                                                  int wave, float (&v)[RW][SMAX], const int* loff, uint32_t& sw,
-                                                 int& nq)
-{
+                                                 int& nq, float (&tv)[kTailMaxBins], int& trow)
+{
+    static_assert(!TAIL || SMAX == 4, "the tail variant is the 4-slot merge's");
+    uint32_t swl = 0;
     constexpr int Q = (RW + 1) / 2;
     static_assert(Q <= 32, "row slots: one lane per slot row");
     const uint32_t* st = slot_table(C, lo);
@@ -976,6 +981,7 @@
         const int qc = qi < Q ? qi : Q - 1;
         const uint4 e = reinterpret_cast<const uint4*>(st)[1 + (lane >> 5) * (kConeWaves * Q) + wave * Q + qc];
         sw = lane < 32 ? e.w : 0u;
+        swl = e.w;
         s1 = (int)(e.z & 1023u);
         constexpr int roll_in = SMAX == 4 ? 0 : 1;
         if constexpr (TWO) {
@@ -1025,7 +1031,7 @@
     }
     const lds_cptr l1 = (lds_cptr)src + lane;
     const lds_cptr s0 = (lds_cptr)src;
-    const lut_cptr lutl = (lut_cptr)(C.aux0 + kLut4Off) + lane;
+    const lut_cptr lutl = (lut_cptr)(C.aux0 + (TAIL ? kLutTailOff : kLut4Off)) + lane;
     const int jl = p - 1 - 64 * (SMAX - 1);
 #pragma unroll
     for (int q = 0; q < Q; ++q) {
@@ -1058,8 +1064,9 @@
                             x = __builtin_amdgcn_update_dpp(nx, __float_as_int(ts[k]), 0x130, 0xF, 0xF, false);
                         } else {
                             x = __builtin_amdgcn_mov_dpp(__float_as_int(ts[k]), 0x130, 0xF, 0xF, true);
-                            asm volatile("s_mov_b32 m0, %2\n\tv_writelane_b32 %0, %1, m0" : "+v"(x) : "s"(w0), "s"(jl)
-                                         : "m0");
+                            if constexpr (!TAIL)
+                                asm volatile("s_mov_b32 m0, %2\n\tv_writelane_b32 %0, %1, m0" : "+v"(x) : "s"(w0), "s"(jl)
+                                             : "m0");
                         }
                         v[qb][k] = __fadd_rn(hs[k], __int_as_float(x));
                     }
@@ -1073,6 +1080,49 @@
                     row_terms<SMAX, TWO>(l1, p, lane, 32 + q, o0, o1, o2, o3, s1, s2, s3, hs, ts, s0, lutl);
 #pragma unroll
                     for (int k = 0; k < SMAX; ++k) v[qb][k] = __fadd_rn(hs[k], ts[k]);
+                }
+            }
+        }
+    }
+    trow = -1;
+    if constexpr (TAIL) {
+        const uint32_t kl = swl >> 20;
+        const bool tact = qi < nq && (lane < 32 || (kl != kSlotOne && 2 * qi + 1 < RW));
+        if (tact) trow = (int)((lane < 32 ? swl : swl >> 10) & 1023u);
+        const int T = p - 256;
+        const lds_cptr sp = (lds_cptr)src;
+        float b255 = 0.0f;
+#pragma unroll
+        for (int t = -1; t < kTailMaxBins; ++t) {
+            if (t < T && tact) {
+                const int j = 256 + t;
+                int j1 = j + s1;
+                j1 -= j1 >= p ? p : 0;
+                float r;
+                if constexpr (TWO) {
+                    int j2 = j + s2, j3 = j + s3;
+                    j2 -= j2 >= p ? p : 0;
+                    j3 -= j3 >= p ? p : 0;
+                    const float hh = lds_ld(sp + o0 + j), x1 = lds_ld(sp + o1 + j1);
+                    const float x2 = lds_ld(sp + o2 + j2), x3 = lds_ld(sp + o3 + j3);
+                    r = __fadd_rn(__fadd_rn(hh, x1), __fadd_rn(x2, x3));
+                } else {
+                    const float hh = lds_ld(sp + o0 + j), x = lds_ld(sp + o1 + j1);
+                    const uint32_t keep = o2 ? 0u : 0xFFFFFFFFu;
+                    const uint32_t neg0 = ~keep & 0x80000000u;
+                    r = __fadd_rn(hh, __uint_as_float((__float_as_uint(x) & keep) | neg0));
+                }
+                if (t < 0) b255 = r;
+                else tv[t < 0 ? 0 : t] = r;
+            }
+        }
+#pragma unroll
+        for (int q = 0; q < Q; ++q) {
+            if (q < nq && 2 * q + 1 < RW) {
+                const uint32_t kq = (uint32_t)__builtin_amdgcn_readlane((int)sw, q) >> 20;
+                if (kq == kSlotPair) {
+                    const int w = __builtin_amdgcn_readlane(__float_as_int(b255), 32 + q);
+                    asm volatile("v_writelane_b32 %0, %1, 63" : "+v"(v[2 * q + 1][3]) : "s"(w));
                 }
             }
         }
@@ -1108,10 +1158,53 @@
 }
 #endif
 
-template <int SMAX, int RW>
+__device__ __forceinline__ void write_row_full4(float* row, int lane, const float (&x)[4])
+{
+#ifndef RT_NO_ADDTID_WRITES
+    typedef __attribute__((address_space(3))) float* lds_fptr;
+    const uint32_t a = (uint32_t)__builtin_amdgcn_readfirstlane((int)(uint32_t)(uintptr_t)(lds_fptr)row);
+    (void)lane;
+    if (a <= 0xFFFFu - 768u) {
+        asm volatile("s_mov_b32 m0, %0\n\ts_nop 0\n\tds_write_addtid_b32 %1\n\tds_write_addtid_b32 %2 offset:256\n\t"
+                     "ds_write_addtid_b32 %3 offset:512\n\tds_write_addtid_b32 %4 offset:768"
+                     :: "s"(a), "v"(x[0]), "v"(x[1]), "v"(x[2]), "v"(x[3]) : "memory", "m0");
+    } else {
+        const uint32_t b = a - 32768u;
+        asm volatile("s_mov_b32 m0, %0\n\ts_nop 0\n\tds_write_addtid_b32 %1 offset:32768\n\t"
+                     "ds_write_addtid_b32 %2 offset:33024\n\tds_write_addtid_b32 %3 offset:33280\n\t"
+                     "ds_write_addtid_b32 %4 offset:33536"
+                     :: "s"(b), "v"(x[0]), "v"(x[1]), "v"(x[2]), "v"(x[3]) : "memory", "m0");
+    }
+#else
+#pragma unroll
+    for (int k = 0; k < 4; ++k) row[lane + 64 * k] = x[k];
+#endif
+}
+
+template <int SMAX, int RW, bool TAIL = false>
 __device__ __forceinline__ void write_rows_slots(float* base, float* dummy, const float (&v)[RW][SMAX], int p,
-                                                 int lane, uint32_t sw, int nq, int q)
-{
+                                                 int lane, uint32_t sw, int nq, int q,
+                                                 const float (&tv)[kTailMaxBins], int trow)
+{
+    if constexpr (TAIL) {
+#pragma unroll
+        for (int i = 0; i < RW; ++i) {
+            if (i / 2 < nq) {
+                const uint32_t w = (uint32_t)__builtin_amdgcn_readlane((int)sw, i / 2);
+                if (i % 2 == 0 || (w >> 20) != kSlotOne) {
+                    const int row = (int)((i % 2 == 0 ? w : w >> 10) & 1023u);
+                    write_row_full4(base + row * q, lane, v[i]);
+                }
+            }
+        }
+        if (trow >= 0) {
+            float* trw = base + trow * q + 256;
+#pragma unroll
+            for (int t = 0; t < kTailMaxBins; ++t)
+                if (t < p - 256) trw[t] = tv[t];
+        }
+        return;
+    }
     const bool tail_ok = lane + 64 * (SMAX - 1) < p;
 #ifndef RT_NO_ADDTID_WRITES
     if constexpr (resolved_slots(SMAX)) {
@@ -1149,11 +1242,20 @@
     }
 }
 
-template <int SMAX, int RW>
+template <int SMAX, int RW, bool TAIL = false>
 __device__ __forceinline__ void store_rows_slots(const float (&v)[RW][SMAX], int p, int lane, uint32_t sw, int nq,
-                                                 __amdgpu_buffer_rsrc_t rs, uint32_t st_o0)
-{
-    const bool tail_ok = lane + 64 * (SMAX - 1) < p;
+                                                 __amdgpu_buffer_rsrc_t rs, uint32_t st_o0,
+                                                 const float (&tv)[kTailMaxBins], int trow)
+{
+    const bool tail_ok = TAIL || lane + 64 * (SMAX - 1) < p;
+    if constexpr (TAIL) {
+        const uint32_t tb = trow >= 0 ? st_o0 + (uint32_t)(trow * p + 256) * 4u : 0x80000000u;
+#pragma unroll
+        for (int t = 0; t < kTailMaxBins; ++t)
+            if (t < p - 256)
+                __builtin_amdgcn_raw_buffer_store_b32(__float_as_uint(tv[t]), rs, (int)(tb + 4u * (uint32_t)t), 0,
+                                                      kStoreCpol);
+    }
 #pragma unroll
     for (int i = 0; i < RW; ++i) {
         if (i / 2 < nq) {
@@ -1420,7 +1522,7 @@
     }
 }
 
-template <int SMAX, int RW, class PreStore>
+template <int SMAX, int RW, bool TAIL, class PreStore>
 __device__ __forceinline__ void merge_levels(const UnitCtx& C, float* base, int p, int L, int tid, bool st,
                                              __amdgpu_buffer_rsrc_t rs, uint32_t st_o0, uint32_t flags, float* dummy,
                                              int qout, int oshift, PreStore&& pre_store)
@@ -1514,18 +1616,20 @@
                 const int* lo_src = first ? loff : nullptr;
                 uint32_t sw;
                 int nq;
-                if (two) merge_step_slots<SMAX, RW, true>(C, src, p, lo, lane, wave, v, lo_src, sw, nq);
-                else merge_step_slots<SMAX, RW, false>(C, src, p, lo, lane, wave, v, lo_src, sw, nq);
+                float tv[kTailMaxBins] = {};
+                int trow;
+                if (two) merge_step_slots<SMAX, RW, true, TAIL>(C, src, p, lo, lane, wave, v, lo_src, sw, nq, tv, trow);
+                else merge_step_slots<SMAX, RW, false, TAIL>(C, src, p, lo, lane, wave, v, lo_src, sw, nq, tv, trow);
                 l = lo - 1;
                 if (lo == 0 && st) {
                     pre_store();
-                    store_rows_slots<SMAX, RW>(v, p, lane, sw, nq, rs, st_o0);
+                    store_rows_slots<SMAX, RW, TAIL>(v, p, lane, sw, nq, rs, st_o0, tv, trow);
                     return;
                 }
                 if (!(flags & kConeDiagNoBarrier)) lds_barrier();
                 if (!(flags & kConeDiagNoWrite))
-                    write_rows_slots<SMAX, RW>(lo == 0 ? base + oshift : base, dummy, v, p, lane, sw, nq,
-                                               lo == 0 ? qout : p);
+                    write_rows_slots<SMAX, RW, TAIL>(lo == 0 ? base + oshift : base, dummy, v, p, lane, sw, nq,
+                                                     lo == 0 ? qout : p, tv, trow);
                 if (!(flags & kConeDiagNoBarrier)) lds_barrier();
             }
             return;
@@ -2233,9 +2337,11 @@
 template <int SMAX> constexpr bool kTrialLoop = SMAX >= 4;
 #endif
 
-template <int SMAX, int RWT, bool WIDE, uint32_t SNR>
+template <int SMAX, int RWT, bool WIDE, uint32_t SNR, bool TAIL = false>
 __global__ __launch_bounds__(kConeBlock, kConeWavesPerSimd) void cone_kernel(ConeArgs a)
 {
+    static_assert(!TAIL || (SMAX == 4 && RWT == 0), "the tail variant is the 4-slot merge's");
+    constexpr int kZeroFloats = zero_row_floats(TAIL ? kTail4 : SMAX);
     constexpr bool FIN = SNR != kSnrNone;
     constexpr bool SEG = SNR == kSnrSeg;
     static_assert(SNR <= kSnrSeg && (!WIDE || SNR == kSnrRows), "S/N kind");
@@ -2268,11 +2374,11 @@
     const bool dma = !(a.flags & kConeDiagNoLand);
     bool ok;
 #ifdef RT_STAMPS
-    UnitCtx C = unit_begin<SMAX, RW>(a, item, t0, aux, data, tid, dma, ok, t_begin);
+    UnitCtx C = unit_begin<SMAX, RW, TAIL>(a, item, t0, aux, data, tid, dma, ok, t_begin);
     unsigned long long tl[kStampMarks] = {};
     tl[0] = __builtin_amdgcn_s_memtime();
 #else
-    UnitCtx C = unit_begin<SMAX, RW>(a, item, t0, aux, data, tid, dma, ok);
+    UnitCtx C = unit_begin<SMAX, RW, TAIL>(a, item, t0, aux, data, tid, dma, ok);
 #endif
     const UnitView& U = C.U;
     const int p = U.p;
@@ -2285,10 +2391,10 @@
     }
     if (FIN && tid < (int)a.num_widths) snr_width_consts(wl[tid], p, whb + 2 * tid);
     if constexpr (SMAX == 4)
-        if (C.slots && ok) build_roll_lut4(aux + kLut4Off, p, tid);
+        if (C.slots && ok) build_roll_lut4(aux + (TAIL ? kLutTailOff : kLut4Off), p, tid);
     if constexpr (resolved_slots(SMAX))
         if (ok && U.zero_row)
-            for (int j = tid; j < 64 * SMAX; j += kConeBlock) data[U.zero_row + j] = -0.0f;
+            for (int j = tid; j < kZeroFloats; j += kConeBlock) data[U.zero_row + j] = -0.0f;
     if constexpr (SMAX == kPack2)
         if (ok && p >= kPackSeg) build_pack_lut(aux, p, tid);
     __builtin_amdgcn_s_waitcnt(0x0F70);
@@ -2296,7 +2402,7 @@
     RT_MARK(1);
     RT_MARK(2);
     if constexpr (SEG)
-        ok = ok && C.slots && snr_seg_unit(SMAX, L, p, wl[kMaxWidths], rows_at(C, 0));
+        ok = ok && C.slots && snr_seg_unit(TAIL ? kTail4 : SMAX, L, p, wl[kMaxWidths], rows_at(C, 0));
     if (!ok) {
         if (tid == 0 && a.error_flag) atomicOr(a.error_flag, 1);
         return;
@@ -2343,7 +2449,7 @@
             next_issued = true;
         };
         if (L > 0 && !(a.flags & kConeDiagNoMerge))
-            merge_levels<SMAX, RW>(C, buf, p, L, tid, st_regs, rs, o0, a.flags, buf + kLdsBufFloats + 4 + (tid & 63),
+            merge_levels<SMAX, RW, TAIL>(C, buf, p, L, tid, st_regs, rs, o0, a.flags, buf + kLdsBufFloats + 4 + (tid & 63),
                                    qout, SEG ? 8 * kSnrSegCols - p : 0, fill_next);
         RT_MARK(3);
         float* const obase = L > 0 ? buf : buf + (C.table ? uni(bottom_offsets(C)[0]) : C.al);
@@ -2390,7 +2496,7 @@
         if (!next_issued) fill_next();
         if constexpr (resolved_slots(SMAX) && FIN)
             if (U.zero_row)
-                for (int j = tid; j < 64 * SMAX; j += kConeBlock) data[U.zero_row + j] = -0.0f;
+                for (int j = tid; j < kZeroFloats; j += kConeBlock) data[U.zero_row + j] = -0.0f;
         ++k;
         C.U.trial = trial + 1;
 #ifdef RT_STAMPS
@@ -2406,21 +2512,23 @@
     }
 }
 
-template <int SMAX, int RW = 0>
+template <int SMAX, int RW = 0, bool TAIL = false>
 static hipError_t launch_kind(const ConeArgs& args, dim3 g, dim3 b, bool wide_snr, uint32_t snr, hipStream_t s)
 {
     if (snr == kSnrNone) {
         if (wide_snr) return hipErrorInvalidValue;
-        hipLaunchKernelGGL((cone_kernel<SMAX, RW, false, kSnrNone>), g, b, 0, s, args);
+        hipLaunchKernelGGL((cone_kernel<SMAX, RW, false, kSnrNone, TAIL>), g, b, 0, s, args);
     } else if (snr == kSnrSeg) {
         if (wide_snr || !resolved_slots(SMAX) || RW != 0) return hipErrorInvalidValue;
-        if constexpr (resolved_slots(SMAX) && RW == 0) hipLaunchKernelGGL((cone_kernel<SMAX, 0, false, kSnrSeg>), g, b, 0, s, args);
+        if constexpr (resolved_slots(SMAX) && RW == 0)
+            hipLaunchKernelGGL((cone_kernel<SMAX, 0, false, kSnrSeg, TAIL>), g, b, 0, s, args);
     } else if (snr != kSnrRows) {
         return hipErrorInvalidValue;
     } else if (wide_snr && SMAX >= 3 && SMAX <= 5 && RW == 0) {
-        if constexpr (SMAX >= 3 && SMAX <= 5 && RW == 0) hipLaunchKernelGGL((cone_kernel<SMAX, 0, true, kSnrRows>), g, b, 0, s, args);
+        if constexpr (SMAX >= 3 && SMAX <= 5 && RW == 0)
+            hipLaunchKernelGGL((cone_kernel<SMAX, 0, true, kSnrRows, TAIL>), g, b, 0, s, args);
     } else {
-        hipLaunchKernelGGL((cone_kernel<SMAX, RW, false, kSnrRows>), g, b, 0, s, args);
+        hipLaunchKernelGGL((cone_kernel<SMAX, RW, false, kSnrRows, TAIL>), g, b, 0, s, args);
     }
     return hipSuccess;
 }
@@ -2452,6 +2560,7 @@
     case 22: e = launch_kind<22>(args, g, b, wide_snr, snr, s); break;
     case kMaxSlots: e = launch_kind<kMaxSlots>(args, g, b, wide_snr, snr, s); break;
     case kPack2: e = launch_kind<kPack2>(args, g, b, wide_snr, snr, s); break;
+    case kTail4: e = launch_kind<4, 0, true>(args, g, b, wide_snr, snr, s); break;
     default: return hipErrorInvalidValue;
     }
     if (e != hipSuccess) return e;
diff --git a/riptide_amd/csrc/host_api.cpp b/riptide_amd/csrc/host_api.cpp
--- a/riptide_amd/csrc/host_api.cpp
+++ b/riptide_amd/csrc/host_api.cpp
@@ -144,6 +144,47 @@
     });
 }
 
+int rt_schedule_buckets(size_t size, double tsamp, const uint64_t* widths, size_t nw, double pmin, double pmax,
+                        size_t bmin, size_t bmax, uint64_t* launches, uint64_t* slot4_launches,
+                        uint64_t* slot5_launches, uint64_t* tail_launches, uint64_t* mixed_launches,
+                        uint8_t* bins_buckets, size_t bins_cap)
+{
+    return guarded([&] {
+        const uint32_t wmax = checked_plan_widths(widths, nw, bmin);
+        const ExecPlan ex = host_plan(size, tsamp, nw, wmax, pmin, pmax, bmin, bmax).ex;
+        uint64_t n4 = 0, n5 = 0, nt = 0, mixed = 0;
+        if (bins_buckets) std::fill(bins_buckets, bins_buckets + bins_cap, (uint8_t)0);
+        for (const Launch& L : ex.launches) {
+            const uint8_t bit = L.smax == 4 ? 1 : (L.smax == 5 ? 2 : (L.smax == (uint32_t)kTail4 ? 4 : 8));
+            n4 += bit == 1;
+            n5 += bit == 2;
+            nt += bit == 4;
+            bool wrong = false;
+            for (uint32_t i = L.first; i < L.first + L.count; ++i) {
+                const uint32_t p = ex.xf[ex.items[i].xform].p;
+                wrong = wrong || !bucket_runs((int)L.smax, p);
+                if (bins_buckets && p < bins_cap) bins_buckets[p] |= bit;
+            }
+            mixed += wrong;
+        }
+        if (launches) *launches = ex.launches.size();
+        if (slot4_launches) *slot4_launches = n4;
+        if (slot5_launches) *slot5_launches = n5;
+        if (tail_launches) *tail_launches = nt;
+        if (mixed_launches) *mixed_launches = mixed;
+        return RT_OK;
+    });
+}
+
+int rt_unit_blob_check(size_t rows, size_t cols, int build_bucket, int check_bucket)
+{
+    return guarded([&] {
+        if (rows > 0xFFFFFFFFull || cols > 0xFFFFFFFFull) throw std::invalid_argument("rt_unit_blob_check: bad shape");
+        check_unit_blob((uint32_t)rows, (uint32_t)cols, build_bucket, check_bucket);
+        return RT_OK;
+    });
+}
+
 int rt_find_peaks_workspace_bytes(size_t batch, size_t length, size_t num_widths, size_t chunk_rows, size_t* bytes)
 {
     return guarded([&] {
diff --git a/riptide_amd/csrc/plan.cpp b/riptide_amd/csrc/plan.cpp
--- a/riptide_amd/csrc/plan.cpp
+++ b/riptide_amd/csrc/plan.cpp
@@ -264,20 +264,26 @@
 
 static bool wide_snr(const FfaXform& X, int smax, bool snr_epilogue, uint32_t max_width)
 {
-    if (!snr_epilogue || smax > 5 || smax == kPack2) return false;
+    if (!snr_epilogue || (smax > 5 && smax != kTail4)) return false;
     if (snr_group((int)X.p) != 16 || (int)max_width <= kSnrWin || max_width >= X.p) return false;
     if (const char* e = std::getenv("RIPTIDE_AMD_SNR_WIDE"))
         if (e[0] == '0') return false;
     return true;
 }
 
+static uint32_t plan_cone_flags()
+{
+    if (const char* e = std::getenv("RIPTIDE_AMD_CONE_FLAGS")) return (uint32_t)std::strtoul(e, nullptr, 0);
+    return kConeDefaultFeatures;
+}
+
+static int plan_bucket(uint32_t p) { return cone_bucket(p, plan_cone_flags()); }
+
 static bool seg_snr(const FfaXform& X, int smax, bool snr_epilogue, uint32_t max_width)
 {
-    if (!snr_epilogue || (smax != 4 && smax != 5)) return false;
+    if (!snr_epilogue || (smax != 4 && smax != 5 && smax != kTail4)) return false;
     if (!snr_seg_ok((int)X.p, (int)max_width, 1)) return false;
-    if (const char* e = std::getenv("RIPTIDE_AMD_CONE_FLAGS"))
-        if (!(std::strtoul(e, nullptr, 0) & kConeSnrSeg)) return false;
-    return true;
+    return (plan_cone_flags() & kConeSnrSeg) != 0;
 }
 
 static uint32_t final_snr_kind(const FfaXform& X, int smax, uint32_t max_width, const std::vector<ConeItem>& items)
@@ -332,14 +338,14 @@
         sched.assign(g1 - g0, {});
         uint32_t gpasses = 0;
         for (size_t i = g0; i < g1; ++i) {
-            plan_transform(out.xf[i], (uint32_t)i, merge_slots(out.xf[i].p),
-                           final_tile_cap(out.xf[i], merge_slots(out.xf[i].p), snr_epilogue, max_width), sched[i - g0]);
+            plan_transform(out.xf[i], (uint32_t)i, plan_bucket(out.xf[i].p),
+                           final_tile_cap(out.xf[i], plan_bucket(out.xf[i].p), snr_epilogue, max_width), sched[i - g0]);
             gpasses = std::max<uint32_t>(gpasses, (uint32_t)sched[i - g0].size());
         }
         out.max_passes = std::max(out.max_passes, gpasses);
         const size_t first_launch = out.launches.size();
         std::vector<int> buckets;
-        for (size_t i = g0; i < g1; ++i) buckets.push_back(merge_slots(out.xf[i].p));
+        for (size_t i = g0; i < g1; ++i) buckets.push_back(plan_bucket(out.xf[i].p));
         std::sort(buckets.begin(), buckets.end());
         buckets.erase(std::unique(buckets.begin(), buckets.end()), buckets.end());
         for (uint32_t k = 0; k < gpasses; ++k) {
@@ -353,7 +359,7 @@
                 for (size_t i = g0; i < g1; ++i) {
                     auto& sp = sched[i - g0];
                     const uint32_t P = (uint32_t)sp.size();
-                    if (k >= P || merge_slots(out.xf[i].p) != bucket) continue;
+                    if (k >= P || plan_bucket(out.xf[i].p) != bucket) continue;
                     const FfaXform& X = out.xf[i];
                     const uint8_t src = k == 0 ? kSelLeaves : (((P - k) % 2 == 0) ? kSelPing : kSelPong);
                     const bool last = (k == P - 1);
@@ -399,7 +405,7 @@
     std::vector<bool> packed(out.items.size(), false);
     std::vector<int> smax_of(out.items.size(), 0);
     for (const Launch& L : out.launches) {
-        const int rw = L.smax <= 5 ? (L.rw ? (int)L.rw : merge_rows_per_wave((int)L.smax)) : 0;
+        const int rw = (L.smax <= 5 || L.smax == (uint32_t)kTail4) ? (L.rw ? (int)L.rw : merge_rows_per_wave((int)L.smax)) : 0;
         for (uint32_t i = L.first; i < L.first + L.count; ++i) {
             slot_rw[i] = rw;
             packed[i] = L.smax == (uint32_t)kPack2;
@@ -606,7 +612,8 @@
         for (int l = 0; l <= L; ++l)
             if (fused[l]) slot_off[l] = base + rel[l];
     } else if (resolved) {
-        if (!tile && L >= 2 && (L % 2) == 0 && 4 * cb + 64 * (uint32_t)smax <= (uint32_t)kLdsDataFloats) zero_row = 4 * cb;
+        if (!tile && L >= 2 && (L % 2) == 0 && 4 * cb + (uint32_t)zero_row_floats(smax) <= (uint32_t)kLdsDataFloats)
+            zero_row = 4 * cb;
         std::vector<uint32_t> sl;
         const uint32_t base0 = kBlobHeader + nb;
         const uint32_t base = (base0 + 3u) & ~3u;
@@ -651,6 +658,10 @@
                 entry(sw & 1023u, ea);
                 ea[3] = sw;
                 if ((sw >> 20) == kSlotTwo || (sw >> 20) == kSlotHalf) entry((sw >> 10) & 1023u, eb);
+                if (smax == kTail4) {
+                    if ((sw >> 20) == kSlotPair) entry((sw >> 10) & 1023u, eb);
+                    eb[3] = sw;
+                }
             }
             l = lo - 1;
         }
@@ -708,6 +719,10 @@
     kBlobHeader + kConeWaves * kRw4 + 3 + kMaxSteps4 * (4 + 4 * 2 * kConeWaves * ((kRw4 + 1) / 2));
 static_assert(kBlobLds4Worst <= kLut4Off, "4-slot unit blobs may overlap the roll table");
 static_assert((kMaxTileLevels + 1) / 2 <= kMaxSteps4, "tile steps");
+constexpr int kBlobLdsTailWorst =
+    kBlobHeader + kLdsDataFloats / 257 + 3 + kMaxSteps4 * (4 + 4 * 2 * kConeWaves * ((kRw4 + 1) / 2));
+static_assert(kBlobLdsTailWorst <= kLutTailOff, "tail-bucket unit blobs may overlap the roll table");
+static_assert(kLutTailOff + kLutTailWords == kLut4Off + kLut4Words, "roll tables end with the metadata area");
 
 static void validate_blob(const ConeItem& it, uint32_t p, int smax, int rw, const uint32_t* w)
 {
@@ -717,8 +732,10 @@
     if (runoff < (uint32_t)kBlobHeader + entries + nb + slot_words || (runoff & 3u) || nb != w[kHdrRows + L])
         throw std::runtime_error("schedule: malformed unit blob header");
     if (4 * fill > (uint32_t)kLdsBufFloats) throw std::runtime_error("schedule: unit fill exceeds the LDS level buffer");
-    if (smax == 4 && slot_words && runoff > (uint32_t)kLut4Off)
+    if (slot_words && ((smax == 4 && runoff > (uint32_t)kLut4Off) || (smax == kTail4 && runoff > (uint32_t)kLutTailOff)))
         throw std::runtime_error("schedule: unit blob overlaps the roll table");
+    if (resolved_slots(smax) && !bucket_runs(smax, p))
+        throw std::runtime_error("schedule: unit blob in the wrong kernel variant");
     uint32_t c = 0;
     const uint32_t K = (nseg + kConeWaves - 1) / kConeWaves;
     for (uint32_t i = 0; i < nseg; ++i) {
@@ -754,13 +771,14 @@
         return;
     }
     if (!slot_words) {
-        if (smax <= 5 && L > 0) throw std::runtime_error("schedule: unit without row-slot tables");
+        if ((smax <= 5 || smax == kTail4) && L > 0) throw std::runtime_error("schedule: unit without row-slot tables");
         return;
     }
     if (resolved_slots(smax)) {
         const int Q = (rw + 1) / 2;
         const uint32_t zero_row = w[kHdrZero];
-        if (zero_row && (tile || (L % 2) || zero_row < 4 * fill || zero_row + 64 * (uint32_t)smax > (uint32_t)kLdsDataFloats))
+        if (zero_row && (tile || (L % 2) || zero_row < 4 * fill ||
+                         zero_row + (uint32_t)zero_row_floats(smax) > (uint32_t)kLdsDataFloats))
             throw std::runtime_error("schedule: bad zero row");
         for (int l = (int)L - 1; l >= 0;) {
             const bool two = l >= 1 && (tile || zero_row || (it.node_size >> l) >= 2);
@@ -792,6 +810,17 @@
                 if (seen[ra]++ || (two_rows && seen[rb]++)) throw std::runtime_error("schedule: row slot covers a row twice");
                 check_entry(e);
                 if (kind == kSlotTwo || kind == kSlotHalf) check_entry(eb);
+                if (smax == kTail4) {
+                    if (eb[3] != sw) throw std::runtime_error("schedule: tail slot without row B's slot word");
+                    if (kind == kSlotPair) {
+                        check_entry(eb);
+                        const uint32_t sa = two ? (e[2] >> 10) & 1023u : e[2] & 1023u;
+                        const uint32_t sb = two ? (eb[2] >> 10) & 1023u : eb[2] & 1023u;
+                        if (eb[0] != e[0] || eb[1] != e[1] || sb != (sa + 1) % p ||
+                            (two && ((eb[2] & 1023u) != (e[2] & 1023u) || (eb[2] >> 20) != ((e[2] >> 20) + 1) % p)))
+                            throw std::runtime_error("schedule: tail pair's row B does not follow row A");
+                    }
+                }
                 if (kind == kSlotHalf &&
                     ((two ? (e[0] != eb[0] || (e[2] & 1023u) != (eb[2] & 1023u))
                           : ((e[0] & 0xFFFFu) != (eb[0] & 0xFFFFu))) ||
@@ -840,6 +869,21 @@
     }
 }
 
+void check_unit_blob(uint32_t rows, uint32_t p, int build_bucket, int check_bucket)
+{
+    if (!rows || !p || !resolved_slots(build_bucket) || !resolved_slots(check_bucket) ||
+        (int)rows > lds_row_capacity(p, build_bucket))
+        throw std::invalid_argument("check_unit_blob: a 4/5-slot whole unit within its row capacity");
+    ConeItem it{};
+    it.node_size = rows;
+    it.s1 = rows;
+    it.mode = kModeWhole;
+    while ((1u << it.levels) < rows) ++it.levels;
+    std::vector<uint32_t> blob;
+    build_tile_blob(it, p, merge_rows_per_wave(build_bucket), build_bucket, blob);
+    validate_blob(it, p, check_bucket, merge_rows_per_wave(check_bucket), blob.data());
+}
+
 void validate_exec_plan(const ExecPlan& ex, bool snr_epilogue)
 {
     std::vector<uint64_t> covered(ex.xf.size(), 0);
@@ -858,7 +902,7 @@
             const ConeItem& it = ex.items[i];
             if (it.xform >= ex.xf.size()) throw std::runtime_error("schedule: item of an unknown transform");
             const FfaXform& X = ex.xf[it.xform];
-            if (merge_slots(X.p) != (int)L.smax) throw std::runtime_error("schedule: item in the wrong kernel variant");
+            if (!bucket_runs((int)L.smax, X.p)) throw std::runtime_error("schedule: item in the wrong kernel variant");
             if (it.s1 <= it.s0 || it.s1 > it.node_size || (uint64_t)it.node_start + it.node_size > X.m)
                 throw std::runtime_error("schedule: tile outside its node");
             int rows;
diff --git a/riptide_amd/csrc/plan.hpp b/riptide_amd/csrc/plan.hpp
--- a/riptide_amd/csrc/plan.hpp
+++ b/riptide_amd/csrc/plan.hpp
@@ -73,6 +73,8 @@
 
 void validate_exec_plan(const ExecPlan& ex, bool snr_epilogue);
 
+void check_unit_blob(uint32_t rows, uint32_t p, int build_bucket, int check_bucket);
+
 constexpr uint64_t kMaxBlockBytes = 1ull << 31;
 
 struct ConeNeed { int max_rows = 0; int max_floats = 0; int ranges = 0; int rows_bottom = 0; int runs_bottom = 0; int entries = 0; bool degenerate = false; };
diff --git a/riptide_amd/csrc/sched_check_main.cpp b/riptide_amd/csrc/sched_check_main.cpp
--- a/riptide_amd/csrc/sched_check_main.cpp
+++ b/riptide_amd/csrc/sched_check_main.cpp
@@ -93,6 +93,22 @@
         std::printf("\n");
         return 0;
     }
+    if (argc >= 9 && !std::strcmp(argv[1], "buckets")) {
+        const size_t n = std::strtoull(argv[2], nullptr, 10);
+        const double tsamp = std::atof(argv[3]), pmin = std::atof(argv[4]), pmax = std::atof(argv[5]);
+        const size_t bmin = std::strtoull(argv[6], nullptr, 10), bmax = std::strtoull(argv[7], nullptr, 10);
+        std::vector<uint64_t> widths;
+        for (int i = 8; i < argc; ++i) widths.push_back(std::strtoull(argv[i], nullptr, 10));
+        uint64_t launches = 0, n4 = 0, n5 = 0, nt = 0, mixed = 0;
+        if (rt_schedule_buckets(n, tsamp, widths.data(), widths.size(), pmin, pmax, bmin, bmax, &launches, &n4, &n5, &nt,
+                                &mixed, nullptr, 0)) {
+            std::printf("buckets: %s\n", rt_last_error());
+            return 1;
+        }
+        std::printf("buckets launches=%llu slot4=%llu slot5=%llu tail4=%llu mixed=%llu\n", (unsigned long long)launches,
+                    (unsigned long long)n4, (unsigned long long)n5, (unsigned long long)nt, (unsigned long long)mixed);
+        return mixed ? 1 : 0;
+    }
     if (argc >= 4 && !std::strcmp(argv[1], "ffa")) {
         uint64_t launches = 0;
         if (rt_ffa_schedule_check(std::strtoull(argv[2], nullptr, 10), std::strtoull(argv[3], nullptr, 10), &launches)) {
```

Result: slower. 157.3 (-1.3%).
